# nianticlabs/relpose-gnn

Hardware: AMD Instinct MI355X
Metric: graphs/sec (8-node fully-connected, 224x224) (higher is better)
Workload: dtype f32; 1 GPU; BASELINE.json configs[1]: batch=32 8-node fully-connected graphs per GPU, 224x224 RGB, fp32, ResNet34 + GNN (D=2048, gnn_recursion=2, droprate=0, eval), random-init weights; nodes_per_graph=8, edges_per_graph=56, streams_per_gpu=2, loaded_library=relpose-gnn_amd/lib/librelpose_gnn_hip.so@a301a6756f67

## Files before the change

include/relpose_gnn_hip.h:

```cpp
#ifndef RELPOSE_GNN_HIP_H
#define RELPOSE_GNN_HIP_H

#include <stddef.h>
#include <stdint.h>

#ifdef __cplusplus
extern "C" {
#endif

#define RPG_OK 0
#define RPG_ERR_BAD_ARG (-1)
#define RPG_ERR_LAUNCH (-2)
#define RPG_ERR_WORKSPACE (-3)

#define RPG_ABI_VERSION 1

int rpg_abi_version(void);
const char* rpg_last_error(void);
int rpg_release_scratch(void);


int rpg_nchw3_to_nhwc4_f32(const float* x_nchw, float* y_nhwc4, int n, int h, int w, void* stream);

int rpg_conv2d_bn_act_nhwc_f32(const float* x, const float* w_ohwi, const float* scale, const float* shift,
                               const float* residual, float* y, int n, int h, int w, int cin, int cout,
                               int kh, int kw, int stride, int pad, int relu, void* stream);

size_t rpg_wino43_weights_floats(int cout, int cin);
int rpg_wino43_transform_weights_f32(const float* w_ohwi , float* u, int cout, int cin,
                                     void* stream);
int rpg_conv3x3_wino43_bn_act_nhwc_f32(const float* x, const float* u, const float* scale, const float* shift,
                                       const float* residual, float* y, int n, int h, int w, int cin, int cout,
                                       int relu, void* stream);

int rpg_stem_conv7x7s2_bn_relu_maxpool_f32(const float* x_nchw, const float* wpack, const float* shift, float* y_nhwc,
                                           int n, int h, int w, void* stream);
int rpg_stem_pair_table(int* tap_a, int* tap_b);

int rpg_maxpool3x3s2_nhwc_f32(const float* x, float* y, int n, int h, int w, int c, void* stream);

int rpg_global_avgpool_nhwc_f32(const float* x, float* y, int n, int hw, int c, void* stream);

size_t rpg_resnet_workspace_bytes(int n, int h, int w, const int* planes);
int rpg_resnet_forward_f32(const float* const* tensors, int n_tensors, const int* blocks, const int* planes,
                           int feat_dim, const float* x_nchw, int n, int h, int w, float* feat,
                           void* workspace, size_t workspace_bytes, void* stream);

int rpg_stem_conv7x7s2_bn_relu_maxpool_bf16(const float* x_nchw, const void* wpack_bf16, const float* scale, const float* shift,
                                            void* y_nhwc_bf16, int n, int h, int w, void* stream);
int rpg_stem_conv7x7s2_bn_relu_maxpool_bf16_xbf16(const void* x_nchw_bf16, const void* wpack_bf16, const float* scale, const float* shift,
                                                  void* y_nhwc_bf16, int n, int h, int w, void* stream);
int rpg_conv2d_bn_act_nhwc_bf16(const void* x, const void* w_ohwi, const float* scale, const float* shift,
                                const void* residual, void* y, int n, int h, int w, int cin, int cout, int kh, int kw,
                                int stride, int pad, int relu, int out_f32, void* stream);
size_t rpg_resnet_bf16_workspace_bytes(int n, int h, int w, const int* planes);
int rpg_resnet_forward_bf16(const void* const* tensors, int n_tensors, const int* blocks, const int* planes, int feat_dim,
                            const float* x_nchw, int n, int h, int w, float* feat, void* workspace,
                            size_t workspace_bytes, void* stream);
int rpg_resnet_forward_bf16_xbf16(const void* const* tensors, int n_tensors, const int* blocks, const int* planes, int feat_dim,
                                  const void* x_nchw_bf16, int n, int h, int w, float* feat, void* workspace,
                                  size_t workspace_bytes, void* stream);


int rpg_graph_prepare(const int64_t* src, const int64_t* dst, int64_t node_offset, int e, int n, int64_t* ends,
                      int32_t* rowptr, int32_t* cursor, int32_t* perm, int32_t* status, void* stream);

int rpg_knn_graph_f32(const float* x, const int64_t* batch, int n, int d, int k, int64_t* edge_index,
                      int32_t* cand, int32_t* cnt, int32_t* total, int32_t* status, void* stream);

int rpg_edge_concat_gather_f32(const float* x, const int64_t* edge_index, int e, int d, float* out, void* stream);

int rpg_linear_gather_f32(int n_src, const float* const* a, const int64_t* const* idx, const int* ld,
                          const int* width, const float* weight, const float* bias, const float* residual,
                          float* out, int m, int n_out, int relu, void* stream);

int rpg_linear_gather_ex_f32(int n_src, const float* const* a, const int64_t* const* idx, const int* ld,
                             const int* width, const long* rows, const float* weight, const float* bias,
                             const float* residual, const int64_t* res_idx, const float* residual2,
                             const int64_t* res2_idx, int ldr, float* out, float* out_relu, int m, int n_out, int relu,
                             void* stream);

int rpg_attention_rows_f32(const float* gtp, int r, int c, float* y, void* stream);

int rpg_scatter_mean_f32(const float* msg, const int32_t* rowptr, const int32_t* perm, int n, int e, int d,
                         float* out, void* stream);

int rpg_attention_aggregate_f32(const float* gtp, const float* msg, const int32_t* rowptr, const int32_t* perm,
                                const float* bias, int n, int e, int c, int d, float* ybar, float* mbar, void* stream);

int rpg_pose_heads_f32(const float* x, const float* w6, const float* b6, int r, int d, float* out, void* stream);

size_t rpg_gnn_workspace_bytes(int n, int e, int d);
int rpg_gnn_forward_f32(const float* const* tensors, int n_tensors, const float* feat, const int64_t* src,
                        const int64_t* dst, int64_t node_offset, int n, int e, int d, int gnn_recursion,
                        float* abs_pose, float* rel_pose,
                        float* node_out, float* edge_out, int32_t* status, void* workspace,
                        size_t workspace_bytes, void* stream);

int rpg_gnn_forward_bf16(const float* const* tensors, int n_tensors, const void* const* weights_bf16, int n_bf16,
                         const float* feat, const int64_t* src, const int64_t* dst, int64_t node_offset, int n, int e, int d,
                         int gnn_recursion, float* abs_pose, float* rel_pose, float* node_out, float* edge_out,
                         int32_t* status, void* workspace, size_t workspace_bytes, void* stream);

int rpg_basicblock64_bf16(const void* x, const void* w1_ohwi, const float* scale1, const float* shift1, const void* w2_ohwi,
                          const float* scale2, const float* shift2, void* y, int n, int h, int w, void* stream);

int rpg_f32_to_bf16(const float* src, int ld_src, void* dst, int ld_dst, int col_off, long rows, int cols, void* stream);
int rpg_linear_bf16(const void* a, const void* weight, const float* bias, const float* residual, const int64_t* res_idx,
                    const float* residual2, const int64_t* res2_idx, int ldr, float* out, int m, int k, int n_out,
                    int relu, void* stream);

#define RPG_TIMER_CONV 0
#define RPG_TIMER_LINEAR 1
#define RPG_TIMER_SCATTER 2
#define RPG_TIMER_ATTENTION 3
#define RPG_TIMER_CONV_WINO 4
#define RPG_TIMER_ATT_AGG 5
#define RPG_TIMER_COUNT 6
int rpg_timing_enable(int enable);
int rpg_timing_read(double* ms, long long* launches, double* work);
int rpg_timing_read_ex(double* ms, long long* launches, double* work, double* executed);

int rpg_probe_mfma_bf16(const void* operands, long iters, int workgroups, float* sink, void* stream);

#define RPG_TUNE_TILE 0
#define RPG_TUNE_BK 1
#define RPG_TUNE_EPILOGUE 2
#define RPG_TUNE_STREAMK 3
#define RPG_TUNE_GNN_SPLIT 5
#define RPG_TUNE_BF16_BK 6
#define RPG_TUNE_BF16_FAST 9
#define RPG_TUNE_GNN_FUSE_AGG 13
#define RPG_TUNE_WAVES8 11
#define RPG_TUNE_FUSED_STEM 10
#define RPG_TUNE_WINO_SPLIT 8
#define RPG_TUNE_FAST_LOADER 7
#define RPG_TUNE_WINOGRAD 4
#define RPG_TUNE_WINO_SHORT 12
#define RPG_TUNE_WINO_PERSIST 14
#define RPG_TUNE_BF16_TILE 15
#define RPG_TUNE_BF16_DMA 16
#define RPG_TUNE_BF16_PATCH 17
#define RPG_TUNE_BF16_WS64 18
int rpg_host_f32_to_bf16(const float* src, void* dst_bf16, size_t count);
int rpg_host_f32_to_bf16_isa(const float* src, void* dst_bf16, size_t count, int isa);

#define RPG_TUNE_SK_MIN_ITS 19
#define RPG_TUNE_INKERNEL_FIXUP 20
#define RPG_TUNE_BF16_CHUNK 21
#define RPG_TUNE_WINO2D 22
#define RPG_TUNE_BF16_LEAN_EPI 23
#define RPG_TUNE_BF16_LINEAR_DMA 24
#define RPG_TUNE_BF16_PERSIST 25
#define RPG_TUNE_FOLD_K 26
#define RPG_TUNE_BF16_FUSE_BLOCK 27
#define RPG_TUNE_BF16_TAIL 28
#define RPG_TUNE_LIN112 29
#define RPG_TUNE_FIXUP_PRIO 30
#define RPG_TUNE_BF16_PAIR 31
int rpg_set_tuning(int key, int value);

#ifdef __cplusplus
}
#endif
#endif
```

relpose-gnn_amd/_lib.py:

```python
from __future__ import annotations

import ctypes as C
import os
from typing import Optional, Sequence

HERE = os.path.dirname(os.path.abspath(__file__))
LIB_PATH = os.environ.get("RPG_HIP_LIB") or os.path.join(HERE, "lib", "librelpose_gnn_hip.so")

RPG_OK, RPG_ERR_BAD_ARG, RPG_ERR_LAUNCH, RPG_ERR_WORKSPACE = 0, -1, -2, -3
TIMER_NAMES = ("conv", "linear", "scatter", "attention", "conv_wino", "att_agg")

SYMBOLS = (
    "rpg_abi_version", "rpg_last_error", "rpg_nchw3_to_nhwc4_f32", "rpg_conv2d_bn_act_nhwc_f32",
    "rpg_maxpool3x3s2_nhwc_f32", "rpg_global_avgpool_nhwc_f32", "rpg_resnet_workspace_bytes",
    "rpg_resnet_forward_f32", "rpg_graph_prepare", "rpg_edge_concat_gather_f32", "rpg_linear_gather_f32",
    "rpg_attention_rows_f32", "rpg_scatter_mean_f32", "rpg_pose_heads_f32", "rpg_gnn_workspace_bytes",
    "rpg_gnn_forward_f32", "rpg_timing_enable", "rpg_timing_read", "rpg_set_tuning", "rpg_knn_graph_f32", "rpg_wino43_transform_weights_f32", "rpg_wino43_weights_floats",
    "rpg_conv3x3_wino43_bn_act_nhwc_f32", "rpg_conv2d_bn_act_nhwc_bf16", "rpg_resnet_bf16_workspace_bytes",
    "rpg_resnet_forward_bf16", "rpg_gnn_forward_bf16", "rpg_f32_to_bf16", "rpg_linear_bf16",
    "rpg_release_scratch", "rpg_timing_read_ex", "rpg_stem_conv7x7s2_bn_relu_maxpool_f32", "rpg_stem_pair_table",
    "rpg_attention_aggregate_f32", "rpg_stem_conv7x7s2_bn_relu_maxpool_bf16", "rpg_stem_conv7x7s2_bn_relu_maxpool_bf16_xbf16",
    "rpg_resnet_forward_bf16_xbf16", "rpg_host_f32_to_bf16", "rpg_basicblock64_bf16", "rpg_linear_gather_ex_f32", "rpg_probe_mfma_bf16", "rpg_host_f32_to_bf16_isa",
)


class HipLibraryMissing(RuntimeError):
    pass


class RpgError(RuntimeError):
    pass


_lib: Optional[C.CDLL] = None
_vp, _i, _sz = C.c_void_p, C.c_int, C.c_size_t


def _declare(lib: C.CDLL) -> None:
    lib.rpg_abi_version.restype = _i
    lib.rpg_last_error.restype = C.c_char_p
    lib.rpg_nchw3_to_nhwc4_f32.argtypes = [_vp, _vp, _i, _i, _i, _vp]
    lib.rpg_conv2d_bn_act_nhwc_f32.argtypes = [_vp] * 6 + [_i] * 10 + [_vp]
    lib.rpg_maxpool3x3s2_nhwc_f32.argtypes = [_vp, _vp, _i, _i, _i, _i, _vp]
    lib.rpg_global_avgpool_nhwc_f32.argtypes = [_vp, _vp, _i, _i, _i, _vp]
    lib.rpg_resnet_workspace_bytes.argtypes = [_i, _i, _i, C.POINTER(_i)]
    lib.rpg_resnet_workspace_bytes.restype = _sz
    lib.rpg_resnet_forward_f32.argtypes = [C.POINTER(_vp), _i, C.POINTER(_i), C.POINTER(_i), _i, _vp, _i, _i, _i, _vp,
                                           _vp, _sz, _vp]
    lib.rpg_graph_prepare.argtypes = [_vp, _vp, C.c_int64, _i, _i, _vp, _vp, _vp, _vp, _vp, _vp]
    lib.rpg_edge_concat_gather_f32.argtypes = [_vp, _vp, _i, _i, _vp, _vp]
    lib.rpg_linear_gather_f32.argtypes = [_i, C.POINTER(_vp), C.POINTER(_vp), C.POINTER(_i), C.POINTER(_i), _vp, _vp,
                                          _vp, _vp, _i, _i, _i, _vp]
    lib.rpg_linear_gather_ex_f32.argtypes = [_i, C.POINTER(_vp), C.POINTER(_vp), C.POINTER(_i), C.POINTER(_i), C.POINTER(C.c_long),
                                             _vp, _vp, _vp, _vp, _vp, _vp, _i, _vp, _vp, _i, _i, _i, _vp]
    lib.rpg_attention_rows_f32.argtypes = [_vp, _i, _i, _vp, _vp]
    lib.rpg_scatter_mean_f32.argtypes = [_vp, _vp, _vp, _i, _i, _i, _vp, _vp]
    lib.rpg_attention_aggregate_f32.argtypes = [_vp, _vp, _vp, _vp, _vp, _i, _i, _i, _i, _vp, _vp, _vp]
    lib.rpg_pose_heads_f32.argtypes = [_vp, _vp, _vp, _i, _i, _vp, _vp]
    lib.rpg_gnn_workspace_bytes.argtypes = [_i, _i, _i]
    lib.rpg_gnn_workspace_bytes.restype = _sz
    lib.rpg_gnn_forward_f32.argtypes = [C.POINTER(_vp), _i, _vp, _vp, _vp, C.c_int64, _i, _i, _i, _i, _vp, _vp, _vp, _vp,
                                        _vp, _vp, _sz, _vp]
    lib.rpg_gnn_forward_bf16.argtypes = [C.POINTER(_vp), _i, C.POINTER(_vp), _i, _vp, _vp, _vp, C.c_int64, _i, _i, _i, _i, _vp,
                                         _vp, _vp, _vp, _vp, _vp, _sz, _vp]
    lib.rpg_f32_to_bf16.argtypes = [_vp, _i, _vp, _i, _i, C.c_long, _i, _vp]
    lib.rpg_linear_bf16.argtypes = [_vp] * 7 + [_i, _vp, _i, _i, _i, _i, _vp]
    lib.rpg_timing_enable.argtypes = [_i]
    lib.rpg_set_tuning.argtypes = [_i, _i]
    lib.rpg_conv2d_bn_act_nhwc_bf16.argtypes = [_vp] * 6 + [_i] * 11 + [_vp]
    lib.rpg_basicblock64_bf16.argtypes = [_vp] * 8 + [_i] * 3 + [_vp]
    lib.rpg_resnet_bf16_workspace_bytes.argtypes = [_i, _i, _i, C.POINTER(_i)]
    lib.rpg_resnet_bf16_workspace_bytes.restype = _sz
    lib.rpg_resnet_forward_bf16.argtypes = [C.POINTER(_vp), _i, C.POINTER(_i), C.POINTER(_i), _i, _vp, _i, _i, _i, _vp,
                                            _vp, _sz, _vp]
    lib.rpg_wino43_transform_weights_f32.argtypes = [_vp, _vp, _i, _i, _vp]
    lib.rpg_wino43_weights_floats.argtypes = [_i, _i]
    lib.rpg_wino43_weights_floats.restype = C.c_size_t
    lib.rpg_conv3x3_wino43_bn_act_nhwc_f32.argtypes = [_vp] * 6 + [_i] * 6 + [_vp]
    lib.rpg_knn_graph_f32.argtypes = [_vp, _vp, _i, _i, _i, _vp, _vp, _vp, _vp, _vp, _vp]
    lib.rpg_timing_read.argtypes = [C.POINTER(C.c_double), C.POINTER(C.c_longlong), C.POINTER(C.c_double)]
    lib.rpg_timing_read_ex.argtypes = [C.POINTER(C.c_double), C.POINTER(C.c_longlong), C.POINTER(C.c_double),
                                       C.POINTER(C.c_double)]
    lib.rpg_release_scratch.argtypes = []
    lib.rpg_stem_conv7x7s2_bn_relu_maxpool_f32.argtypes = [_vp, _vp, _vp, _vp, _i, _i, _i, _vp]
    lib.rpg_stem_pair_table.argtypes = [C.POINTER(_i), C.POINTER(_i)]
    lib.rpg_stem_conv7x7s2_bn_relu_maxpool_bf16.argtypes = [_vp, _vp, _vp, _vp, _vp, _i, _i, _i, _vp]
    lib.rpg_stem_conv7x7s2_bn_relu_maxpool_bf16_xbf16.argtypes = [_vp, _vp, _vp, _vp, _vp, _i, _i, _i, _vp]
    lib.rpg_resnet_forward_bf16_xbf16.argtypes = lib.rpg_resnet_forward_bf16.argtypes
    lib.rpg_host_f32_to_bf16.argtypes = [_vp, _vp, _sz]
    lib.rpg_host_f32_to_bf16_isa.argtypes = [_vp, _vp, _sz, _i]
    lib.rpg_probe_mfma_bf16.argtypes = [_vp, C.c_long, _i, _vp, _vp]
    for name in SYMBOLS:
        getattr(lib, name)


def lib() -> C.CDLL:
    global _lib
    if _lib is None:
        path = os.environ.get("RPG_LIB_PATH") or LIB_PATH
        return _load(path)
    return _lib


def _load(LIB_PATH: str) -> C.CDLL:
    global _lib
    if _lib is None:
        if not os.path.exists(LIB_PATH):
            raise HipLibraryMissing(
                f"{LIB_PATH} not found: build it with `python relpose-gnn_amd/build.py` "
                "(the HIP library is the only compute path; there is no fallback)")
        l = C.CDLL(LIB_PATH)
        _declare(l)
        if l.rpg_abi_version() != 1:
            raise HipLibraryMissing(f"{LIB_PATH}: ABI version {l.rpg_abi_version()} != 1, rebuild")
        _lib = l
    return _lib


def check(rc: int, what: str) -> None:
    if rc == RPG_OK:
        return
    if rc == RPG_ERR_BAD_ARG:
        raise ValueError(f"{what}: bad argument (null pointer, non-positive size, unsupported shape or alignment)")
    if rc == RPG_ERR_WORKSPACE:
        raise RpgError(f"{what}: workspace too small")
    msg = lib().rpg_last_error().decode(errors="replace")
    raise RpgError(f"{what}: HIP launch failed: {msg}")


def ptr_array(ptrs: Sequence[Optional[int]]):
    arr = (_vp * len(ptrs))()
    for i, p in enumerate(ptrs):
        arr[i] = p
    return arr


def int_array(vals: Sequence[int]):
    return (_i * len(vals))(*vals)
```

relpose-gnn_amd/build.py:

```python
from __future__ import annotations

import os
import shutil
import subprocess
import sys

HERE = os.path.dirname(os.path.abspath(__file__))
CSRC = os.path.join(HERE, "csrc")
LIB_DIR = os.path.join(HERE, "lib")
LIB_PATH = os.path.join(LIB_DIR, "librelpose_gnn_hip.so")
SOURCES = ("gemm_f32.hip", "winograd.hip", "stem.hip", "stem_bf16.hip", "conv_bf16.hip", "encoder_ops.hip", "gnn_ops.hip", "forward.hip", "timing.hip", "host_ops.hip")
ARCH = "gfx950"
WINOGRAD_SOURCES = ("winograd.hip", "rpg_coherent.h")


def _hipcc() -> str:
    for cand in (os.environ.get("HIPCC"), shutil.which("hipcc"), "/opt/rocm/bin/hipcc"):
        if cand and os.path.exists(cand):
            return cand
    raise RuntimeError("hipcc not found (set HIPCC or install ROCm under /opt/rocm)")


def source_digest(names=None) -> str:
    import hashlib
    h = hashlib.sha256()
    if names is not None:
        files = [os.path.join(CSRC, f) for f in sorted(names)]
    else:
        files = sorted(os.path.join(CSRC, f) for f in os.listdir(CSRC)) + [
            os.path.join(os.path.dirname(HERE), "include", "relpose_gnn_hip.h")]
    for f in files:
        h.update(os.path.basename(f).encode())
        with open(f, "rb") as fh:
            h.update(fh.read())
    return h.hexdigest()[:12]


def needs_build() -> bool:
    if not os.path.exists(LIB_PATH):
        return True
    t = os.path.getmtime(LIB_PATH)
    deps = [os.path.join(CSRC, f) for f in os.listdir(CSRC)] + [
        os.path.join(os.path.dirname(HERE), "include", "relpose_gnn_hip.h")]
    return any(os.path.getmtime(d) > t for d in deps)


def build(force: bool = False, verbose: bool = False) -> str:
    defines = os.environ.get("RPG_BUILD_DEFINES", "").split()
    if defines:
        return _build_to(os.path.join(LIB_DIR, "librelpose_gnn_hip_probe.so"), defines, verbose, obj_suffix=".probe.o")
    if not force and not needs_build():
        return LIB_PATH
    return _build_to(LIB_PATH, [], verbose)


def _build_to(lib_path: str, defines, verbose: bool, obj_suffix: str = ".o") -> str:
    os.makedirs(LIB_DIR, exist_ok=True)
    from concurrent.futures import ThreadPoolExecutor

    def compile_one(src):
        obj = os.path.join(LIB_DIR, src.replace(".hip", obj_suffix))
        cmd = [_hipcc(), f"--offload-arch={ARCH}", "-O3", "-std=c++17", "-fPIC", *defines,
               "-c", os.path.join(CSRC, src), "-o", obj]
        if verbose:
            print(" ".join(cmd), flush=True)
        subprocess.run(cmd, check=True)
        return obj
    with ThreadPoolExecutor(max_workers=min(4, os.cpu_count() or 1)) as pool:
        objs = list(pool.map(compile_one, SOURCES))
    cmd = [_hipcc(), f"--offload-arch={ARCH}", "-shared", "-fPIC", "-o", lib_path + ".tmp", *objs]
    if verbose:
        print(" ".join(cmd), flush=True)
    subprocess.run(cmd, check=True)
    os.replace(lib_path + ".tmp", lib_path)
    return lib_path


if __name__ == "__main__":
    print(build(force="--force" in sys.argv, verbose=True))
```

relpose-gnn_amd/csrc/forward.hip:

```cpp
#include "rpg_common.h"

namespace rpg {
int launch_relu_inplace(float* x, long n_floats, hipStream_t s);
bool stem_pool_supported(int h, int w, int cout);
int launch_stem_pool(const float* x_nchw, const float* wpack, const float* shift, float* out, int n, int h, int w, hipStream_t s);
}

namespace {

inline size_t align_up(size_t v, size_t a) { return (v + a - 1) / a * a; }
inline int conv_out(int x, int k, int s, int p) { return (x + 2 * p - k) / s + 1; }

struct Carver {
    char* base;
    size_t off;
    template <class T>
    T* take(size_t count) {
        T* p = reinterpret_cast<T*>(base + off);
        off += align_up(count * sizeof(T), 256) + rpg::kWorkspaceSkew;
        return p;
    }
};

struct ResnetPlan {
    int h1, w1, h2, w2;
    size_t in4, stem, blk, pool, total_bytes;
};

ResnetPlan plan_resnet(int n, int h, int w, const int* planes) {
    ResnetPlan p{};
    p.h1 = conv_out(h, 7, 2, 3); p.w1 = conv_out(w, 7, 2, 3);
    p.h2 = conv_out(p.h1, 3, 2, 1); p.w2 = conv_out(p.w1, 3, 2, 1);
    p.in4 = (size_t)n * h * w * 4;
    p.stem = (size_t)n * p.h1 * p.w1 * planes[0];
    size_t blk = 0;
    int hh = p.h2, ww = p.w2;
    for (int l = 0; l < 4; ++l) {
        if (l > 0) { hh = conv_out(hh, 3, 2, 1); ww = conv_out(ww, 3, 2, 1); }
        const size_t sz = (size_t)n * hh * ww * planes[l];
        if (sz > blk) blk = sz;
    }
    p.blk = blk;
    p.pool = (size_t)n * planes[3];
    p.total_bytes = align_up(p.in4 * 4, 256) + align_up(p.stem * 4, 256) + 4 * align_up(p.blk * 4, 256) +
                    align_up(p.pool * 4, 256) + align_up(rpg::split_scratch_bytes(), 256) + 8 * rpg::kWorkspaceSkew;
    return p;
}

}

extern "C" size_t rpg_resnet_workspace_bytes(int n, int h, int w, const int* planes) {
    if (n <= 0 || h <= 0 || w <= 0 || !planes) return 0;
    return plan_resnet(n, h, w, planes).total_bytes;
}

extern "C" int rpg_resnet_forward_f32(const float* const* tensors, int n_tensors, const int* blocks, const int* planes,
                                      int feat_dim, const float* x_nchw, int n, int h, int w, float* feat,
                                      void* workspace, size_t workspace_bytes, void* stream) {
    if (!tensors || !blocks || !planes || !x_nchw || !feat || !workspace || n <= 0 || h <= 0 || w <= 0 || feat_dim <= 0)
        return RPG_ERR_BAD_ARG;
    int expect = 4 + 2, cin = planes[0];
    for (int l = 0; l < 4; ++l)
        for (int b = 0; b < blocks[l]; ++b) {
            const int stride = (l > 0 && b == 0) ? 2 : 1;
            expect += 8 + ((stride != 1 || cin != planes[l]) ? 4 : 0);
            cin = planes[l];
        }
    if (n_tensors != expect) return RPG_ERR_BAD_ARG;
    for (int i = 0; i < n_tensors; ++i)
        if (!tensors[i] && !((i & 3) == 3 && i < n_tensors - 2)) return RPG_ERR_BAD_ARG;
    const ResnetPlan p = plan_resnet(n, h, w, planes);
    if (workspace_bytes < p.total_bytes) return RPG_ERR_WORKSPACE;
    hipStream_t s = rpg::as_stream(stream);

    Carver cv{reinterpret_cast<char*>(workspace), 0};
    float* in4 = cv.take<float>(p.in4);
    float* stem = cv.take<float>(p.stem);
    float* buf[4];
    for (int i = 0; i < 4; ++i) buf[i] = cv.take<float>(p.blk);
    float* pool = cv.take<float>(p.pool);
    const size_t scratch_bytes = rpg::split_scratch_bytes();
    rpg::ScratchScope scratch(cv.take<char>(scratch_bytes), scratch_bytes, s);

    int rc;
    int ti = 0;
    if (tensors[3] && rpg::stem_pool_supported(h, w, planes[0])) {
        if ((rc = rpg::launch_stem_pool(x_nchw, tensors[3], tensors[2], buf[0], n, h, w, s)) != RPG_OK) return rc;
    } else {
        if ((rc = rpg_nchw3_to_nhwc4_f32(x_nchw, in4, n, h, w, stream)) != RPG_OK) return rc;
        if ((rc = rpg::launch_conv(in4, tensors[ti], tensors[ti + 1], tensors[ti + 2], nullptr, stem, n, h, w, 4,
                                   planes[0], 7, 7, 2, 3, 1, s, 3)) != RPG_OK)
            return rc;
        if ((rc = rpg_maxpool3x3s2_nhwc_f32(stem, buf[0], n, p.h1, p.w1, planes[0], stream)) != RPG_OK) return rc;
    }
    ti += 4;

    int cur = 0, hh = p.h2, ww = p.w2;
    cin = planes[0];
    for (int l = 0; l < 4; ++l) {
        for (int b = 0; b < blocks[l]; ++b) {
            const int stride = (l > 0 && b == 0) ? 2 : 1;
            const int c = planes[l];
            const bool ds = (stride != 1 || cin != c);
            const int ho = conv_out(hh, 3, stride, 1), wo = conv_out(ww, 3, stride, 1);
            float* X = buf[cur];
            float* T = buf[(cur + 1) & 3];
            float* Y = buf[(cur + 2) & 3];
            float* D = buf[(cur + 3) & 3];
            const bool wino1 = stride == 1 && tensors[ti + 3] && rpg::wino_pays(n, hh, ww, cin, c);
            const bool wino2 = tensors[ti + 7] && rpg::wino_pays(n, ho, wo, c, c);
            if (wino1)
                rc = rpg::launch_conv_wino(X, tensors[ti + 3], tensors[ti + 1], tensors[ti + 2], nullptr, T, n, hh, ww, cin,
                                           c, 1, s);
            else
                rc = rpg::launch_conv(X, tensors[ti], tensors[ti + 1], tensors[ti + 2], nullptr, T, n, hh, ww, cin, c, 3, 3,
                                      stride, 1, 1, s);
            if (rc != RPG_OK) return rc;
            const float* identity = X;
            if (ds) {
                if ((rc = rpg::launch_conv(X, tensors[ti + 8], tensors[ti + 9], tensors[ti + 10], nullptr, D, n, hh, ww,
                                           cin, c, 1, 1, stride, 0, 0, s)) != RPG_OK)
                    return rc;
                identity = D;
            }
            if (wino2)
                rc = rpg::launch_conv_wino(T, tensors[ti + 7], tensors[ti + 5], tensors[ti + 6], identity, Y, n, ho, wo, c, c,
                                           1, s);
            else
                rc = rpg::launch_conv(T, tensors[ti + 4], tensors[ti + 5], tensors[ti + 6], identity, Y, n, ho, wo, c, c, 3,
                                      3, 1, 1, 1, s);
            if (rc != RPG_OK) return rc;
            ti += ds ? 12 : 8;
            cur = (cur + 2) & 3;
            hh = ho; ww = wo; cin = c;
        }
    }
    if ((rc = rpg_global_avgpool_nhwc_f32(buf[cur], pool, n, hh * ww, cin, stream)) != RPG_OK) return rc;
    rpg::GatherSrc src{};
    src.n = 1; src.a[0] = pool; src.idx[0] = nullptr; src.ld[0] = cin; src.width[0] = cin;
    return rpg::launch_linear(src, tensors[ti], tensors[ti + 1], nullptr, feat, n, feat_dim, 0, s);
}

namespace {
enum GnnTensor {
    T_PROJ_W, T_PROJ_B, T_EDGE0_W, T_EDGE0_B, T_EDGE2_W, T_EDGE2_B, T_MSG0_W, T_MSG0_B, T_MSG2_W, T_MSG2_B,
    T_GTP_W, T_GTP_B, T_ATTW_W, T_ATTW_B, T_UPD0_W, T_UPD0_B, T_UPD2_W, T_UPD2_B, T_HEADN_W, T_HEADN_B,
    T_HEADE_W, T_HEADE_B, T_COUNT,
    T_PROJN_W = T_COUNT,
    T_NODE3_W,
    T_EDGE0E_W,
    T_MSG0E_W,
    T_COUNT_SPLIT
};

struct GnnPlan {
    size_t total_bytes;
};
size_t gnn_bytes(int n, int e, int d) {
    const size_t c = d / 8;
    size_t b = 0;
    auto add = [&](size_t bytes, int count = 1) { b += count * (align_up(bytes, 256) + rpg::kWorkspaceSkew); };
    add((size_t)4 * e * 8);
    add((size_t)(n + 1) * 4);
    add((size_t)n * 4);
    add((size_t)e * 4);
    add((size_t)e * d * 4, 6);
    add((size_t)e * 3 * c * 4);
    add((size_t)e * c * 4);
    add((size_t)n * d * 4, 4);
    add((size_t)n * 3 * d * 4);
    add((size_t)(e > 2 * n ? e : 2 * n) * d * 2);
    add(rpg::split_scratch_bytes());
    return b;
}
}

extern "C" size_t rpg_gnn_workspace_bytes(int n, int e, int d) {
    if (n <= 0 || e <= 0 || d <= 0 || (d & 31)) return 0;
    return gnn_bytes(n, e, d);
}

namespace {
enum BfWeight { B_PROJN, B_NODE3, B_EDGE0E, B_EDGE2, B_MSG0E, B_MSG2, B_GTP, B_ATTW, B_UPD0, B_UPD2, B_COUNT };

int gnn_forward_impl(const float* const* tensors, int n_tensors, const void* const* wb, const float* feat, const int64_t* esrc,
                     const int64_t* edst, int64_t node_offset, int n, int e, int d, int gnn_recursion, float* abs_pose,
                     float* rel_pose, float* node_out, float* edge_out, int32_t* status, void* workspace,
                     size_t workspace_bytes, void* stream) {
    if (!tensors || (n_tensors != T_COUNT && n_tensors != T_COUNT_SPLIT) || !feat || !esrc || !edst || !abs_pose || !rel_pose || !status || !workspace ||
        n <= 0 || e <= 0 || d <= 0 || (d & 31) || gnn_recursion < 0)
        return RPG_ERR_BAD_ARG;
    for (int i = 0; i < n_tensors; ++i)
        if (!tensors[i]) return RPG_ERR_BAD_ARG;
    if (workspace_bytes < gnn_bytes(n, e, d)) return RPG_ERR_WORKSPACE;
    const bool split = (n_tensors == T_COUNT_SPLIT) && (wb || rpg::gnn_split_enabled());
    if (wb && !split) return RPG_ERR_BAD_ARG;
    hipStream_t s = rpg::as_stream(stream);
    const int c = d / 8;

    Carver cv{reinterpret_cast<char*>(workspace), 0};
    int64_t* ends = cv.take<int64_t>((size_t)4 * e);
    int32_t* rowptr = cv.take<int32_t>((size_t)n + 1);
    int32_t* cursor = cv.take<int32_t>((size_t)n);
    int32_t* perm = cv.take<int32_t>((size_t)e);
    float* ebuf[2] = {cv.take<float>((size_t)e * d), cv.take<float>((size_t)e * d)};
    float* eraw = cv.take<float>((size_t)e * d);
    float* hid = cv.take<float>((size_t)e * d);
    float* msg = cv.take<float>((size_t)e * d);
    float* att = cv.take<float>((size_t)e * d);
    float* gtp = cv.take<float>((size_t)e * 3 * c);
    float* yat = cv.take<float>((size_t)e * c);
    float* agg = cv.take<float>((size_t)n * d);
    float* nhid = cv.take<float>((size_t)n * d);
    float* xbuf[2] = {cv.take<float>((size_t)n * d), cv.take<float>((size_t)n * d)};
    float* node3 = cv.take<float>((size_t)n * 3 * d);
    void* abf = cv.take<unsigned short>((size_t)(e > 2 * n ? e : 2 * n) * d);
    const size_t scratch_bytes = rpg::split_scratch_bytes();
    rpg::ScratchScope scratch(cv.take<char>(scratch_bytes), scratch_bytes, s);

    int rc;
    if ((rc = rpg_graph_prepare(esrc, edst, node_offset, e, n, ends, rowptr, cursor, perm, status, stream)) != RPG_OK) return rc;
    const int64_t* src = ends;
    const int64_t* dst = ends + e;
    const int64_t* lo = ends + 2 * (size_t)e;
    const int64_t* hi = ends + 3 * (size_t)e;

    auto linear = [&](int ns, const float* a0, const int64_t* i0, int w0, const float* a1, const int64_t* i1, int w1,
                      const float* a2, const int64_t* i2, int w2, int wt, const float* residual, float* out, int m,
                      int n_out, int relu, float* out_relu = nullptr, bool with_bias = true) {
        const float* bias = with_bias ? tensors[wt + 1] : nullptr;
        rpg::GatherSrc g{};
        g.n = ns;
        g.a[0] = a0; g.idx[0] = i0; g.ld[0] = w0; g.width[0] = w0;
        g.a[1] = a1; g.idx[1] = i1; g.ld[1] = w1; g.width[1] = w1;
        g.a[2] = a2; g.idx[2] = i2; g.ld[2] = w2; g.width[2] = w2;
        for (int i = 0; i < 3; ++i) g.rows[i] = g.idx[i] ? (n > e ? n : e) : 0;
        if (wb) {
            int bw = -1;
            switch (wt) {
                case T_EDGE2_W: bw = B_EDGE2; break;
                case T_MSG2_W: bw = B_MSG2; break;
                case T_GTP_W: bw = B_GTP; break;
                case T_ATTW_W: bw = B_ATTW; break;
                case T_UPD0_W: bw = B_UPD0; break;
                case T_UPD2_W: bw = B_UPD2; break;
                default: return RPG_ERR_BAD_ARG;
            }
            const int k = w0 + (ns > 1 ? w1 : 0);
            if (ns > 2 || i0 || i1) return RPG_ERR_BAD_ARG;
            int r2;
            if ((r2 = rpg::launch_f32_to_bf16(a0, w0, abf, k, 0, m, w0, s)) != RPG_OK) return r2;
            if (ns > 1 && (r2 = rpg::launch_f32_to_bf16(a1, w1, abf, k, w0, m, w1, s)) != RPG_OK) return r2;
            if (out_relu) return RPG_ERR_BAD_ARG;
            return rpg::launch_linear_bf16(abf, wb[bw], bias, residual, nullptr, nullptr, nullptr, n_out, out, m, k,
                                           n_out, relu, s);
        }
        return rpg::launch_linear(g, tensors[wt], bias, residual, out, m, n_out, relu, s, nullptr, out_relu);
    };

    auto node_gemm = [&](const float* xin, int wt, int n_out) {
        rpg::GatherSrc g{};
        g.n = 1; g.a[0] = xin; g.idx[0] = nullptr; g.ld[0] = d; g.width[0] = d;
        if (wb) {
            int r2;
            if ((r2 = rpg::launch_f32_to_bf16(xin, d, abf, d, 0, n, d, s)) != RPG_OK) return r2;
            return rpg::launch_linear_bf16(abf, wb[wt == T_PROJN_W ? B_PROJN : B_NODE3], nullptr, nullptr, nullptr, nullptr,
                                           nullptr, 0, node3, n, d, n_out, 0, s);
        }
        return rpg::launch_linear(g, tensors[wt], nullptr, nullptr, node3, n, n_out, 0, s);
    };
    auto edge_gemm = [&](const float* ein, int wt, int bias_t, const float* r1, const int64_t* i1, const float* r2,
                         const int64_t* i2, float* out) {
        rpg::GatherSrc g{};
        g.n = 1; g.a[0] = ein; g.idx[0] = nullptr; g.ld[0] = d; g.width[0] = d;
        const rpg::GatherRes gr{r1, i1, r2, i2, 3 * d};
        if (wb) {
            int rcb;
            if ((rcb = rpg::launch_f32_to_bf16(ein, d, abf, d, 0, e, d, s)) != RPG_OK) return rcb;
            return rpg::launch_linear_bf16(abf, wb[wt == T_EDGE0E_W ? B_EDGE0E : B_MSG0E], tensors[bias_t], r1, i1, r2, i2, 3 * d,
                                           out, e, d, d, 1, s);
        }
        return rpg::launch_linear(g, tensors[wt], tensors[bias_t], nullptr, out, e, d, 1, s, &gr);
    };

    const bool fuse_agg = rpg::gnn_fuse_agg_enabled();
    if (wb && fuse_agg && split) {
        typedef unsigned short bf;
        {
            const size_t e_buf = (size_t)e * d * sizeof(float), n_buf = (size_t)n * d * sizeof(float);
            const size_t a_buf = (size_t)(e > 2 * n ? e : 2 * n) * d * sizeof(bf);
            if (2 * (size_t)e * d * sizeof(bf) > e_buf ||
                (size_t)n * 2 * d * sizeof(bf) > n_buf ||
                (size_t)n * d * sizeof(bf) > n_buf ||
                (size_t)n * c * sizeof(bf) > a_buf)
                return RPG_ERR_WORKSPACE;
        }
        bf* eb = reinterpret_cast<bf*>(eraw);
        bf* enb = eb + (size_t)e * d;
        bf* hb = reinterpret_cast<bf*>(hid);
        bf* mb = hb + (size_t)e * d;
        bf* xab = reinterpret_cast<bf*>(nhid);
        bf* nhb = reinterpret_cast<bf*>(agg);
        bf* yb = reinterpret_cast<bf*>(abf);
        auto gemm = [&](const void* a, int lda, int k, int bw, const float* bias, const float* r1, const int64_t* i1, const float* r2,
                        const int64_t* i2, int ldr, void* out, int out_f32, void* out2, int ld2, int relu2, int m, int n_out, int relu) {
            rpg::LinearBf16Out o{};
            o.out = out; o.out_f32 = out_f32; o.out2 = out2; o.ld2 = ld2; o.relu2 = relu2;
            return rpg::launch_linear_bf16_ex(a, lda, wb[bw], bias, r1, i1, r2, i2, ldr, o, m, k, n_out, relu, s);
        };
        if ((rc = rpg::launch_f32_to_bf16(feat, d, xab, 2 * d, 0, n, d, s)) != RPG_OK) return rc;
        if ((rc = gemm(xab, 2 * d, d, B_PROJN, nullptr, nullptr, nullptr, nullptr, nullptr, 0, node3, 1, nullptr, 0, 0, n, 2 * d, 0)) != RPG_OK) return rc;
        float* ecur = ebuf[0];
        if ((rc = rpg::launch_gather_add2_relu(node3, lo, hi, tensors[T_PROJ_B], ecur, e, d, s)) != RPG_OK) return rc;
        if ((rc = rpg::launch_f32_to_bf16(ecur, d, eb, d, 0, e, d, s)) != RPG_OK) return rc;
        const float* x = feat;
        for (int r = 0; r < gnn_recursion; ++r) {
            const bool last = r + 1 == gnn_recursion;
            float* xnew = xbuf[r & 1];
            if ((rc = gemm(xab, 2 * d, d, B_NODE3, nullptr, nullptr, nullptr, nullptr, nullptr, 0, node3, 1, nullptr, 0, 0, n, 3 * d, 0)) != RPG_OK) return rc;
            if ((rc = gemm(eb, d, d, B_EDGE0E, tensors[T_EDGE0_B], node3, src, node3 + d, dst, 3 * d, hb, 0, nullptr, 0, 0, e, d, 1)) != RPG_OK) return rc;
            if (last) rc = gemm(hb, d, d, B_EDGE2, tensors[T_EDGE2_B], nullptr, nullptr, nullptr, nullptr, 0, ebuf[1], 1, enb, d, 0, e, d, 1);
            else rc = gemm(hb, d, d, B_EDGE2, tensors[T_EDGE2_B], nullptr, nullptr, nullptr, nullptr, 0, eb, 0, enb, d, 0, e, d, 1);
            if (rc != RPG_OK) return rc;
            if (last) ecur = ebuf[1];
            if ((rc = gemm(enb, d, d, B_MSG0E, tensors[T_MSG0_B], node3 + 2 * d, src, nullptr, nullptr, 3 * d, hb, 0, nullptr, 0, 0, e, d, 1)) != RPG_OK) return rc;
            if ((rc = gemm(hb, d, d, B_MSG2, tensors[T_MSG2_B], nullptr, nullptr, nullptr, nullptr, 0, msg, 1, mb, d, 0, e, d, 0)) != RPG_OK) return rc;
            if ((rc = gemm(mb, d, d, B_GTP, tensors[T_GTP_B], nullptr, nullptr, nullptr, nullptr, 0, gtp, 1, nullptr, 0, 0, e, 3 * c, 0)) != RPG_OK) return rc;
            if ((rc = rpg_attention_aggregate_f32(gtp, msg, rowptr, perm, tensors[T_ATTW_B], n, e, c, d, yat, att, stream)) != RPG_OK) return rc;
            if ((rc = rpg::launch_f32_to_bf16(yat, c, yb, c, 0, n, c, s)) != RPG_OK) return rc;
            if ((rc = gemm(yb, c, c, B_ATTW, nullptr, att, nullptr, nullptr, nullptr, d, nullptr, 0, xab + d, 2 * d, 0, n, d, 0)) != RPG_OK) return rc;
            if ((rc = gemm(xab, 2 * d, 2 * d, B_UPD0, tensors[T_UPD0_B], nullptr, nullptr, nullptr, nullptr, 0, nhb, 0, nullptr, 0, 0, n, d, 1)) != RPG_OK) return rc;
            if ((rc = gemm(nhb, d, d, B_UPD2, tensors[T_UPD2_B], nullptr, nullptr, nullptr, nullptr, 0, xnew, 1, xab, 2 * d, 1, n, d, 1)) != RPG_OK) return rc;
            x = xnew;
        }
        if (node_out && hipMemcpyAsync(node_out, x, (size_t)n * d * 4, hipMemcpyDeviceToDevice, s) != hipSuccess) {
            rpg::set_last_error("gnn_forward node_out", hipGetLastError());
            return RPG_ERR_LAUNCH;
        }
        if (edge_out && hipMemcpyAsync(edge_out, ecur, (size_t)e * d * 4, hipMemcpyDeviceToDevice, s) != hipSuccess) {
            rpg::set_last_error("gnn_forward edge_out", hipGetLastError());
            return RPG_ERR_LAUNCH;
        }
        if ((rc = rpg_pose_heads_f32(x, tensors[T_HEADN_W], tensors[T_HEADN_B], n, d, abs_pose, stream)) != RPG_OK) return rc;
        return rpg_pose_heads_f32(ecur, tensors[T_HEADE_W], tensors[T_HEADE_B], e, d, rel_pose, stream);
    }

    const float* x = feat;
    float* ecur = ebuf[0];
    if (split) {
        if ((rc = node_gemm(x, T_PROJN_W, 2 * d)) != RPG_OK) return rc;
        if ((rc = rpg::launch_gather_add2_relu(node3, lo, hi, tensors[T_PROJ_B], ecur, e, d, s)) != RPG_OK) return rc;
    } else if ((rc = linear(2, x, lo, d, x, hi, d, nullptr, nullptr, 0, T_PROJ_W, nullptr, ecur, e, d, 1)) != RPG_OK) {
        return rc;
    }

    const bool dual = !wb;
    for (int r = 0; r < gnn_recursion; ++r) {
        float* enext = (ecur == ebuf[0]) ? ebuf[1] : ebuf[0];
        float* enew = dual ? eraw : enext;
        float* xnew = xbuf[r & 1];
        if (split) {
            if ((rc = node_gemm(x, T_NODE3_W, 3 * d)) != RPG_OK) return rc;
            if ((rc = edge_gemm(ecur, T_EDGE0E_W, T_EDGE0_B, node3, src, node3 + d, dst, hid)) != RPG_OK) return rc;
        } else if ((rc = linear(3, x, src, d, x, dst, d, ecur, nullptr, d, T_EDGE0_W, nullptr, hid, e, d, 1)) != RPG_OK) {
            return rc;
        }
        if ((rc = linear(1, hid, nullptr, d, nullptr, nullptr, 0, nullptr, nullptr, 0, T_EDGE2_W, nullptr, enew, e, d, 0,
                         dual ? enext : nullptr)) != RPG_OK)
            return rc;
        if (split) {
            if ((rc = edge_gemm(enew, T_MSG0E_W, T_MSG0_B, node3 + 2 * d, src, nullptr, nullptr, hid)) != RPG_OK) return rc;
        } else if ((rc = linear(2, x, src, d, enew, nullptr, d, nullptr, nullptr, 0, T_MSG0_W, nullptr, hid, e, d, 1)) != RPG_OK) {
            return rc;
        }
        if ((rc = linear(1, hid, nullptr, d, nullptr, nullptr, 0, nullptr, nullptr, 0, T_MSG2_W, nullptr, msg, e, d, 0)) != RPG_OK) return rc;
        if ((rc = linear(1, msg, nullptr, d, nullptr, nullptr, 0, nullptr, nullptr, 0, T_GTP_W, nullptr, gtp, e, 3 * c, 0)) != RPG_OK) return rc;
        if (fuse_agg) {
            if ((rc = rpg_attention_aggregate_f32(gtp, msg, rowptr, perm, tensors[T_ATTW_B], n, e, c, d, yat, att, stream)) != RPG_OK)
                return rc;
            if ((rc = linear(1, yat, nullptr, c, nullptr, nullptr, 0, nullptr, nullptr, 0, T_ATTW_W, att, agg, n, d, 0, nullptr,
                             false)) != RPG_OK)
                return rc;
        } else {
            if ((rc = rpg_attention_rows_f32(gtp, e, c, yat, stream)) != RPG_OK) return rc;
            if ((rc = linear(1, yat, nullptr, c, nullptr, nullptr, 0, nullptr, nullptr, 0, T_ATTW_W, msg, att, e, d, 0)) != RPG_OK) return rc;
            if ((rc = rpg_scatter_mean_f32(att, rowptr, perm, n, e, d, agg, stream)) != RPG_OK) return rc;
        }
        if ((rc = linear(2, x, nullptr, d, agg, nullptr, d, nullptr, nullptr, 0, T_UPD0_W, nullptr, nhid, n, d, 1)) != RPG_OK) return rc;
        if ((rc = linear(1, nhid, nullptr, d, nullptr, nullptr, 0, nullptr, nullptr, 0, T_UPD2_W, nullptr, xnew, n, d, 1)) != RPG_OK) return rc;
        if (!dual && (rc = rpg::launch_relu_inplace(enext, (long)e * d, s)) != RPG_OK) return rc;
        x = xnew;
        ecur = enext;
    }
    if (node_out && hipMemcpyAsync(node_out, x, (size_t)n * d * 4, hipMemcpyDeviceToDevice, s) != hipSuccess) {
        rpg::set_last_error("gnn_forward node_out", hipGetLastError());
        return RPG_ERR_LAUNCH;
    }
    if (edge_out && hipMemcpyAsync(edge_out, ecur, (size_t)e * d * 4, hipMemcpyDeviceToDevice, s) != hipSuccess) {
        rpg::set_last_error("gnn_forward edge_out", hipGetLastError());
        return RPG_ERR_LAUNCH;
    }
    if ((rc = rpg_pose_heads_f32(x, tensors[T_HEADN_W], tensors[T_HEADN_B], n, d, abs_pose, stream)) != RPG_OK) return rc;
// ... 23 lines not shown
```

relpose-gnn_amd/csrc/gemm_f32.hip:

```cpp
#include <atomic>
#include <map>
#include <mutex>
#include <type_traits>
#include <utility>
#include <vector>

#include "rpg_common.h"

typedef float f32x16 __attribute__((ext_vector_type(16)));

namespace {


struct Epilogue {
    const float* scale;
    const float* shift;
    const float* residual;
    float* out;
    int ldc;
    int relu;
    const int64_t* res_idx = nullptr;
    const float* residual2 = nullptr;
    const int64_t* res2_idx = nullptr;
    int ldr = 0;
// ... 193 lines not shown
        const int row = qj < 4 ? 32 * qj : L112_BM + 32 * (qj - 4);
        if (qj == 3) {
            if (srow < 16) *reinterpret_cast<float4*>(&lds[img + st_off + row * L112_LD]) = rr[set][qj];
        } else {
            *reinterpret_cast<float4*>(&lds[img + st_off + row * L112_LD]) = rr[set][qj];
        }
    };
    const int a_off = (lane & 15) * L112_LD + 4 * (lane >> 4);
    const int b_off = (L112_BM + 16 * wave + (lane & 15)) * L112_LD + 4 * (lane >> 4);
    float4 fa[2][7], fb[2];
    auto read_job = [&](int set, int rj, int kb, int img) {
        if (rj < 7) fa[set][rj] = *reinterpret_cast<const float4*>(&lds[img + a_off + rj * 16 * L112_LD + kb]);
        else fb[set] = *reinterpret_cast<const float4*>(&lds[img + b_off + kb]);
    };
    auto comp = [](const float4& v, int c) { return c == 0 ? v.x : c == 1 ? v.y : c == 2 ? v.z : v.w; };
    f32x4m acc[7], acc2[7];
#pragma unroll
    for (int i = 0; i < 7; ++i)
#pragma unroll
        for (int e = 0; e < 4; ++e) { acc[i][e] = 0.f; acc2[i][e] = 0.f; }

    const int nsteps = K / L112_BK;
    auto kstep = [&](int cur, int nxt, int wset, int kload) {
        __builtin_amdgcn_sched_barrier(0);
#pragma unroll
        for (int g = 0; g < 2; ++g) {
#pragma unroll
            for (int ms = 0; ms < 28; ++ms) {
                const int c = ms / 7, i = ms % 7;
                acc[i] = __builtin_amdgcn_mfma_f32_16x16x4f32(comp(fa[g][i], c), comp(fb[g], c), acc[i], 0, 0, 0);
                if (g == 0) {
                    if (ms < 8) read_job(1, ms, 16, cur);
                    else if (ms < 14) write_job(wset, ms - 8, nxt);
                    else if (ms < 20) load_job(wset, ms - 14, kload);
                } else {
                    if (ms < 8) read_job(0, ms, 0, nxt);
                }
                __builtin_amdgcn_sched_barrier(0);
            }
            if (g == 0) {
                __syncthreads();
                __builtin_amdgcn_sched_barrier(0);
            }
        }
    };
#pragma unroll
    for (int qj = 0; qj < 6; ++qj) load_job(0, qj, 0);
#pragma unroll
    for (int qj = 0; qj < 6; ++qj) load_job(1, qj, L112_BK);
#pragma unroll
    for (int qj = 0; qj < 6; ++qj) write_job(0, qj, 0);
#pragma unroll
    for (int qj = 0; qj < 6; ++qj) load_job(0, qj, 2 * L112_BK);
    __syncthreads();
#pragma unroll
    for (int rj = 0; rj < 8; ++rj) read_job(0, rj, 0, 0);
    const int fold_steps = fold_k >= 2 * L112_BK ? (fold_k / L112_BK) & ~1 : 0x7ffffffe;
    int kt = 0;
    while (kt + 1 < nsteps) {
        int kstop = kt + fold_steps;
        if (kstop > nsteps) kstop = nsteps;
        for (; kt + 1 < kstop; kt += 2) {
            kstep(0, L112_STAGE, 1, (kt + 3) * L112_BK);
            kstep(L112_STAGE, 0, 0, (kt + 4) * L112_BK);
        }
        if (kt + 1 < nsteps) {
            asm volatile("");
#pragma unroll
            for (int i = 0; i < 7; ++i) { acc2[i] += acc[i]; acc[i] = f32x4m{0.f, 0.f, 0.f, 0.f}; }
        }
    }
    if (kt < nsteps) kstep(0, L112_STAGE, 1, (kt + 3) * L112_BK);
#pragma unroll
    for (int i = 0; i < 7; ++i) acc[i] += acc2[i];
    __syncthreads();
    constexpr int SP = L112_BN + 4;
#pragma unroll
    for (int i = 0; i < 7; ++i)
#pragma unroll
        for (int e = 0; e < 4; ++e) lds[(16 * i + 4 * (lane >> 4) + e) * SP + 16 * wave + (lane & 15)] = acc[i][e];
    __syncthreads();
#pragma unroll
    for (int t = 0; t < L112_BM * (L112_BN / 4) / L112_NT; ++t) {
        const int idx4 = t * L112_NT + tid;
        const int row = idx4 / (L112_BN / 4), c4 = idx4 % (L112_BN / 4);
        const float4 v = *reinterpret_cast<const float4*>(&lds[row * SP + 4 * c4]);
        eng4::streamk_finish_quad<L112_BM, L112_BN>(v, ep, M, N, tiles_n, tile, idx4, 1);
    }
}

constexpr int L112_NT2 = 512;
__global__ __launch_bounds__(L112_NT2, 1) void linear112k2_kernel(const float* __restrict__ A, int lda, const float* __restrict__ Wt, int ldw,
                                                                 int M, int N, int K, Epilogue ep, int tiles_n, int fold_k) {
    extern __shared__ __attribute__((aligned(16))) float lds[];
    const int nwg = gridDim.x, bid = blockIdx.x;
    const int xcd = bid & 7, loc = bid >> 3, q = nwg >> 3, r = nwg & 7;
    const int tile = (xcd < r ? xcd * (q + 1) : r * (q + 1) + (xcd - r) * q) + loc;
    const int m0 = (tile / tiles_n) * L112_BM, n0 = (tile % tiles_n) * L112_BN;
    const int tid = threadIdx.x, lane = tid & 63;
    const int wave = __builtin_amdgcn_readfirstlane(tid >> 6);
    const int kw = wave >> 2, wv = wave & 3;
    const int slot = tid & 7, srow = tid >> 3;
    const __amdgpu_buffer_rsrc_t rsa = make_rsrc(A + (size_t)m0 * lda);
    const __amdgpu_buffer_rsrc_t rsw = make_rsrc(Wt + (size_t)n0 * ldw);
    unsigned soff[3];
    soff[0] = 4u * (unsigned)(srow * lda + 4 * slot);
    soff[1] = srow + 64 < L112_BM ? 4u * (unsigned)((srow + 64) * lda + 4 * slot) : OOB;
    soff[2] = 4u * (unsigned)(srow * ldw + 4 * slot);
    const int st_off = srow * L112_LD + 4 * slot;
    float4 rr[2][3];
    auto load_job = [&](int set, int qj, int kpos) {
        const bool live = kpos < K;
        rr[set][qj] = buf_ld4(qj < 2 ? rsa : rsw, live ? soff[qj] : OOB, 4u * (unsigned)kpos);
    };
    auto write_job = [&](int set, int qj, int img) {
        const int row = qj == 0 ? 0 : (qj == 1 ? 64 : L112_BM);
        if (qj == 1) {
            if (srow + 64 < L112_BM) *reinterpret_cast<float4*>(&lds[img + st_off + row * L112_LD]) = rr[set][qj];
        } else {
            *reinterpret_cast<float4*>(&lds[img + st_off + row * L112_LD]) = rr[set][qj];
        }
    };
    const int a_off = (lane & 15) * L112_LD + 4 * (lane >> 4) + 16 * kw;
    const int b_off = (L112_BM + 16 * wv + (lane & 15)) * L112_LD + 4 * (lane >> 4) + 16 * kw;
    float4 fa[2][7], fb[2];
    auto read_job = [&](int set, int rj, int img) {
        if (rj < 7) fa[set][rj] = *reinterpret_cast<const float4*>(&lds[img + a_off + rj * 16 * L112_LD]);
        else fb[set] = *reinterpret_cast<const float4*>(&lds[img + b_off]);
    };
    auto comp = [](const float4& v, int c) { return c == 0 ? v.x : c == 1 ? v.y : c == 2 ? v.z : v.w; };
    f32x4m acc[7], acc2[7];
#pragma unroll
    for (int i = 0; i < 7; ++i)
#pragma unroll
        for (int e = 0; e < 4; ++e) { acc[i][e] = 0.f; acc2[i][e] = 0.f; }
    const int nsteps = K / L112_BK;
    auto kstep = [&](int fset, int nxt, int wset, int kload) {
        __builtin_amdgcn_sched_barrier(0);
#pragma unroll
        for (int ms = 0; ms < 28; ++ms) {
            const int c = ms / 7, i = ms % 7;
            acc[i] = __builtin_amdgcn_mfma_f32_16x16x4f32(comp(fa[fset][i], c), comp(fb[fset], c), acc[i], 0, 0, 0);
            if (ms < 3) write_job(wset, ms, nxt);
            else if (ms < 6) load_job(wset, ms - 3, kload);
            else if (ms >= 14 && ms < 22) read_job(fset ^ 1, ms - 14, nxt);
            __builtin_amdgcn_sched_barrier(0);
            if (ms == 13) {
                __syncthreads();
                __builtin_amdgcn_sched_barrier(0);
            }
        }
    };
#pragma unroll
    for (int qj = 0; qj < 3; ++qj) load_job(0, qj, 0);
#pragma unroll
    for (int qj = 0; qj < 3; ++qj) load_job(1, qj, L112_BK);
#pragma unroll
    for (int qj = 0; qj < 3; ++qj) write_job(0, qj, 0);
#pragma unroll
    for (int qj = 0; qj < 3; ++qj) load_job(0, qj, 2 * L112_BK);
    __syncthreads();
#pragma unroll
    for (int rj = 0; rj < 8; ++rj) read_job(0, rj, 0);
    const int fold_steps = fold_k >= 2 * L112_BK ? (fold_k / L112_BK) & ~1 : 0x7ffffffe;
    int kt = 0;
    while (kt + 1 < nsteps) {
        int kstop = kt + fold_steps;
        if (kstop > nsteps) kstop = nsteps;
        for (; kt + 1 < kstop; kt += 2) {
            kstep(0, L112_STAGE, 1, (kt + 3) * L112_BK);
            kstep(1, 0, 0, (kt + 4) * L112_BK);
        }
        if (kt + 1 < nsteps) {
            asm volatile("");
#pragma unroll
            for (int i = 0; i < 7; ++i) { acc2[i] += acc[i]; acc[i] = f32x4m{0.f, 0.f, 0.f, 0.f}; }
        }
    }
    if (kt < nsteps) kstep(0, L112_STAGE, 1, (kt + 3) * L112_BK);
#pragma unroll
    for (int i = 0; i < 7; ++i) acc[i] += acc2[i];
    __syncthreads();
    constexpr int SP = L112_BN + 4;
    if (kw == 1) {
#pragma unroll
        for (int i = 0; i < 7; ++i)
#pragma unroll
            for (int e = 0; e < 4; ++e) lds[(16 * i + 4 * (lane >> 4) + e) * SP + 16 * wv + (lane & 15)] = acc[i][e];
    }
    __syncthreads();
    if (kw == 0) {
#pragma unroll
        for (int i = 0; i < 7; ++i)
#pragma unroll
            for (int e = 0; e < 4; ++e) {
                float* p = &lds[(16 * i + 4 * (lane >> 4) + e) * SP + 16 * wv + (lane & 15)];
                *p = acc[i][e] + *p;
            }
    }
    __syncthreads();
    for (int idx4 = tid; idx4 < L112_BM * (L112_BN / 4); idx4 += L112_NT2) {
        const int row = idx4 / (L112_BN / 4), c4 = idx4 % (L112_BN / 4);
        const float4 v = *reinterpret_cast<const float4*>(&lds[row * SP + 4 * c4]);
        eng4::streamk_finish_quad<L112_BM, L112_BN>(v, ep, M, N, tiles_n, tile, idx4, 1);
    }
}

bool launch_linear112(const float* A, int lda, const float* Wt, int ldw, int M, int N, int K, const Epilogue& ep, hipStream_t s) {
    if (!(g_lin112 & 1) || M % L112_BM || N % L112_BN || K % L112_BK || K < 2 * L112_BK) return false;
    const int tm = M / L112_BM, tn = N / L112_BN;
    const long tiles = (long)tm * tn;
    if (tiles < cu_count() || (long)L112_BM * lda * 4 >= (1L << 31) || (long)L112_BN * ldw * 4 >= (1L << 31)) return false;
    const bool vec_ok = (ep.ldc % 4 == 0) && rpg::aligned16(ep.out) && (!ep.residual || rpg::aligned16(ep.residual)) &&
                        (!ep.residual2 || rpg::aligned16(ep.residual2)) && (ep.ldr % 4 == 0) && (!ep.scale || rpg::aligned16(ep.scale)) &&
                        (!ep.shift || rpg::aligned16(ep.shift)) && (!ep.out_relu || rpg::aligned16(ep.out_relu)) && rpg::aligned16(A) &&
                        rpg::aligned16(Wt) && (lda % 4 == 0) && (ldw % 4 == 0);
    if (!vec_ok) return false;
    t_executed = 2.0 * (double)M * N * (double)K;
    if ((g_lin112 & 2) && 2 * tiles < 3L * cu_count())
        hipLaunchKernelGGL(linear112k2_kernel, dim3((unsigned)tiles), dim3(L112_NT2), L112_LDS_BYTES, s, A, lda, Wt, ldw, M, N, K, ep, tn, g_fold_k);
    else
        hipLaunchKernelGGL(linear112_kernel, dim3((unsigned)tiles), dim3(L112_NT), L112_LDS_BYTES, s, A, lda, Wt, ldw, M, N, K, ep, tn, g_fold_k);
    return true;
}

template <int BK, bool EPI, template <int, int> class Loader, class Args>
void launch_shape(TileShape t, const Args& args, const float* Wt, int ldw, int M, int N, int K, const Epilogue& ep,
                  bool vec_ok, hipStream_t s) {
    switch (t) {
        case TILE_128x128: eng4::launch_one<128, 128, 2, 2, BK, EPI, Loader, Args>(args, Wt, ldw, M, N, K, ep, vec_ok, s); break;
        case TILE_256x64: eng4::launch_one<256, 64, 4, 1, BK, EPI, Loader, Args>(args, Wt, ldw, M, N, K, ep, vec_ok, s); break;
        case TILE_128x64: eng4::launch_one<128, 64, 2, 2, BK, EPI, Loader, Args>(args, Wt, ldw, M, N, K, ep, vec_ok, s); break;
        default: eng4::launch_one<64, 64, 2, 2, BK, EPI, Loader, Args>(args, Wt, ldw, M, N, K, ep, vec_ok, s); break;
    }
}

template <template <int, int> class Loader8, class Args>
void launch_shape8(TileShape t, const Args& args, const float* Wt, int ldw, int M, int N, int K, const Epilogue& ep,
                   hipStream_t s) {
    if (t == TILE_128x128) eng8::launch_one<128, 128, 2, 4, 32, true, Loader8, Args>(args, Wt, ldw, M, N, K, ep, true, s);
    else eng8::launch_one<128, 64, 4, 2, 32, true, Loader8, Args>(args, Wt, ldw, M, N, K, ep, true, s);
}

int g_fast = 1;
int g_waves8 = 1;

struct ConvKind {
    template <int R, int BK> using L4 = eng4::ConvLoader<R, BK>;
    template <int R, int BK> using B4 = eng4::ConvLoaderB<R, BK>;
    template <int R, int BK> using T4 = eng4::ConvLoaderTap<R, BK>;
    template <int R, int BK> using B8 = eng8::ConvLoaderB<R, BK>;
};
struct GatherKind {
    template <int R, int BK> using L4 = eng4::GatherLoader<R, BK>;
    template <int R, int BK> using B4 = eng4::GatherLoaderB<R, BK>;
    template <int R, int BK> using T4 = eng4::GatherLoaderB<R, BK>;
    template <int R, int BK> using B8 = eng8::GatherLoaderB<R, BK>;
};

template <class Kind, class Args>
int launch_tiles(const Args& args, const float* Wt, int ldw, int M, int N, int K, const Epilogue& ep, hipStream_t s,
                 int seg_align) {
    TileShape t = pick_tile(M, N, K);
    if (std::is_same<Kind, GatherKind>::value && g_fold_k > 0 && g_force_tile < 0 && t == TILE_128x128 && K >= 2 * g_fold_k) t = TILE_128x64;
    const int bk = g_bk ? g_bk : (((t == TILE_128x128 || t == TILE_128x64) && K >= 256) ? 32 : 16);
    const bool vec_ok = (N % 4 == 0) && (ep.ldc % 4 == 0) && rpg::aligned16(ep.out) &&
                        (!ep.residual || rpg::aligned16(ep.residual)) && (!ep.residual2 || rpg::aligned16(ep.residual2)) &&
                        (ep.ldr % 4 == 0) && (!ep.scale || rpg::aligned16(ep.scale)) &&
                        (!ep.shift || rpg::aligned16(ep.shift));
    const bool epi = g_epi_lds && vec_ok;
    const bool fast = g_fast && epi && seg_align > 0 && seg_align % bk == 0 && K % bk == 0 &&
                      (long)N * ldw * 4 < (1L << 31);
    if (g_fast && epi && seg_align == -1 && (long)N * ldw * 4 < (1L << 31)) {
        if (bk == 32) launch_shape<32, true, Kind::template T4, Args>(t, args, Wt, ldw, M, N, K, ep, vec_ok, s);
        else launch_shape<16, true, Kind::template T4, Args>(t, args, Wt, ldw, M, N, K, ep, vec_ok, s);
        return 0;
    }
    if (fast && bk == 32 && g_waves8 && (t == TILE_128x128 || t == TILE_128x64)) {
        launch_shape8<Kind::template B8, Args>(t, args, Wt, ldw, M, N, K, ep, s);
        return 0;
    }
    if (bk == 32) {
        if (fast) launch_shape<32, true, Kind::template B4, Args>(t, args, Wt, ldw, M, N, K, ep, vec_ok, s);
        else if (epi) launch_shape<32, true, Kind::template L4, Args>(t, args, Wt, ldw, M, N, K, ep, vec_ok, s);
        else launch_shape<32, false, Kind::template L4, Args>(t, args, Wt, ldw, M, N, K, ep, vec_ok, s);
    } else {
        if (fast) launch_shape<16, true, Kind::template B4, Args>(t, args, Wt, ldw, M, N, K, ep, vec_ok, s);
        else if (epi) launch_shape<16, true, Kind::template L4, Args>(t, args, Wt, ldw, M, N, K, ep, vec_ok, s);
        else launch_shape<16, false, Kind::template L4, Args>(t, args, Wt, ldw, M, N, K, ep, vec_ok, s);
    }
    return 0;
}

}

namespace rpg {

bool gnn_split_enabled() { return g_gnn_split != 0; }
bool gnn_fuse_agg_enabled() { return g_gnn_fuse_agg != 0; }
float* stream_scratch(hipStream_t s, size_t bytes, unsigned** counters) { return get_scratch(s, bytes, counters); }
hipStream_t fixup_hop_begin(hipStream_t s) { return fixup_hop_begin_impl(s); }
void fixup_hop_end(hipStream_t s, hipStream_t used) { fixup_hop_end_impl(s, used); }
bool inkernel_fixup_enabled() { return (g_inkernel_fixup & 2) != 0; }
ScratchScope::ScratchScope(void* p, size_t bytes, hipStream_t s) {
    if (p && bytes >= kCounterBytes && hipMemsetAsync(p, 0, kCounterBytes, s) != hipSuccess) { (void)hipGetLastError(); p = nullptr; bytes = 0; }
    t_scratch.p = static_cast<float*>(p);
    t_scratch.bytes = p ? bytes : 0;
    t_scratch.on = true;
}
ScratchScope::~ScratchScope() { t_scratch = ScratchTls{}; }
size_t split_scratch_bytes() { return (size_t)2 * 3 * cu_count() * 65536 + kCounterBytes; }
int num_cus() { return cu_count(); }

int launch_conv(const float* x, const float* w, const float* scale, const float* shift, const float* residual,
                float* y, int n, int h, int wd, int cin, int cout, int kh, int kw, int stride, int pad, int relu,
                hipStream_t s, int alg_cin) {
    if (!x || !w || !y || n <= 0 || h <= 0 || wd <= 0 || cin <= 0 || cout <= 0 || kh <= 0 || kw <= 0 ||
        stride <= 0 || pad < 0 || (cin & 3) || !aligned16(x) || !aligned16(w) || !aligned16(y))
        return RPG_ERR_BAD_ARG;
    const int ho = (h + 2 * pad - kh) / stride + 1, wo = (wd + 2 * pad - kw) / stride + 1;
    if (ho <= 0 || wo <= 0) return RPG_ERR_BAD_ARG;
    const long M = (long)n * ho * wo;
    const long K = (long)kh * kw * cin;
    if (M >= (1L << 31) || K >= (1 << 24) || (long)h * wd * cin >= (1L << 31)) return RPG_ERR_BAD_ARG;
    ConvArgs a{x, h, wd, cin, kh, kw, stride, pad, ho, wo};
    Epilogue ep{scale, shift, residual, y, cout, relu};
    const int slot = timing_begin(RPG_TIMER_CONV, s);
    const long span = 256 / ((long)ho * wo) + 2;
    int seg = span * h * wd * cin * 4 >= (1L << 31) ? 0 : (cin % 32 == 0 ? 32 : (cin % 16 == 0 ? 16 : 0));
    if (cin == 4 && kh * kw <= 64 && kw >= 4 && span * h * wd * cin * 4 < (1L << 31)) seg = -1;
    launch_tiles<ConvKind, ConvArgs>(a, w, (int)K, (int)M, cout, (int)K, ep, s, seg);
    timing_end(slot, 2.0 * (double)M * cout * (double)kh * kw * (alg_cin > 0 ? alg_cin : cin), s, t_executed);
    RPG_CHECK_LAUNCH("conv2d_bn_act");
    return RPG_OK;
}

int launch_linear(const GatherSrc& src, const float* weight, const float* bias, const float* residual, float* out,
                  int m, int n_out, int relu, hipStream_t s, const GatherRes* gres, float* out_relu) {
    if (src.n < 1 || src.n > 3 || !weight || !out || m <= 0 || n_out <= 0 || !aligned16(weight)) return RPG_ERR_BAD_ARG;
    GatherArgs a{};
    int K = 0;
    for (int i = 0; i < 3; ++i) {
        if (i < src.n) {
            if (!src.a[i] || src.width[i] <= 0 || (src.width[i] & 3) || (src.ld[i] & 3) || src.ld[i] < src.width[i] ||
                !aligned16(src.a[i]))
                return RPG_ERR_BAD_ARG;
            a.a[i] = src.a[i]; a.idx[i] = src.idx[i]; a.ld[i] = src.ld[i];
            K += src.width[i];
        } else {
            a.a[i] = nullptr; a.idx[i] = nullptr; a.ld[i] = 0;
        }
    }
    a.w0 = src.width[0];
    a.w01 = src.n >= 2 ? src.width[0] + src.width[1] : K;
    a.K = K;
    a.fold_k = g_fold_k;
    Epilogue ep{nullptr, bias, residual, out, n_out, relu};
    ep.out_relu = out_relu;
    if (out_relu && !aligned16(out_relu)) return RPG_ERR_BAD_ARG;
    if (gres) {
        if (!gres->res1 || !gres->idx1 || gres->ld < n_out || (gres->res2 && !gres->idx2)) return RPG_ERR_BAD_ARG;
        ep.residual = gres->res1; ep.res_idx = gres->idx1;
        ep.residual2 = gres->res2; ep.res2_idx = gres->idx2;
        ep.ldr = gres->ld;
    }
    const int slot = timing_begin(RPG_TIMER_LINEAR, s);
    int seg = 32;
    for (int i = 0; i < src.n; ++i) {
        if (src.width[i] % 32) seg = src.width[i] % 16 ? 0 : (seg ? 16 : 0);
        const long rows = src.idx[i] ? src.rows[i] : (long)m;
        if (rows <= 0 || rows * src.ld[i] * 4 >= (1L << 31)) seg = 0;
    }
    if (!(src.n == 1 && !src.idx[0] && launch_linear112(src.a[0], src.ld[0], weight, K, m, n_out, K, ep, s)))
        launch_tiles<GatherKind, GatherArgs>(a, weight, K, m, n_out, K, ep, s, seg);
    timing_end(slot, 2.0 * (double)m * n_out * (double)K, s, t_executed);
    RPG_CHECK_LAUNCH("linear_gather");
    return RPG_OK;
}

}

extern "C" int rpg_conv2d_bn_act_nhwc_f32(const float* x, const float* w_ohwi, const float* scale, const float* shift,
                                          const float* residual, float* y, int n, int h, int w, int cin, int cout,
                                          int kh, int kw, int stride, int pad, int relu, void* stream) {
    return rpg::launch_conv(x, w_ohwi, scale, shift, residual, y, n, h, w, cin, cout, kh, kw, stride, pad, relu,
                            rpg::as_stream(stream));
}

extern "C" int rpg_linear_gather_f32(int n_src, const float* const* a, const int64_t* const* idx, const int* ld,
                                     const int* width, const float* weight, const float* bias, const float* residual,
                                     float* out, int m, int n_out, int relu, void* stream) {
    if (n_src < 1 || n_src > 3 || !a || !ld || !width) return RPG_ERR_BAD_ARG;
    rpg::GatherSrc src{};
    src.n = n_src;
    for (int i = 0; i < n_src; ++i) {
        src.a[i] = a[i];
        src.idx[i] = idx ? idx[i] : nullptr;
        src.ld[i] = ld[i];
        src.width[i] = width[i];
    }
    return rpg::launch_linear(src, weight, bias, residual, out, m, n_out, relu, rpg::as_stream(stream));
}

extern "C" int rpg_linear_gather_ex_f32(int n_src, const float* const* a, const int64_t* const* idx, const int* ld,
                                        const int* width, const long* rows, const float* weight, const float* bias,
                                        const float* residual, const int64_t* res_idx, const float* residual2,
                                        const int64_t* res2_idx, int ldr, float* out, float* out_relu, int m, int n_out,
                                        int relu, void* stream) {
    if (n_src < 1 || n_src > 3 || !a || !ld || !width) return RPG_ERR_BAD_ARG;
    rpg::GatherSrc src{};
    src.n = n_src;
    for (int i = 0; i < n_src; ++i) {
        src.a[i] = a[i];
        src.idx[i] = idx ? idx[i] : nullptr;
        src.ld[i] = ld[i];
        src.width[i] = width[i];
        src.rows[i] = rows ? rows[i] : 0;
    }
    if (!res_idx && !residual2)
        return (res2_idx || (residual && ldr && ldr != n_out)) ? RPG_ERR_BAD_ARG
               : rpg::launch_linear(src, weight, bias, residual, out, m, n_out, relu, rpg::as_stream(stream), nullptr, out_relu);
    rpg::GatherRes gr{residual, res_idx, residual2, res2_idx, ldr};
    return rpg::launch_linear(src, weight, bias, nullptr, out, m, n_out, relu, rpg::as_stream(stream), &gr, out_relu);
}

extern "C" int rpg_release_scratch(void) {
    if (hipDeviceSynchronize() != hipSuccess) {
        rpg::set_last_error("release_scratch", hipGetLastError());
        return RPG_ERR_LAUNCH;
    }
    std::lock_guard<std::mutex> lk(g_scratch_mu);
    for (auto& kv : g_scratch)
        if (kv.second.p) (void)hipFree(kv.second.p);
    g_scratch.clear();
    for (float* p : g_retired) (void)hipFree(p);
    g_retired.clear();
    return RPG_OK;
}

extern "C" int rpg_set_tuning(int key, int value) {
    switch (key) {
        case RPG_TUNE_FIXUP_PRIO: g_fixup_prio = value != 0; return RPG_OK;
        case RPG_TUNE_BF16_PAIR: rpg::bf16_set_pair(value != 0); return RPG_OK;
        case RPG_TUNE_TILE: g_force_tile = value; return RPG_OK;
        case RPG_TUNE_BK: if (value != 0 && value != 16 && value != 32) return RPG_ERR_BAD_ARG; g_bk = value; return RPG_OK;
        case RPG_TUNE_EPILOGUE: g_epi_lds = value != 0; return RPG_OK;
        case RPG_TUNE_STREAMK: g_streamk = value != 0; return RPG_OK;
        case RPG_TUNE_BF16_BK: if (value != 32 && value != 64) return RPG_ERR_BAD_ARG; rpg::bf16_set_bk(value); return RPG_OK;
        case RPG_TUNE_INKERNEL_FIXUP:
            if (value < 0 || value > 7) return RPG_ERR_BAD_ARG;
            g_inkernel_fixup = value & 3;
            rpg::wino_combine_max_set((value & 4) ? 32 : 8);
            return RPG_OK;
        case RPG_TUNE_GNN_SPLIT: g_gnn_split = value != 0; return RPG_OK;
        case RPG_TUNE_GNN_FUSE_AGG: g_gnn_fuse_agg = value != 0; return RPG_OK;
        case RPG_TUNE_LIN112: if (value < 0 || value > 3) return RPG_ERR_BAD_ARG; g_lin112 = value; return RPG_OK;
        case RPG_TUNE_FOLD_K: if (value < 0 || (value % 64)) return RPG_ERR_BAD_ARG; g_fold_k = value; return RPG_OK;
        case RPG_TUNE_FAST_LOADER: g_fast = value != 0; return RPG_OK;
        case RPG_TUNE_WAVES8: g_waves8 = value != 0; return RPG_OK;
        case RPG_TUNE_WINO_SPLIT: if (value < 0 || value > 96) return RPG_ERR_BAD_ARG; rpg::wino_split_set(value); return RPG_OK;
        case RPG_TUNE_BF16_TILE: if (value < -1 || value > 3) return RPG_ERR_BAD_ARG; rpg::bf16_set_tile(value); return RPG_OK;
        case RPG_TUNE_BF16_FAST: rpg::bf16_set_fast(value != 0); return RPG_OK;
        case RPG_TUNE_BF16_LEAN_EPI: rpg::bf16_set_lean_epi(value != 0); return RPG_OK;
        case RPG_TUNE_BF16_PERSIST: rpg::bf16_set_persist(value != 0); return RPG_OK;
        case RPG_TUNE_BF16_FUSE_BLOCK: rpg::bf16_set_fuse_block((int)(value & 7)); return RPG_OK;
        case RPG_TUNE_BF16_TAIL: if (value < 0 || value > 7) return RPG_ERR_BAD_ARG; rpg::bf16_set_tail(value); return RPG_OK;
        case RPG_TUNE_BF16_LINEAR_DMA: if (value != 0 && (value < 10 || value > 19)) return RPG_ERR_BAD_ARG; rpg::bf16_set_linear_dma(value); return RPG_OK;
        case RPG_TUNE_WINO2D:
            if (value < 0 || value > 2 || (value != 0 && rpg_wino43_weights_floats(1, 1) != 42)) return RPG_ERR_BAD_ARG;
            rpg::wino2d_set(value);
            return RPG_OK;
        case RPG_TUNE_BF16_CHUNK:
            if (value < 0) return RPG_ERR_BAD_ARG;
            rpg::bf16_set_chunk(value & 4095, (value >> 12) ? (value >> 12) : 64);
            return RPG_OK;
        case RPG_TUNE_BF16_PATCH: if (value < 0 || value % 10 > 4 || value > 14) return RPG_ERR_BAD_ARG; rpg::bf16_set_patch(value); return RPG_OK;
        case RPG_TUNE_BF16_DMA: if (value < 0 || value > 40) return RPG_ERR_BAD_ARG; rpg::bf16_set_dma(value); return RPG_OK;
        case RPG_TUNE_SK_MIN_ITS: if (value < 1 || value > 4096) return RPG_ERR_BAD_ARG; SK_MIN_ITS = value; return RPG_OK;
        case RPG_TUNE_BF16_WS64: if (value < 0 || value > 2) return RPG_ERR_BAD_ARG; return rpg::bf16_set_ws64(value);
        case RPG_TUNE_FUSED_STEM: rpg::stem_pool_set((value & 1) != 0); rpg::stem_pool_set_strip((value & 128) != 0, value >> 8); rpg::bf16_set_fused_stem((value & 1) != 0); rpg::bf16_set_stem_strip((value & 2) ? 0 : ((value & 32) ? 1 : 9), value >> 8); return RPG_OK;
        case RPG_TUNE_WINOGRAD: if (value < 0 || (value > 3 && value < 16)) return RPG_ERR_BAD_ARG; rpg::wino_set(value); return RPG_OK;
        case RPG_TUNE_WINO_PERSIST: if (value < 0 || value > 2) return RPG_ERR_BAD_ARG; rpg::wino_persist_set(value); return RPG_OK;
        case RPG_TUNE_WINO_SHORT: if (value < 0) return RPG_ERR_BAD_ARG; rpg::wino_short_set(value); return RPG_OK;
        default: return RPG_ERR_BAD_ARG;
    }
}
```

relpose-gnn_amd/csrc/rpg_common.h:

```cpp
#pragma once
#include <hip/hip_runtime.h>
#include <stdint.h>
#include <stdio.h>

#include "../../include/relpose_gnn_hip.h"

#include "rpg_coherent.h"

namespace rpg {

void set_last_error(const char* where, hipError_t e);

inline hipStream_t as_stream(void* s) { return reinterpret_cast<hipStream_t>(s); }

int timing_begin(int klass, hipStream_t s);
void timing_end(int slot, double work, hipStream_t s, double executed = 0.0);

#define RPG_CHECK_LAUNCH(where)                         \
    do {                                                \
        hipError_t _e = hipGetLastError();              \
        if (_e != hipSuccess) {                         \
            rpg::set_last_error(where, _e);             \
            return RPG_ERR_LAUNCH;                      \
        }                                               \
    } while (0)

inline bool aligned16(const void* p) { return (reinterpret_cast<uintptr_t>(p) & 15u) == 0; }


struct GatherSrc {
    const float* a[3];
    const int64_t* idx[3];
    int ld[3];
    int width[3];
    int n;
    long rows[3];
};

int launch_conv(const float* x, const float* w, const float* scale, const float* shift, const float* residual,
                float* y, int n, int h, int wd, int cin, int cout, int kh, int kw, int stride, int pad, int relu,
                hipStream_t s, int alg_cin = 0 );
int launch_conv_wino(const float* x, const float* u, const float* scale, const float* shift, const float* residual,
                     float* y, int n, int h, int w, int cin, int cout, int relu, hipStream_t s);
constexpr size_t kWorkspaceSkew = 260 * 1024 + 4096;

float* stream_scratch(hipStream_t s, size_t bytes, unsigned** counters = nullptr);
hipStream_t fixup_hop_begin(hipStream_t s);
void fixup_hop_end(hipStream_t s, hipStream_t used);
bool inkernel_fixup_enabled();
struct ScratchScope {
    ScratchScope(void* p, size_t bytes, hipStream_t s);
    ~ScratchScope();
    ScratchScope(const ScratchScope&) = delete;
    ScratchScope& operator=(const ScratchScope&) = delete;
};
size_t split_scratch_bytes();
int num_cus();
bool wino_enabled();
bool wino_pays(int n, int h, int w, int cin, int cout);
void wino_set(int on);
void wino2d_set(int v);
size_t wino_weight_floats(int cout, int cin);
int launch_wino2d_weights(const float* w_ohwi, float* u2, int cout, int cin, hipStream_t s);
bool wino2d_takes(int n, int h, int w, int cin, int cout);
int launch_conv_wino2d(const float* x, const float* u2, const float* scale, const float* shift, const float* residual, float* y,
                       int n, int h, int w, int cin, int cout, int relu, hipStream_t s);
void stem_pool_set(int on);
void stem_pool_set_strip(int on, int band_rows);
void wino_split_set(int on);
void wino_short_set(int cin);
void wino_persist_set(int on);
void wino_combine_max_set(int v);
void bf16_set_fast(int on);
void bf16_set_tile(int t);
void bf16_set_dma(int v);
void bf16_set_patch(int v);
void bf16_set_fused_stem(int on);
void bf16_set_stem_strip(int on, int band_rows);
void bf16_set_chunk(int images, int min_mb);
void bf16_set_lean_epi(int on);
void bf16_set_persist(int v);
void bf16_set_fuse_block(int v);
void bf16_set_tail(int v);
void bf16_set_pair(int v);
void bf16_set_linear_dma(int v);
int bf16_set_ws64(int v);
bool stem_pool_bf16_supported(int n, int h, int w, int cout);
int launch_stem_pool_bf16(const void* x_nchw, int x_is_bf16, const void* wpack, const float* scale, const float* shift, void* out, int n, int h,
                          int w, hipStream_t s);
int launch_f32_to_bf16(const float* src, int ld_src, void* dst, int ld_dst, int col_off, long rows, int cols, hipStream_t s);
int launch_linear_bf16(const void* a, const void* w, const float* bias, const float* res, const int64_t* res_idx,
                       const float* res2, const int64_t* res2_idx, int ldr, float* out, int m, int k, int n_out, int relu,
                       hipStream_t s);
struct LinearBf16Out {
    void* out = nullptr;
    int out_f32 = 1;
    void* out2 = nullptr;
    int ld2 = 0;
    int relu2 = 0;
};
int launch_linear_bf16_ex(const void* a, int lda, const void* w, const float* bias, const float* res, const int64_t* res_idx,
                          const float* res2, const int64_t* res2_idx, int ldr, const LinearBf16Out& o, int m, int k, int n_out,
                          int relu, hipStream_t s);
struct GatherRes {
    const float* res1;
    const int64_t* idx1;
    const float* res2;
    const int64_t* idx2;
    int ld;
};
int launch_linear(const GatherSrc& src, const float* weight, const float* bias, const float* residual, float* out,
                  int m, int n_out, int relu, hipStream_t s, const GatherRes* gres = nullptr, float* out_relu = nullptr);
int launch_gather_add2_relu(const float* pq, const int64_t* lo, const int64_t* hi, const float* bias, float* out, int e,
                            int d, hipStream_t s);
bool gnn_split_enabled();
bool gnn_fuse_agg_enabled();
void bf16_set_bk(int bk);

}
```

relpose-gnn_amd/csrc/winograd.hip:

```cpp
#include "rpg_common.h"

typedef float f32x16 __attribute__((ext_vector_type(16)));

namespace {

constexpr int NT = 256;
constexpr int BK = 16, LD = BK;
constexpr int P = 6;
constexpr int BMT = 64, BN = 64;
constexpr int A_FLOATS = P * BMT * LD, B_FLOATS = P * BN * LD;
constexpr int LDS_BYTES = (A_FLOATS + B_FLOATS) * (int)sizeof(float);

struct Epi {
    const float* scale;
    const float* shift;
    const float* residual;
    float* out;
    int relu;
};

__device__ __forceinline__ float4 f4zero() { return make_float4(0.f, 0.f, 0.f, 0.f); }
__device__ __forceinline__ float4 lin(float a, const float4& x, float b, const float4& y) {
    return make_float4(a * x.x + b * y.x, a * x.y + b * y.y, a * x.z + b * y.z, a * x.w + b * y.w);
}
__device__ __forceinline__ float4 add(const float4& x, const float4& y) {
    return make_float4(x.x + y.x, x.y + y.y, x.z + y.z, x.w + y.w);
}
__device__ __forceinline__ float4 sub(const float4& x, const float4& y) {
    return make_float4(x.x - y.x, x.y - y.y, x.z - y.z, x.w - y.w);
}

typedef unsigned int u32x4 __attribute__((ext_vector_type(4)));
typedef float f32x2 __attribute__((ext_vector_type(2)));
__device__ __forceinline__ void wino43_epilogue(const f32x16 (&acc)[P], float* slab, int lane, int mw0, int nw0, int M,
                                                int Tw, int W, int Cout, const Epi& ep) {
    constexpr int EP = 32 + 4;
    constexpr unsigned OOB = 0x80000000u;
    const int c4 = lane & 7, pr = lane >> 3;
    const int nb = nw0 + 4 * c4;
    const bool n_ok = nb < Cout;
    float4 sc = make_float4(1.f, 1.f, 1.f, 1.f), sh = f4zero();
    if (n_ok && ep.scale) sc = *reinterpret_cast<const float4*>(ep.scale + nb);
    if (n_ok && ep.shift) sh = *reinterpret_cast<const float4*>(ep.shift + nb);

    const int t_first = mw0 / Tw;
    const size_t row0 = (size_t)t_first * W * Cout;
    const __amdgpu_buffer_rsrc_t ro = __builtin_amdgcn_make_buffer_rsrc(ep.out + row0, 0, 0x7fffffff, 0x00020000);
    const __amdgpu_buffer_rsrc_t rr = __builtin_amdgcn_make_buffer_rsrc(
        const_cast<float*>(ep.residual ? ep.residual + row0 : ep.out + row0), 0, 0x7fffffff, 0x00020000);
    const int step_t = 4 / Tw, step_tw = 4 % Tw;
    int mt = mw0 + (pr >> 1);
    int trel = mt / Tw - t_first, tw = mt % Tw;
    unsigned voff[2][8];
#pragma unroll
    for (int it = 0; it < 8; ++it) {
        const int wo = 4 * tw + (pr & 1);
        const bool ok = n_ok && mt < M;
        const unsigned o = 4u * (unsigned)((trel * W + wo) * Cout + nb);
        voff[0][it] = ok && wo < W ? o : OOB;
        voff[1][it] = ok && wo + 2 < W ? o + 8u * (unsigned)Cout : OOB;
        mt += 4;
        trel += step_t;
        tw += step_tw;
        if (tw >= Tw) { tw -= Tw; ++trel; }
    }
    float4 rs[2][8];
    if (ep.residual) {
#pragma unroll
        for (int half = 0; half < 2; ++half)
#pragma unroll
            for (int it = 0; it < 8; ++it)
                rs[half][it] = __builtin_bit_cast(float4, __builtin_amdgcn_raw_buffer_load_b128(rr, voff[half][it], 0, 0));
    } else {
#pragma unroll
        for (int half = 0; half < 2; ++half)
#pragma unroll
            for (int it = 0; it < 8; ++it) rs[half][it] = f4zero();
    }
    const float floor_v = ep.relu ? 0.f : -INFINITY;
    f32x2 y[4][8];
#pragma unroll
    for (int q = 0; q < 8; ++q) {
        const int e = 2 * q;
        const f32x2 m0 = {acc[0][e], acc[0][e + 1]}, m1 = {acc[1][e], acc[1][e + 1]}, m2 = {acc[2][e], acc[2][e + 1]};
        const f32x2 m3 = {acc[3][e], acc[3][e + 1]}, m4 = {acc[4][e], acc[4][e + 1]}, m5 = {acc[5][e], acc[5][e + 1]};
        const f32x2 s12 = m1 + m2, d12 = m1 - m2, s34 = m3 + m4, d34 = m3 - m4;
        const f32x2 u = d34 + d34;
        y[0][q] = (m0 + s12) + s34;
        y[1][q] = d12 + u;
        y[2][q] = s12 + 4.f * s34;
        y[3][q] = (d12 + 4.f * u) + m5;
    }
#pragma unroll
    for (int half = 0; half < 2; ++half) {
#pragma unroll
        for (int q = 0; q < 8; ++q) {
            const int e = 2 * q;
            const int trow = (e & 3) + 8 * (e >> 2) + 4 * (lane >> 5);
            float* sp = slab + (2 * trow) * EP + (lane & 31);
            sp[0] = y[2 * half][q].x;
            sp[EP] = y[2 * half + 1][q].x;
            sp[2 * EP] = y[2 * half][q].y;
            sp[3 * EP] = y[2 * half + 1][q].y;
        }
        __builtin_amdgcn_wave_barrier();
#pragma unroll
        for (int it = 0; it < 8; ++it) {
            const int prow = pr + 8 * it;
            const float4 v = *reinterpret_cast<const float4*>(&slab[prow * EP + 4 * c4]);
            const f32x2 r0 = {rs[half][it].x, rs[half][it].y}, r1 = {rs[half][it].z, rs[half][it].w};
            f32x2 o0 = f32x2{v.x, v.y} * f32x2{sc.x, sc.y} + f32x2{sh.x, sh.y} + r0;
            f32x2 o1 = f32x2{v.z, v.w} * f32x2{sc.z, sc.w} + f32x2{sh.z, sh.w} + r1;
            const float4 yv = make_float4(fmaxf(o0.x, floor_v), fmaxf(o0.y, floor_v), fmaxf(o1.x, floor_v), fmaxf(o1.y, floor_v));
            __builtin_amdgcn_raw_buffer_store_b128(__builtin_bit_cast(u32x4, yv), ro, voff[half][it], 0, 0);
        }
        __builtin_amdgcn_wave_barrier();
    }
}

template <bool RES, class Mid>
__device__ __forceinline__ void wino43_epilogue_lean_body(const f32x16 (&acc)[P], float* slab, int lane, int mw0, int nw0, int M,
                                                          int Tw, int W, int Cout, const Epi& ep, Mid mid) {
    constexpr int EP = 32 + 4;
    constexpr unsigned OOB = 0x80000000u;
    const int c4 = lane & 7, pr = lane >> 3;
    const int nb = nw0 + 4 * c4;
    const bool n_ok = nb < Cout;
    float4 sc = make_float4(1.f, 1.f, 1.f, 1.f), sh = f4zero();
    if (n_ok && ep.scale) sc = *reinterpret_cast<const float4*>(ep.scale + nb);
    if (n_ok && ep.shift) sh = *reinterpret_cast<const float4*>(ep.shift + nb);
    const int t_first = mw0 / Tw;
    const size_t row0 = (size_t)t_first * W * Cout;
    const __amdgpu_buffer_rsrc_t ro = __builtin_amdgcn_make_buffer_rsrc(ep.out + row0, 0, 0x7fffffff, 0x00020000);
    const __amdgpu_buffer_rsrc_t rr = __builtin_amdgcn_make_buffer_rsrc(
        const_cast<float*>(ep.residual ? ep.residual + row0 : ep.out + row0), 0, 0x7fffffff, 0x00020000);
    const int step_t = 4 / Tw, step_tw = 4 % Tw;
    int mt = mw0 + (pr >> 1);
    int trel = mt / Tw - t_first, tw = mt % Tw;
    unsigned voff[8], ok2 = 0;
#pragma unroll
    for (int it = 0; it < 8; ++it) {
        const int wo = 4 * tw + (pr & 1);
        const bool ok = n_ok && mt < M;
        voff[it] = ok && wo < W ? 4u * (unsigned)((trel * W + wo) * Cout + nb) : OOB;
        if (ok && wo + 2 < W) ok2 |= 1u << it;
        mt += 4;
        trel += step_t;
        tw += step_tw;
        if (tw >= Tw) { tw -= Tw; ++trel; }
    }
    const unsigned half_b = 8u * (unsigned)Cout;
    auto off = [&](int half, int it) -> unsigned {
        return half == 0 ? voff[it] : ((ok2 >> it) & 1u) ? voff[it] + half_b : OOB;
    };
    int relu_i = ep.relu;
    asm volatile("" : "+s"(relu_i));
    const float floor_v = relu_i ? 0.f : -INFINITY;
    float4 rs[2][8];
    auto load_res = [&](int half) {
        if (RES) {
#pragma unroll
            for (int it = 0; it < 8; ++it)
                rs[half][it] = __builtin_bit_cast(float4, __builtin_amdgcn_raw_buffer_load_b128(rr, off(half, it), 0, 0));
        }
    };
    auto transform_to_slab = [&](int half) {
#pragma unroll
        for (int q = 0; q < 8; ++q) {
            const int e = 2 * q;
            const f32x2 m1 = {acc[1][e], acc[1][e + 1]}, m2 = {acc[2][e], acc[2][e + 1]};
            const f32x2 m3 = {acc[3][e], acc[3][e + 1]}, m4 = {acc[4][e], acc[4][e + 1]};
            f32x2 ya, yb;
            if (half == 0) {
                const f32x2 m0 = {acc[0][e], acc[0][e + 1]};
                const f32x2 d34 = m3 - m4;
                ya = (m0 + (m1 + m2)) + (m3 + m4);
                yb = (m1 - m2) + (d34 + d34);
            } else {
                const f32x2 m5 = {acc[5][e], acc[5][e + 1]};
                const f32x2 d34 = m3 - m4, u = d34 + d34;
                ya = (m1 + m2) + 4.f * (m3 + m4);
                yb = ((m1 - m2) + 4.f * u) + m5;
            }
            const int trow = (e & 3) + 8 * (e >> 2) + 4 * (lane >> 5);
            float* sp = slab + (2 * trow) * EP + (lane & 31);
            sp[0] = ya.x;
            sp[EP] = yb.x;
            sp[2 * EP] = ya.y;
            sp[3 * EP] = yb.y;
        }
    };
    auto finish = [&](int half) {
#pragma unroll
        for (int it = 0; it < 8; ++it) {
            const int prow = pr + 8 * it;
            const float4 v = *reinterpret_cast<const float4*>(&slab[prow * EP + 4 * c4]);
            f32x2 o0 = f32x2{v.x, v.y} * f32x2{sc.x, sc.y} + f32x2{sh.x, sh.y};
            f32x2 o1 = f32x2{v.z, v.w} * f32x2{sc.z, sc.w} + f32x2{sh.z, sh.w};
            if (RES) {
                o0 += f32x2{rs[half][it].x, rs[half][it].y};
                o1 += f32x2{rs[half][it].z, rs[half][it].w};
            }
            const float4 yv = make_float4(fmaxf(o0.x, floor_v), fmaxf(o0.y, floor_v), fmaxf(o1.x, floor_v), fmaxf(o1.y, floor_v));
#ifdef RPG_ABL_NOSTORE
            if (yv.x == 1234.5678f)
#endif
            __builtin_amdgcn_raw_buffer_store_b128(__builtin_bit_cast(u32x4, yv), ro, off(half, it), 0, 0);
        }
    };
    load_res(0);
    transform_to_slab(0);
    __builtin_amdgcn_wave_barrier();
    finish(0);
    load_res(1);
    __builtin_amdgcn_wave_barrier();
    transform_to_slab(1);
    mid();
    __builtin_amdgcn_wave_barrier();
    finish(1);
    __builtin_amdgcn_wave_barrier();
}

template <class Mid>
__device__ __forceinline__ void wino43_epilogue_lean(const f32x16 (&acc)[P], float* slab, int lane, int mw0, int nw0, int M,
                                                     int Tw, int W, int Cout, const Epi& ep, Mid mid) {
    if (ep.residual) wino43_epilogue_lean_body<true>(acc, slab, lane, mw0, nw0, M, Tw, W, Cout, ep, mid);
    else wino43_epilogue_lean_body<false>(acc, slab, lane, mw0, nw0, M, Tw, W, Cout, ep, mid);
}

struct NoMid { __device__ __forceinline__ void operator()() const {} };
template <class Mid = NoMid>
__device__ __forceinline__ void wino43_epilogue_partial(const f32x16 (&acc)[P], float* slab, int lane, int mw, int nw,
                                                        float* __restrict__ dst, Mid mid = Mid()) {
    constexpr int EP = 32 + 4;
    const int c4 = lane & 7, pr = lane >> 3;
    const __amdgpu_buffer_rsrc_t rd = rpg::agent_rsrc(dst);
#pragma unroll
    for (int half = 0; half < 2; ++half) {
#pragma unroll
        for (int e = 0; e < 16; ++e) {
            const float m1 = acc[1][e], m2 = acc[2][e], m3 = acc[3][e], m4 = acc[4][e];
            float ya, yb;
            if (half == 0) {
                ya = acc[0][e] + m1 + m2 + m3 + m4;
                yb = (m1 - m2) + 2.f * (m3 - m4);
            } else {
                ya = (m1 + m2) + 4.f * (m3 + m4);
                yb = (m1 - m2) + 8.f * (m3 - m4) + acc[5][e];
            }
            const int trow = (e & 3) + 8 * (e >> 2) + 4 * (lane >> 5);
            slab[(2 * trow) * EP + (lane & 31)] = ya;
            slab[(2 * trow + 1) * EP + (lane & 31)] = yb;
        }
        if (half == 1) mid();
        __builtin_amdgcn_wave_barrier();
#pragma unroll
        for (int it = 0; it < 8; ++it) {
            const int prow = pr + 8 * it;
            const float4 v = *reinterpret_cast<const float4*>(&slab[prow * EP + 4 * c4]);
            const int px = 4 * (mw + (prow >> 1)) + 2 * half + (prow & 1);
            rpg::agent_store_f4(rd, 4u * (unsigned)(px * BN + nw + 4 * c4), 0, v);
        }
        __builtin_amdgcn_wave_barrier();
    }
}

__global__ __launch_bounds__(NT, 2) void wino43_conv_kernel(const float* __restrict__ x, const float* __restrict__ U,
                                                         int H, int W, int Cin, int Cout, int Tw, int M, Epi ep,
                                                         int tiles_n) {
    extern __shared__ __attribute__((aligned(16))) float lds[];
    float* As = lds;
    float* Bs = lds + A_FLOATS;
    const int K = 3 * Cin;

    const int nwg = gridDim.x, bid = blockIdx.x;
    const int xcd = bid & 7, loc = bid >> 3, q = nwg >> 3, r8 = nwg & 7;
    const int tile = (xcd < r8 ? xcd * (q + 1) : r8 * (q + 1) + (xcd - r8) * q) + loc;
    const int m0 = (tile / tiles_n) * BMT;
    const int n0 = (tile % tiles_n) * BN;

    const int tid = threadIdx.x, lane = tid & 63, wave = tid >> 6;
    const int wm = wave >> 1, wn = wave & 1;
    const int row = tid >> 2, slot = tid & 3;

    const int n_first = (m0 / Tw) / H;
    const size_t img_floats = (size_t)H * W * Cin;
    const __amdgpu_buffer_rsrc_t ra = __builtin_amdgcn_make_buffer_rsrc(
        const_cast<float*>(x + n_first * img_floats) - (size_t)W * Cin, 0, 0x7fffffff, 0x00020000);
    const __amdgpu_buffer_rsrc_t rb = __builtin_amdgcn_make_buffer_rsrc(const_cast<float*>(U), 0, 0x7fffffff, 0x00020000);
    constexpr unsigned OOB = 0x80000000u;
    const int m = m0 + row;
    unsigned va[P];
    unsigned rowbits = 0;
    {
        int img_off = 0, ho = 0, wi0 = -(1 << 24);
        if (m < M) {
            const int tw = m % Tw;
            const int t = m / Tw;
            ho = t % H;
            img_off = (t / H - n_first) * (int)img_floats;
            wi0 = 4 * tw - 1;
            rowbits = (ho > 0 ? 1u : 0u) | 2u | (ho < H - 1 ? 4u : 0u);
        }
#pragma unroll
        for (int j = 0; j < P; ++j) {
            const int wi = wi0 + j;
            va[j] = (unsigned)wi < (unsigned)W ? 4u * (unsigned)(img_off + (ho * W + wi) * Cin + 4 * slot) : OOB;
        }
    }
    const int nrow = n0 + row;
    const unsigned vb = nrow < Cout ? 4u * (unsigned)(nrow * K + 4 * slot) : OOB;
    const unsigned ustride_b = (unsigned)Cout * K * 4u;
    const int nk = 3 * ((Cin + BK - 1) / BK);
    int f_kt = 0, f_kh = 0, f_c0 = 0;

    float4 d[P], ub[P];
    auto fetch_one = [&](int i) {
        const bool cv = f_c0 + 4 * slot < Cin;
        if (i < P) {
            const bool rv = ((rowbits >> f_kh) & 1u) && cv;
            const unsigned sa = 4u * (unsigned)(f_kh * W * Cin + f_c0);
            d[i] = __builtin_bit_cast(float4, __builtin_amdgcn_raw_buffer_load_b128(ra, rv ? va[i] : OOB, sa, 0));
        } else {
            const unsigned vbe = (f_kt < nk && cv) ? vb : OOB;
            const unsigned sb = 4u * (unsigned)(f_kh * Cin + f_c0) + (unsigned)(i - P) * ustride_b;
            ub[i - P] = __builtin_bit_cast(float4, __builtin_amdgcn_raw_buffer_load_b128(rb, vbe, sb, 0));
        }
    };
    auto fetch_next = [&]() {
        ++f_kt;
        f_c0 += BK;
        if (f_c0 >= Cin) { f_c0 = 0; ++f_kh; }
    };
    auto stage = [&]() {
        const float4 t0 = lin(4.f, d[0], -5.f, d[2]);
        const float4 v0 = add(t0, d[4]);
        const float4 s12 = lin(-4.f, d[2], 1.f, d[4]);
        const float4 q12 = lin(4.f, d[1], -1.f, d[3]);
        const float4 v1 = sub(s12, q12);
        const float4 v2 = add(s12, q12);
        const float4 s34 = sub(d[4], d[2]);
        const float4 q34 = lin(2.f, d[3], -2.f, d[1]);
        const float4 v3 = add(s34, q34);
        const float4 v4 = sub(s34, q34);
        const float4 v5 = add(lin(4.f, d[1], -5.f, d[3]), d[5]);
        const int sw = 4 * (slot ^ ((row >> 2) & 3));
        float* ap = As + row * LD + sw;
        *reinterpret_cast<float4*>(ap + 0 * BMT * LD) = v0;
        *reinterpret_cast<float4*>(ap + 1 * BMT * LD) = v1;
        *reinterpret_cast<float4*>(ap + 2 * BMT * LD) = v2;
        *reinterpret_cast<float4*>(ap + 3 * BMT * LD) = v3;
        *reinterpret_cast<float4*>(ap + 4 * BMT * LD) = v4;
        *reinterpret_cast<float4*>(ap + 5 * BMT * LD) = v5;
        float* bp = Bs + row * LD + sw;
#pragma unroll
        for (int xi = 0; xi < P; ++xi) *reinterpret_cast<float4*>(bp + xi * BN * LD) = ub[xi];
    };

    f32x16 acc[P];
#pragma unroll
    for (int xi = 0; xi < P; ++xi)
#pragma unroll
        for (int e = 0; e < 16; ++e) acc[xi][e] = 0.f;

    const int rsw = 4 * ((lane >> 5) ^ ((lane >> 2) & 3));
    const int a_off = (wm * 32 + (lane & 31)) * LD + rsw;
    const int b_off = (wn * 32 + (lane & 31)) * LD + rsw;
#pragma unroll
    for (int i = 0; i < 2 * P; ++i) fetch_one(i);
    fetch_next();
    for (int kt = 0; kt < nk; ++kt) {
        __syncthreads();
        stage();
        __syncthreads();
        float4 fa[2][2], fb[2][2];
        auto frag_one = [&](int g, int set, int i) {
            const int kb = (g / 3) * 8, xi = 2 * (g % 3) + (i >> 1);
            if (i & 1) fb[set][i >> 1] = *reinterpret_cast<const float4*>(&Bs[xi * BN * LD + (b_off ^ kb)]);
            else       fa[set][i >> 1] = *reinterpret_cast<const float4*>(&As[xi * BMT * LD + (a_off ^ kb)]);
        };
#pragma unroll
        for (int i = 0; i < 4; ++i) frag_one(0, 0, i);
        __builtin_amdgcn_sched_barrier(0);
#pragma unroll
        for (int g = 0; g < 6; ++g) {
            const int set = g & 1, x0 = 2 * (g % 3);
#pragma unroll
            for (int i = 0; i < 8; ++i) {
                const int j = i & 1, e = i >> 1;
                const float av = e == 0 ? fa[set][j].x : e == 1 ? fa[set][j].y : e == 2 ? fa[set][j].z : fa[set][j].w;
                const float bv = e == 0 ? fb[set][j].x : e == 1 ? fb[set][j].y : e == 2 ? fb[set][j].z : fb[set][j].w;
                acc[x0 + j] = __builtin_amdgcn_mfma_f32_32x32x2f32(av, bv, acc[x0 + j], 0, 0, 0);
                if (i < 4 && g + 1 < 6) frag_one(g + 1, set ^ 1, i);
                if (i >= 4 && i < 6) fetch_one(2 * g + (i - 4));
                __builtin_amdgcn_sched_barrier(0);
            }
        }
        fetch_next();
    }
    __syncthreads();

    const int ws = __builtin_amdgcn_readfirstlane(wave);
    wino43_epilogue(acc, lds + ws * (64 * 36), lane, m0 + (ws >> 1) * 32, n0 + (ws & 1) * 32, M, Tw, W, Cout, ep);
}

constexpr int NT8 = 512, BMT8 = 128;
constexpr int A8_FLOATS = P * BMT8 * LD, IMG8_FLOATS = A8_FLOATS + B_FLOATS;
constexpr int LDS8_BYTES = 2 * IMG8_FLOATS * (int)sizeof(float);

typedef float f32x2 __attribute__((ext_vector_type(2)));
struct F4 { f32x2 lo, hi; };
__device__ __forceinline__ F4 to_f4(const float4& v) { return F4{f32x2{v.x, v.y}, f32x2{v.z, v.w}}; }
__device__ __forceinline__ float4 to_float4(const F4& v) { return make_float4(v.lo.x, v.lo.y, v.hi.x, v.hi.y); }
#define RPG_PK_FMA(NAME, CONST)                                                                               \
    __device__ __forceinline__ f32x2 NAME(f32x2 x, f32x2 y) {                                                 \
        f32x2 r;                                                                                              \
        asm("v_pk_fma_f32 %0, %1, " CONST ", %2 op_sel_hi:[1,0,1]" : "=v"(r) : "v"(x), "v"(y));               \
        return r;                                                                                             \
    }
RPG_PK_FMA(pk_fma_p4, "4.0")
RPG_PK_FMA(pk_fma_m4, "-4.0")
RPG_PK_FMA(pk_fma_p2, "2.0")
RPG_PK_FMA(pk_fma_m2, "-2.0")
#undef RPG_PK_FMA
__device__ __forceinline__ f32x2 pk_add(f32x2 x, f32x2 y) {
    f32x2 r;
    asm("v_pk_add_f32 %0, %1, %2" : "=v"(r) : "v"(x), "v"(y));
    return r;
}
__device__ __forceinline__ f32x2 pk_sub(f32x2 x, f32x2 y) {
    f32x2 r;
    asm("v_pk_add_f32 %0, %1, %2 neg_lo:[0,1] neg_hi:[0,1]" : "=v"(r) : "v"(x), "v"(y));
    return r;
}
#define RPG_F4_OP(NAME, OP) \
    __device__ __forceinline__ F4 NAME(const F4& x, const F4& y) { return F4{OP(x.lo, y.lo), OP(x.hi, y.hi)}; }
RPG_F4_OP(fma4_p4, pk_fma_p4)
RPG_F4_OP(fma4_m4, pk_fma_m4)
RPG_F4_OP(fma4_p2, pk_fma_p2)
RPG_F4_OP(fma4_m2, pk_fma_m2)
RPG_F4_OP(add4, pk_add)
RPG_F4_OP(sub4, pk_sub)
#undef RPG_F4_OP

struct Split { int tile_base, parts, n_split; float* partial; unsigned* arrive; };

#ifdef RPG_WINO_TRACE
__device__ unsigned long long* g_wino_trace = nullptr;
#define RPG_TRACE(i)                                                                         \
    do {                                                                                     \
        if (g_wino_trace && threadIdx.x == 0) g_wino_trace[5 * blockIdx.x + (i)] = __builtin_readcyclecounter(); \
    } while (0)
#else
#define RPG_TRACE(i) do {} while (0)
#endif

__device__ __forceinline__ void wino43_finish_quad(const float4& s, const Epi& ep, int tile, int p, int c4, int M, int Tw, int W,
                                                   int Cout, int tiles_n) {
    const int m = (tile / tiles_n) * BMT8 + (p >> 2), nb = (tile % tiles_n) * BN + 4 * c4;
    if (m >= M || nb >= Cout) return;
    const int t = m / Tw, wo = 4 * (m - t * Tw) + (p & 3);
    if (wo >= W) return;
    const size_t o = ((size_t)t * W + wo) * Cout + nb;
    float4 sc = make_float4(1.f, 1.f, 1.f, 1.f), sh = f4zero(), rs = f4zero();
    if (ep.scale) sc = *reinterpret_cast<const float4*>(ep.scale + nb);
    if (ep.shift) sh = *reinterpret_cast<const float4*>(ep.shift + nb);
    if (ep.residual) rs = *reinterpret_cast<const float4*>(ep.residual + o);
    float4 y;
    y.x = s.x * sc.x + sh.x + rs.x; y.y = s.y * sc.y + sh.y + rs.y;
    y.z = s.z * sc.z + sh.z + rs.z; y.w = s.w * sc.w + sh.w + rs.w;
    if (ep.relu) { y.x = fmaxf(y.x, 0.f); y.y = fmaxf(y.y, 0.f); y.z = fmaxf(y.z, 0.f); y.w = fmaxf(y.w, 0.f); }
    *reinterpret_cast<float4*>(ep.out + o) = y;
}

__device__ __forceinline__ void wino43_combine_last(const Split& sp, int tt, const Epi& ep, int M, int Tw, int W, int Cout,
                                                    int tiles_n, int* flag) {
    if (!rpg::last_arriver(sp.arrive + tt, (unsigned)sp.parts, flag)) return;
    const __amdgpu_buffer_rsrc_t rs = rpg::agent_rsrc(sp.partial + (size_t)tt * sp.parts * (BMT8 * 4 * BN));
    constexpr unsigned SLAB_B = BMT8 * 4 * BN * 4;
    const int tile = sp.tile_base + tt;
    const int tid_c = threadIdx.x;
#pragma unroll 1
    for (int h = 0; h < 2; ++h) {
        const unsigned vo = 16u * (unsigned)(tid_c + h * 8 * NT8);
        float4 sum[8];
#pragma unroll
        for (int c = 0; c < 8; ++c) sum[c] = rpg::agent_load_f4(rs, vo + 16u * c * NT8, 0);
        for (int i = 1; i < sp.parts; ++i) {
            float4 v[8];
#pragma unroll
            for (int c = 0; c < 8; ++c) v[c] = rpg::agent_load_f4(rs, vo + 16u * c * NT8, (unsigned)i * SLAB_B);
#pragma unroll
            for (int c = 0; c < 8; ++c) { sum[c].x += v[c].x; sum[c].y += v[c].y; sum[c].z += v[c].z; sum[c].w += v[c].w; }
        }
#pragma unroll
        for (int c = 0; c < 8; ++c) {
            const int idx = tid_c + NT8 * (8 * h + c);
            wino43_finish_quad(sum[c], ep, tile, idx >> 4, idx & 15, M, Tw, W, Cout, tiles_n);
        }
    }
}

__global__ __launch_bounds__(NT8) void wino43_conv8_kernel(const float* __restrict__ x, const float* __restrict__ U, int H,
                                                          int W, int Cin, int Cout, int Tw, int M, Epi ep, int tiles_n,
                                                          Split sp) {
    extern __shared__ __attribute__((aligned(16))) float lds[];
#ifdef RPG_WINO_TRACE
    if (g_wino_trace && threadIdx.x == 0) g_wino_trace[5 * blockIdx.x] = __builtin_amdgcn_s_getreg(0xF804);
#endif
    RPG_TRACE(1);
    const int K = 3 * Cin;
    const int kpr = (Cin + BK - 1) / BK;
    int tile, kb = 0, nk = 3 * kpr;
    const bool is_split = (int)blockIdx.x < sp.n_split;
    if (is_split) {
        const int tt = blockIdx.x / sp.parts, part = blockIdx.x - tt * sp.parts;
        tile = sp.tile_base + tt;
        kb = 3 * (part * kpr / sp.parts);
        nk = 3 * ((part + 1) * kpr / sp.parts);
    } else {
        const int nwg = gridDim.x - sp.n_split, bid = blockIdx.x - sp.n_split;
        const int xcd = bid & 7, loc = bid >> 3, q = nwg >> 3, r8 = nwg & 7;
        tile = (xcd < r8 ? xcd * (q + 1) : r8 * (q + 1) + (xcd - r8) * q) + loc;
    }
    const int m0 = (tile / tiles_n) * BMT8;
    const int n0 = (tile % tiles_n) * BN;

    const int tid = threadIdx.x, lane = tid & 63, wave = tid >> 6;
    const int wm = wave >> 1, wn = wave & 1;
    const int row = tid >> 2, slot = tid & 3;
// ... 149 lines not shown
        kstep(0, IMG8_FLOATS, 0);
        kstep(IMG8_FLOATS, 0, 1);
    }
    if (kt < nk) {
        kstep(0, IMG8_FLOATS, 2);
        kstep(IMG8_FLOATS, 0, 0);
        kstep(0, IMG8_FLOATS, 1);
    }
    __syncthreads();
    RPG_TRACE(3);
    const int ws = __builtin_amdgcn_readfirstlane(wave);
    if (is_split) {
        wino43_epilogue_partial(acc, lds + ws * (64 * 36), lane, (ws >> 1) * 32, (ws & 1) * 32,
                                sp.partial + (size_t)blockIdx.x * (BMT8 * 4 * BN));
        if (sp.arrive) wino43_combine_last(sp, tile - sp.tile_base, ep, M, Tw, W, Cout, tiles_n, reinterpret_cast<int*>(lds));
    } else
        wino43_epilogue(acc, lds + ws * (64 * 36), lane, m0 + (ws >> 1) * 32, n0 + (ws & 1) * 32, M, Tw, W, Cout, ep);
#ifdef RPG_WINO_TRACE
    asm volatile("s_waitcnt vmcnt(0)" ::: "memory");
#endif
    RPG_TRACE(4);
}

__global__ __launch_bounds__(NT8) void wino43_conv8p_kernel(const float* __restrict__ x, const float* __restrict__ U, int H,
                                                           int W, int Cin, int Cout, int Tw, int M, Epi ep, int tiles_n,
                                                           Split sp, int n_items) {
    extern __shared__ __attribute__((aligned(16))) float lds[];
#ifdef RPG_ABL_STAGGER
    {
        const unsigned long long t0 = __builtin_readcyclecounter();
        const unsigned long long wait = (unsigned long long)((blockIdx.x >> 3) & 7) * RPG_ABL_STAGGER;
        while (__builtin_readcyclecounter() - t0 < wait) __builtin_amdgcn_s_sleep(8);
    }
#endif
    const int K = 3 * Cin;
    const int kpr = Cin / BK;
    const int tid = threadIdx.x, lane = tid & 63, wave = tid >> 6;
    const int wm = wave >> 1, wn = wave & 1;
    const int row = tid >> 2, slot = tid & 3;
    const int brow = row & 63, bhalf = tid >> 8;
    const size_t img_floats = (size_t)H * W * Cin;
    const __amdgpu_buffer_rsrc_t rb = __builtin_amdgcn_make_buffer_rsrc(const_cast<float*>(U), 0, 0x7fffffff, 0x00020000);
    constexpr unsigned OOB = 0x80000000u;
    const unsigned ustride_b = (unsigned)Cout * K * 4u;
    const unsigned row_b = 4u * (unsigned)(W * Cin), krow_b = 4u * (unsigned)Cin;

    int f_item = blockIdx.x, f_m0 = 0, f_n0 = 0, f_kb = 0, f_nk = 0, f_kt = 0, f_c0 = 0;
    const float* f_base = x;
    unsigned va3[3][P], vb_eff;
    auto decode = [&]() {
        asm volatile("" ::: "memory");
        int tid_d = tid;
        asm volatile("" : "+v"(tid_d));
        const int row = tid_d >> 2, slot = tid_d & 3, brow = row & 63, bhalf = tid_d >> 8;
        const bool valid = f_item < n_items;
        int tile, kb = 0, nk = 3 * kpr;
        if (f_item < sp.n_split) {
            const int tt = f_item / sp.parts, part = f_item - tt * sp.parts;
            tile = sp.tile_base + tt;
            kb = 3 * (part * kpr / sp.parts);
            nk = 3 * ((part + 1) * kpr / sp.parts);
        } else {
            const int nwg = n_items - sp.n_split, bid = f_item - sp.n_split;
            const int xcd = bid & 7, loc = bid >> 3, q = nwg >> 3, r8 = nwg & 7;
            tile = (xcd < r8 ? xcd * (q + 1) : r8 * (q + 1) + (xcd - r8) * q) + loc;
        }
        f_m0 = (tile / tiles_n) * BMT8;
        f_n0 = (tile - (tile / tiles_n) * tiles_n) * BN;
        const int n_first = (f_m0 / Tw) / H;
        f_base = x + n_first * img_floats - (size_t)W * Cin;
        const int m = f_m0 + row;
        int img_off = 0, ho = 0, wi0 = -(1 << 24);
        unsigned rowbits = 0;
        if (valid && m < M) {
            const int t = m / Tw;
            const int tw = m - t * Tw;
            const int n = t / H;
            ho = t - n * H;
            img_off = (n - n_first) * (int)img_floats;
            wi0 = 4 * tw - 1;
            rowbits = (ho > 0 ? 1u : 0u) | 2u | (ho < H - 1 ? 4u : 0u);
        }
#pragma unroll
        for (int j = 0; j < P; ++j) {
            const int wi = wi0 + j;
            const unsigned o = (unsigned)wi < (unsigned)W ? 4u * (unsigned)(img_off + (ho * W + wi) * Cin + 4 * slot) : OOB;
            va3[0][j] = (rowbits & 1u) ? o : OOB;
            va3[1][j] = OOB;
            va3[2][j] = (rowbits & 4u) ? o : OOB;
        }
        vb_eff = valid && f_n0 + brow < Cout ? 4u * (unsigned)((f_n0 + brow) * K + 4 * slot) + 3u * bhalf * ustride_b : OOB;
        f_kb = kb;
        f_kt = kb;
        f_nk = valid ? nk : 0x3fffffff;
        f_c0 = (kb / 3) * BK;
    };
    auto fix_row1 = [&]() {
#pragma unroll
        for (int j = 0; j < P; ++j) va3[1][j] = va3[0][j] < va3[2][j] ? va3[0][j] : va3[2][j];
    };
    decode();
    fix_row1();

    float4 d[P], ub[3];
    auto fetch_one = [&](int i, int kh) {
        if (i < P) {
            const __amdgpu_buffer_rsrc_t ra =
                __builtin_amdgcn_make_buffer_rsrc(const_cast<float*>(f_base), 0, 0x7fffffff, 0x00020000);
            const unsigned sa = (unsigned)kh * row_b + 4u * (unsigned)f_c0;
            d[i] = __builtin_bit_cast(float4, __builtin_amdgcn_raw_buffer_load_b128(ra, va3[kh][i], sa, 0));
        } else {
            const unsigned sb = (unsigned)kh * krow_b + 4u * (unsigned)f_c0 + (unsigned)(i - P) * ustride_b;
            ub[i - P] = __builtin_bit_cast(float4, __builtin_amdgcn_raw_buffer_load_b128(rb, vb_eff, sb, 0));
        }
    };
    auto fetch_next = [&](int kh) {
        ++f_kt;
        if (kh == 2) {
            f_c0 += BK;
            if (f_kt >= f_nk) {
                f_item += gridDim.x;
                decode();
            }
        }
    };

    const int st_a = row * LD + 4 * (slot ^ ((row >> 2) & 3));
    const int st_b = A8_FLOATS + (3 * bhalf) * BN * LD + brow * LD + 4 * (slot ^ ((brow >> 2) & 3));
    struct Img { int a[2], b[2], sa, sb; };
    float4* lds4 = reinterpret_cast<float4*>(lds);
    auto stage_one = [&](int p, const Img& I) {
        if (p >= P) {
            lds4[I.sb + (p - P) * (BN * LD / 4)] = ub[p - P];
            return;
        }
#ifdef RPG_ABL_NOXF
        lds4[I.sa + p * (BMT8 * LD / 4)] = d[p];
        return;
#endif
        const F4 d0 = to_f4(d[0]), d1 = to_f4(d[1]), d2 = to_f4(d[2]), d3 = to_f4(d[3]), d4 = to_f4(d[4]), d5 = to_f4(d[5]);
        F4 v;
        if (p == 0) v = fma4_p4(sub4(d0, d2), sub4(d4, d2));
        else if (p == 5) v = fma4_m4(sub4(d3, d1), sub4(d5, d3));
        else if (p <= 2) {
            const F4 sx = fma4_m4(d2, d4);
            const F4 tx = fma4_m4(d1, d3);
            v = p == 1 ? add4(sx, tx) : sub4(sx, tx);
        } else {
            const F4 r = sub4(d4, d2), t = sub4(d3, d1);
            v = p == 3 ? fma4_p2(t, r) : fma4_m2(t, r);
        }
        lds4[I.sa + p * (BMT8 * LD / 4)] = to_float4(v);
    };

    f32x16 acc[P];
    const int rsw = 4 * ((lane >> 5) ^ ((lane >> 2) & 3));
    const int a_off = (wm * 32 + (lane & 31)) * LD + rsw;
    const int b_off = A8_FLOATS + (wn * 32 + (lane & 31)) * LD + rsw;
    float4 fa[2][2], fb[2][2];
    constexpr int IMG4 = IMG8_FLOATS / 4;
    Img X{{a_off >> 2, (a_off ^ 8) >> 2}, {b_off >> 2, (b_off ^ 8) >> 2}, st_a >> 2, st_b >> 2};
    Img Y{{X.a[0] + IMG4, X.a[1] + IMG4}, {X.b[0] + IMG4, X.b[1] + IMG4}, X.sa + IMG4, X.sb + IMG4};
    int ybase = IMG8_FLOATS;
    auto frag_one = [&](int g, int set, int i, const Img& I) {
        const int xi = 2 * (g % 3) + (i >> 1);
        if (i & 1) fb[set][i >> 1] = lds4[I.b[g / 3] + xi * (BN * LD / 4)];
        else       fa[set][i >> 1] = lds4[I.a[g / 3] + xi * (BMT8 * LD / 4)];
    };
    auto kstep = [&](const Img& cur, const Img& nxt, int khf) {
        __builtin_amdgcn_sched_barrier(0);
#pragma unroll
        for (int g = 0; g < 6; ++g) {
            const int set = g & 1, x0 = 2 * (g % 3);
#pragma unroll
            for (int i = 0; i < 8; ++i) {
                const int j = i & 1, e = i >> 1;
                const float av = e == 0 ? fa[set][j].x : e == 1 ? fa[set][j].y : e == 2 ? fa[set][j].z : fa[set][j].w;
                const float bv = e == 0 ? fb[set][j].x : e == 1 ? fb[set][j].y : e == 2 ? fb[set][j].z : fb[set][j].w;
                acc[x0 + j] = __builtin_amdgcn_mfma_f32_32x32x2f32(av, bv, acc[x0 + j], 0, 0, 0);
                if (i < 4) {
                    if (g < 5) frag_one(g + 1, set ^ 1, i, cur);
                    else frag_one(0, 0, i, nxt);
                } else {
                    const int s = 4 * (g % 3) + (i - 4);
                    if (s < 9) {
                        if (g < 3) stage_one(s, nxt);
                        else fetch_one(s, khf);
                    }
                }
                __builtin_amdgcn_sched_barrier(0);
            }
#ifndef RPG_ABL_NOBAR
            if (g == 4) {
                __syncthreads();
                __builtin_amdgcn_sched_barrier(0);
            }
#endif
        }
        fetch_next(khf);
    };

    int c_item = f_item, c_m0 = f_m0, c_n0 = f_n0, c_ns = f_nk - f_kb;
#pragma unroll
    for (int i = 0; i < 9; ++i) fetch_one(i, 0);
    fetch_next(0);
#pragma unroll
    for (int p = 0; p < 9; ++p) stage_one(p, X);
#pragma unroll
    for (int i = 0; i < 9; ++i) fetch_one(i, 1);
    fetch_next(1);
    const int ws = __builtin_amdgcn_readfirstlane(wave);
    for (;;) {
#ifdef RPG_WINO_TRACE
        if (g_wino_trace && threadIdx.x == 0) {
            g_wino_trace[5 * c_item] = __builtin_amdgcn_s_getreg(0xF804);
            g_wino_trace[5 * c_item + 1] = __builtin_readcyclecounter();
        }
#endif
#pragma unroll
        for (int xi = 0; xi < P; ++xi)
#pragma unroll
            for (int e = 0; e < 16; ++e) acc[xi][e] = 0.f;
        __syncthreads();
#pragma unroll
        for (int i = 0; i < 4; ++i) frag_one(0, 0, i, X);
#ifdef RPG_WINO_TRACE
        if (g_wino_trace && threadIdx.x == 0) g_wino_trace[5 * c_item + 2] = __builtin_readcyclecounter();
#endif
        int s = 0;
        for (; s + 6 <= c_ns; s += 6) {
            kstep(X, Y, 2);
            kstep(Y, X, 0);
            kstep(X, Y, 1);
            kstep(Y, X, 2);
            kstep(X, Y, 0);
            kstep(Y, X, 1);
        }
        if (s < c_ns) {
            kstep(X, Y, 2);
            kstep(Y, X, 0);
            kstep(X, Y, 1);
            const Img t = X;
            X = Y;
            Y = t;
            ybase = IMG8_FLOATS - ybase;
        }
        __syncthreads();
        float* slab = lds + ybase + ws * (64 * 36);
#ifdef RPG_WINO_TRACE
        if (g_wino_trace && threadIdx.x == 0) g_wino_trace[5 * c_item + 3] = __builtin_readcyclecounter();
#endif
        auto refetch = [&]() {
            fix_row1();
#pragma unroll
            for (int i = 0; i < 9; ++i) fetch_one(i, 1);
        };
        int lane_e = lane;
        asm volatile("" : "+v"(lane_e));
        if (c_item < sp.n_split)
            wino43_epilogue_partial(acc, slab, lane_e, (ws >> 1) * 32, (ws & 1) * 32,
                                    sp.partial + (size_t)c_item * (BMT8 * 4 * BN), refetch);
        else
            wino43_epilogue_lean(acc, slab, lane_e, c_m0 + (ws >> 1) * 32, c_n0 + (ws & 1) * 32, M, Tw, W, Cout, ep, refetch);
#ifdef RPG_WINO_TRACE
        if (g_wino_trace && threadIdx.x == 0) g_wino_trace[5 * c_item + 4] = __builtin_readcyclecounter();
#endif
        if (f_item >= n_items) break;
        c_item = f_item;
        c_m0 = f_m0;
        c_n0 = f_n0;
        c_ns = f_nk - f_kb;
    }
}

__global__ __launch_bounds__(256) void wino43_fixup_kernel(const float* __restrict__ partial, Epi ep, int M, int Tw, int W,
                                                           int Cout, int tiles_n, Split sp) {
    const int tt = blockIdx.x >> 5, idx = (blockIdx.x & 31) * 256 + threadIdx.x;
    const float* src = partial + (size_t)tt * sp.parts * (BMT8 * 4 * BN) + 4 * idx;
    float4 s = *reinterpret_cast<const float4*>(src);
    for (int i = 1; i < sp.parts; ++i) {
        const float4 v = *reinterpret_cast<const float4*>(src + (size_t)i * (BMT8 * 4 * BN));
        s.x += v.x; s.y += v.y; s.z += v.z; s.w += v.w;
    }
    wino43_finish_quad(s, ep, sp.tile_base + tt, idx >> 4, idx & 15, M, Tw, W, Cout, tiles_n);
}

__global__ __launch_bounds__(NT) void wino43_weights_kernel(const float* __restrict__ w, float* __restrict__ U, int Cout,
                                                            int Cin, long total) {
    const long i = (long)blockIdx.x * NT + threadIdx.x;
    if (i >= total) return;
    const int c = (int)(i % Cin);
    const long t = i / Cin;
    const int kh = (int)(t % 3);
    const long co = t / 3;
    const float* wp = w + ((co * 3 + kh) * 3) * (long)Cin + c;
    const double g0 = wp[0], g1 = wp[Cin], g2 = wp[2 * (long)Cin];
    const double u[6] = {g0 / 4.0, -(g0 + g1 + g2) / 6.0, -(g0 - g1 + g2) / 6.0,
                         g0 / 24.0 + g1 / 12.0 + g2 / 6.0, g0 / 24.0 - g1 / 12.0 + g2 / 6.0, g2};
    const long plane = (long)Cout * 3 * Cin;
#pragma unroll
    for (int xi = 0; xi < 6; ++xi) U[xi * plane + i] = (float)u[xi];
}

int g_wino_split = 1;
int g_wino_split_steps = 3;
int g_wino = 1;
int g_wino_min_blocks = 16;
int g_wino_persist = 1;
int g_wino_combine_max = 8;

}

#ifdef RPG_PROBE_WINO2D
#include "../../tools/probes/winograd2d.hip"
#endif

namespace rpg {

#ifndef RPG_PROBE_WINO2D
void wino2d_set(int) {}
#endif
bool wino_enabled() { return g_wino != 0; }
void wino_set(int on) { if (on >= 16) { g_wino = 1; g_wino_min_blocks = on; } else { g_wino = on; g_wino_min_blocks = 16; } }
void wino_split_set(int v) { g_wino_split = v != 0; g_wino_split_steps = v >= 2 ? v : 3; }
void wino_short_set(int) {}
void wino_persist_set(int on) { g_wino_persist = on; }
void wino_combine_max_set(int v) { g_wino_combine_max = v; }

bool wino_pays(int n, int h, int w, int cin, int cout) {
    if (!g_wino || (cin & 3) || (cout & 3)) return false;
    const long tiles = (long)n * h * ((w + 3) / 4);
    const long blocks = ((tiles + BMT - 1) / BMT) * ((cout + BN - 1) / BN);
    const int tw = (w + 3) / 4;
    return blocks >= g_wino_min_blocks && (long)h * w * cin * 4 * 67 < (1L << 31) && 6L * cout * 3 * cin * 4 < (1L << 31) &&
           (32L / tw + 3) * w * cout * 4 < (1L << 31);
}

int launch_conv_wino(const float* x, const float* u, const float* scale, const float* shift, const float* residual,
                     float* y, int n, int h, int w, int cin, int cout, int relu, hipStream_t s) {
    if (!x || !u || !y || n <= 0 || h <= 0 || w <= 0 || cin <= 0 || cout <= 0 || (cin & 3) || (cout & 3) ||
        !aligned16(x) || !aligned16(u) || !aligned16(y) || (scale && !aligned16(scale)) || (shift && !aligned16(shift)) ||
        (residual && !aligned16(residual)))
        return RPG_ERR_BAD_ARG;
#ifdef RPG_PROBE_WINO2D
    if (wino2d_takes(n, h, w, cin, cout))
        return launch_conv_wino2d(x, u + (size_t)18 * cout * cin, scale, shift, residual, y, n, h, w, cin, cout, relu, s);
#endif
    const int tw = (w + 3) / 4;
    const long M = (long)n * h * tw;
    if (M >= (1L << 31) || (long)h * w * cin * 4 * 67 >= (1L << 31) || 6L * cout * 3 * cin * 4 >= (1L << 31) ||
        (32L / tw + 3) * w * cout * 4 >= (1L << 31))
        return RPG_ERR_BAD_ARG;
    int dev = 0;
    if (hipGetDevice(&dev) != hipSuccess || dev < 0 || dev >= 64) dev = 0;
    static bool attr[64] = {};
    if (!attr[dev]) {
        (void)hipFuncSetAttribute(reinterpret_cast<const void*>(wino43_conv_kernel),
                                  hipFuncAttributeMaxDynamicSharedMemorySize, LDS_BYTES);
        attr[dev] = true;
    }
    const int tn = (cout + BN - 1) / BN;
    Epi ep{scale, shift, residual, y, relu};
    const int slot = timing_begin(RPG_TIMER_CONV_WINO, s);
    double executed = 0.0;
    const long tm8 = (M + BMT8 - 1) / BMT8;
    const bool fits8 = (long)h * w * cin * 4 * 131 < (1L << 31);
    if (fits8 && (g_wino == 3 || (g_wino == 1 && tm8 * tn >= 8))) {
        static bool attr8[64] = {};
        if (!attr8[dev]) {
            (void)hipFuncSetAttribute(reinterpret_cast<const void*>(wino43_conv8_kernel),
                                      hipFuncAttributeMaxDynamicSharedMemorySize, LDS8_BYTES);
            attr8[dev] = true;
        }
        const long T = tm8 * tn;
        const int S = num_cus(), kpr = (cin + BK - 1) / BK, nk = 3 * kpr;
        executed = (double)T * nk * 48.0 * 8.0 * 4096.0;
        long t_main = T;
        Split sp{0, 1, 0, nullptr, nullptr};
        const long tail = T % S;
        if (g_wino_persist && cin % BK == 0 && (T > S || g_wino_persist == 2) && h >= 2) {
            static bool attr8p[64] = {};
            if (!attr8p[dev]) {
                (void)hipFuncSetAttribute(reinterpret_cast<const void*>(wino43_conv8p_kernel),
                                          hipFuncAttributeMaxDynamicSharedMemorySize, LDS8_BYTES);
                attr8p[dev] = true;
            }
            if (g_wino_split && tail > 0) {
                int parts = (int)(S / tail);
                if (parts > kpr) parts = kpr;
                if (parts >= 2) {
                    sp.partial = stream_scratch(s, (size_t)tail * parts * (BMT8 * 4 * BN) * sizeof(float));
                    if (sp.partial) { sp.parts = parts; t_main = T - tail; sp.tile_base = (int)t_main; sp.n_split = (int)(tail * parts); }
                }
            }
            const long items = sp.n_split + t_main;
            hipLaunchKernelGGL(wino43_conv8p_kernel, dim3((unsigned)(items < S ? items : S)), dim3(NT8), LDS8_BYTES, s, x, u, h, w,
                               cin, cout, tw, (int)M, ep, tn, sp, (int)items);
            if (sp.n_split) {
                hipStream_t fs = fixup_hop_begin(s);
                hipLaunchKernelGGL(wino43_fixup_kernel, dim3((unsigned)(T - t_main) * 32), dim3(256), 0, fs, sp.partial, ep, (int)M,
                                   tw, w, cout, tn, sp);
                fixup_hop_end(s, fs);
            }
            timing_end(slot, 2.0 * (double)n * h * w * cout * 9.0 * cin, s, executed);
            RPG_CHECK_LAUNCH("conv3x3_wino43");
            return RPG_OK;
        }
        if (g_wino_split && tail > 0) {
            int parts = (int)(S / tail);
            if (parts > kpr) parts = kpr;
            if (parts > nk / g_wino_split_steps && nk / g_wino_split_steps >= 2) parts = nk / g_wino_split_steps;
            if (parts >= 2) {
                unsigned* counters = nullptr;
                sp.partial = stream_scratch(s, (size_t)tail * parts * (BMT8 * 4 * BN) * sizeof(float), &counters);
                if (sp.partial) { sp.parts = parts; t_main = T - tail; sp.tile_base = (int)t_main; sp.n_split = (int)(tail * parts); }
                if (sp.partial && inkernel_fixup_enabled() && parts <= g_wino_combine_max) sp.arrive = counters;
            }
        }
        hipLaunchKernelGGL(wino43_conv8_kernel, dim3((unsigned)(sp.n_split + t_main)), dim3(NT8), LDS8_BYTES, s, x, u, h, w, cin,
                           cout, tw, (int)M, ep, tn, sp);
        if (sp.n_split && !sp.arrive) {
            hipStream_t fs = fixup_hop_begin(s);
            hipLaunchKernelGGL(wino43_fixup_kernel, dim3((unsigned)(T - t_main) * 32), dim3(256), 0, fs, sp.partial, ep, (int)M, tw, w,
                               cout, tn, sp);
            fixup_hop_end(s, fs);
        }
    } else {
        const int tm = (int)((M + BMT - 1) / BMT);
        executed = (double)tm * tn * (3 * ((cin + BK - 1) / BK)) * 48.0 * 4.0 * 4096.0;
        hipLaunchKernelGGL(wino43_conv_kernel, dim3(tm * tn), dim3(NT), LDS_BYTES, s, x, u, h, w, cin, cout, tw, (int)M, ep, tn);
    }
    timing_end(slot, 2.0 * (double)n * h * w * cout * 9.0 * cin, s, executed);
    RPG_CHECK_LAUNCH("conv3x3_wino43");
    return RPG_OK;
}

}

#ifdef RPG_WINO_TRACE
extern "C" int rpg_wino_trace_set(unsigned long long* buf) {
    return hipMemcpyToSymbol(HIP_SYMBOL(g_wino_trace), &buf, sizeof(buf)) == hipSuccess ? RPG_OK : RPG_ERR_LAUNCH;
}
#endif

extern "C" size_t rpg_wino43_weights_floats(int cout, int cin) {
    if (cout <= 0 || cin <= 0) return 0;
#ifdef RPG_PROBE_WINO2D
    return rpg::wino_weight_floats(cout, cin);
#else
    return (size_t)18 * cout * cin;
#endif
}

extern "C" int rpg_wino43_transform_weights_f32(const float* w_ohwi, float* u, int cout, int cin, void* stream) {
    if (!w_ohwi || !u || cout <= 0 || cin <= 0) return RPG_ERR_BAD_ARG;
    const long total = (long)cout * 3 * cin;
    hipLaunchKernelGGL(wino43_weights_kernel, dim3((unsigned)((total + NT - 1) / NT)), dim3(NT), 0, rpg::as_stream(stream),
                       w_ohwi, u, cout, cin, total);
    RPG_CHECK_LAUNCH("wino43_transform_weights");
#ifdef RPG_PROBE_WINO2D
    return rpg::launch_wino2d_weights(w_ohwi, u + (size_t)18 * cout * cin, cout, cin, rpg::as_stream(stream));
#else
    return RPG_OK;
#endif
}

extern "C" int rpg_conv3x3_wino43_bn_act_nhwc_f32(const float* x, const float* u, const float* scale, const float* shift,
                                                  const float* residual, float* y, int n, int h, int w, int cin, int cout,
                                                  int relu, void* stream) {
    return rpg::launch_conv_wino(x, u, scale, shift, residual, y, n, h, w, cin, cout, relu, rpg::as_stream(stream));
}
```

relpose-gnn_amd/ops.py:

```python
from __future__ import annotations

import ctypes as C
from typing import Dict, Optional, Sequence, Tuple

import torch

from . import _lib as L


def _stream() -> int:
    return torch.cuda.current_stream().cuda_stream


def _req(t: torch.Tensor, name: str, dtype=torch.float32) -> torch.Tensor:
    if not torch.is_tensor(t):
        raise TypeError(f"{name}: expected a tensor")
    if not t.is_cuda:
        raise RuntimeError(f"{name}: expected a tensor on the GPU (the HIP kernels are the only compute path), got {t.device}")
    if t.dtype != dtype:
        raise TypeError(f"{name}: expected {dtype}, got {t.dtype}")
    return t if t.is_contiguous() else t.contiguous()


def _p(t: Optional[torch.Tensor]) -> Optional[int]:
# ... 61 lines not shown
    for name, t in (("scale", scale), ("shift", shift)):
        if t is not None and t.numel() != cout:
            raise ValueError(f"{name} must have Cout = {cout} elements, got {t.numel()}")
    if residual is not None and tuple(residual.shape) != (n, h, w, cout):
        raise ValueError("residual shape mismatch")
    L.check(L.lib().rpg_conv3x3_wino43_bn_act_nhwc_f32(_p(x), _p(u), _p(scale), _p(shift), _p(residual), _p(y), n, h, w, cin,
                                                        cout, int(relu), _stream()), "conv3x3_wino43_bn_act_nhwc")
    return y


def conv2d_bn_act_nhwc_bf16(x: torch.Tensor, w_ohwi: torch.Tensor, scale: Optional[torch.Tensor], shift: Optional[torch.Tensor],
                            residual: Optional[torch.Tensor] = None, stride: int = 1, pad: int = 0, relu: bool = False,
                            out_f32: bool = False) -> torch.Tensor:
    x, w_ohwi = _req(x, "x", torch.bfloat16), _req(w_ohwi, "w_ohwi", torch.bfloat16)
    n, h, w, cin = x.shape
    cout, kh, kw, cin_w = w_ohwi.shape
    if cin_w != cin:
        raise ValueError(f"channel mismatch: x has {cin}, weight has {cin_w}")
    ho, wo = (h + 2 * pad - kh) // stride + 1, (w + 2 * pad - kw) // stride + 1
    y = torch.empty((n, ho, wo, cout), dtype=torch.float32 if out_f32 else torch.bfloat16, device=x.device)
    scale = None if scale is None else _req(scale, "scale")
    shift = None if shift is None else _req(shift, "shift")
    residual = None if residual is None else _req(residual, "residual", torch.bfloat16)
    L.check(L.lib().rpg_conv2d_bn_act_nhwc_bf16(_p(x), _p(w_ohwi), _p(scale), _p(shift), _p(residual), _p(y), n, h, w, cin,
                                                 cout, kh, kw, stride, pad, int(relu), int(out_f32), _stream()),
            "conv2d_bn_act_nhwc_bf16")
    return y


def basicblock64_bf16(x: torch.Tensor, w1_ohwi: torch.Tensor, scale1: torch.Tensor, shift1: torch.Tensor, w2_ohwi: torch.Tensor,
                      scale2: torch.Tensor, shift2: torch.Tensor) -> torch.Tensor:
    x = _req(x, "x", torch.bfloat16)
    w1_ohwi, w2_ohwi = _req(w1_ohwi, "w1_ohwi", torch.bfloat16), _req(w2_ohwi, "w2_ohwi", torch.bfloat16)
    n, h, w, c = x.shape
    if c != 64 or tuple(w1_ohwi.shape) != (64, 3, 3, 64) or tuple(w2_ohwi.shape) != (64, 3, 3, 64):
        raise ValueError("basicblock64_bf16: x [n,h,w,64], weights [64,3,3,64]")
    ps = [_req(t, nm) for t, nm in ((scale1, "scale1"), (shift1, "shift1"), (scale2, "scale2"), (shift2, "shift2"))]
    if any(t.numel() != 64 for t in ps):
        raise ValueError("basicblock64_bf16: scale / shift must have 64 elements")
    y = torch.empty_like(x)
    L.check(L.lib().rpg_basicblock64_bf16(_p(x), _p(w1_ohwi), _p(ps[0]), _p(ps[1]), _p(w2_ohwi), _p(ps[2]), _p(ps[3]), _p(y), n, h, w,
                                          _stream()), "basicblock64_bf16")
    return y


def probe_mfma_bf16(data: str = "relu_like", iters: int = 20000, workgroups: int = 0, device=None) -> float:
    dev = torch.device("cuda", torch.cuda.current_device()) if device is None else torch.device(device)
    g = torch.Generator(device=dev).manual_seed(17)
    n = 65536 * 8
    if data == "zeros":
        v = torch.zeros(n, device=dev)
    elif data == "random":
        v = (torch.rand(n, generator=g, device=dev) - 0.5) * 2e-3
    elif data == "relu_like":
        v = torch.rand(n, generator=g, device=dev) * 2e-3 * (torch.rand(n, generator=g, device=dev) < 0.5)
    else:
        raise ValueError("data: zeros | random | relu_like")
    src = v.bfloat16().contiguous()
    sink = torch.zeros(1, device=dev)
    wgs = workgroups or 2 * torch.cuda.get_device_properties(dev).multi_processor_count
    lib = L.lib()
    L.check(lib.rpg_probe_mfma_bf16(_p(src), max(1, iters // 10), wgs, _p(sink), _stream()), "probe_mfma_bf16")
    e0, e1 = torch.cuda.Event(enable_timing=True), torch.cuda.Event(enable_timing=True)
    e0.record()
    L.check(lib.rpg_probe_mfma_bf16(_p(src), iters, wgs, _p(sink), _stream()), "probe_mfma_bf16")
    e1.record()
    e1.synchronize()
    return wgs * 8 * iters * 16 * 32768.0 / (e0.elapsed_time(e1) * 1e-3) / 1e15


def f32_to_bf16(x: torch.Tensor, out: Optional[torch.Tensor] = None, col_off: int = 0) -> torch.Tensor:
    x = _req(x, "x")
    rows, cols = x.shape
    if out is None:
        out = torch.empty((rows, cols), dtype=torch.bfloat16, device=x.device)
    out = _req(out, "out", torch.bfloat16)
    L.check(L.lib().rpg_f32_to_bf16(_p(x), cols, _p(out), out.shape[1], col_off, rows, cols, _stream()), "f32_to_bf16")
    return out


def linear_bf16(a: torch.Tensor, weight: torch.Tensor, bias: Optional[torch.Tensor] = None,
                residual: Optional[torch.Tensor] = None, res_idx: Optional[torch.Tensor] = None,
                residual2: Optional[torch.Tensor] = None, res2_idx: Optional[torch.Tensor] = None, relu: bool = False) -> torch.Tensor:
    a, weight = _req(a, "a", torch.bfloat16), _req(weight, "weight", torch.bfloat16)
    m, k = a.shape
    n_out = weight.shape[0]
    if weight.shape[1] != k:
        raise ValueError("a.shape[1] != weight.shape[1]")
    bias = None if bias is None else _req(bias, "bias")
    residual = None if residual is None else _req(residual, "residual")
    residual2 = None if residual2 is None else _req(residual2, "residual2")
    res_idx = None if res_idx is None else _req(res_idx, "res_idx", torch.int64)
    res2_idx = None if res2_idx is None else _req(res2_idx, "res2_idx", torch.int64)
    if residual2 is not None and (residual is None or residual2.shape[1] != residual.shape[1]):
        raise ValueError("residual2 needs residual with the same row pitch")
    ldr = 0 if residual is None else residual.shape[1]
    out = torch.empty((m, n_out), dtype=torch.float32, device=a.device)
    L.check(L.lib().rpg_linear_bf16(_p(a), _p(weight), _p(bias), _p(residual), _p(res_idx), _p(residual2), _p(res2_idx), ldr,
                                    _p(out), m, k, n_out, int(relu), _stream()), "linear_bf16")
    return out


def stem_conv_bn_relu_maxpool(x_nchw: torch.Tensor, wpack: torch.Tensor, shift: torch.Tensor) -> torch.Tensor:
    x, wpack, shift = _req(x_nchw, "x_nchw"), _req(wpack, "wpack"), _req(shift, "shift")
    n, c, h, w = x.shape
    if c != 3 or wpack.numel() != (74 + 75) * 2 * 64 or shift.numel() != 64:
        raise ValueError("expected x [N,3,H,W], wpack from params.pack_stem_pairs (19,072 floats), shift [64]")
    hc, wc = (h - 1) // 2 + 1, (w - 1) // 2 + 1
    y = torch.empty((n, (hc - 1) // 2 + 1, (wc - 1) // 2 + 1, 64), dtype=torch.float32, device=x.device)
    L.check(L.lib().rpg_stem_conv7x7s2_bn_relu_maxpool_f32(_p(x), _p(wpack), _p(shift), _p(y), n, h, w, _stream()),
            "stem_conv_bn_relu_maxpool")
    return y


def stem_conv_bn_relu_maxpool_bf16(x_nchw: torch.Tensor, wpack_bf16: torch.Tensor, scale: torch.Tensor, shift: torch.Tensor) -> torch.Tensor:
    xbf = x_nchw.dtype == torch.bfloat16
    x_nchw, scale, shift = _req(x_nchw, "x_nchw", torch.bfloat16 if xbf else torch.float32), _req(scale, "scale"), _req(shift, "shift")
    wpack_bf16 = _req(wpack_bf16, "wpack_bf16", torch.bfloat16)
    n, c, h, w = x_nchw.shape
    if c != 3 or wpack_bf16.numel() != (11 * 2 + 2 * 3 * 4) * 64 * 8 or scale.numel() != 64 or shift.numel() != 64:
        raise ValueError("expected x [N,3,H,W], wpack_bf16 from params.pack_stem_bf16 (23,552 bf16), scale / shift [64]")
    hc, wc = (h - 1) // 2 + 1, (w - 1) // 2 + 1
    hp, wp = (hc - 1) // 2 + 1, (wc - 1) // 2 + 1
    y = torch.empty((n, hp, wp, 64), dtype=torch.bfloat16, device=x_nchw.device)
    fn = L.lib().rpg_stem_conv7x7s2_bn_relu_maxpool_bf16_xbf16 if xbf else L.lib().rpg_stem_conv7x7s2_bn_relu_maxpool_bf16
    L.check(fn(_p(x_nchw), _p(wpack_bf16), _p(scale), _p(shift), _p(y), n, h, w, _stream()), "stem_conv_bn_relu_maxpool_bf16")
    return y


def maxpool3x3s2_nhwc(x: torch.Tensor) -> torch.Tensor:
    x = _req(x, "x")
    n, h, w, c = x.shape
    y = torch.empty((n, (h - 1) // 2 + 1, (w - 1) // 2 + 1, c), dtype=torch.float32, device=x.device)
    L.check(L.lib().rpg_maxpool3x3s2_nhwc_f32(_p(x), _p(y), n, h, w, c, _stream()), "maxpool3x3s2_nhwc")
    return y


def global_avgpool_nhwc(x: torch.Tensor) -> torch.Tensor:
    x = _req(x, "x")
    n, h, w, c = x.shape
    y = torch.empty((n, c), dtype=torch.float32, device=x.device)
    L.check(L.lib().rpg_global_avgpool_nhwc_f32(_p(x), _p(y), n, h * w, c, _stream()), "global_avgpool_nhwc")
    return y


def graph_prepare(edge_index: torch.Tensor, n: int) -> Dict[str, torch.Tensor]:
    ei = _req(edge_index, "edge_index", torch.int64)
    if ei.dim() != 2 or ei.shape[0] != 2:
        raise ValueError("edge_index must be [2, E]")
    e = ei.shape[1]
    dev = ei.device
    ends = torch.empty((4, e), dtype=torch.int64, device=dev)
    rowptr = torch.empty(n + 1, dtype=torch.int32, device=dev)
    cursor = torch.empty(n, dtype=torch.int32, device=dev)
    perm = torch.empty(e, dtype=torch.int32, device=dev)
    status = torch.zeros(1, dtype=torch.int32, device=dev)
    L.check(L.lib().rpg_graph_prepare(ei.data_ptr(), ei.data_ptr() + 8 * e, 0, e, n, _p(ends), _p(rowptr), _p(cursor), _p(perm),
                                      _p(status), _stream()), "graph_prepare")
    return {"ends": ends, "rowptr": rowptr, "perm": perm, "status": status}


def knn_graph_launch(x: torch.Tensor, k: int, batch: Optional[torch.Tensor] = None) -> Tuple[torch.Tensor, torch.Tensor]:
    x = _req(x, "x")
    n, d = x.shape
    batch = None if batch is None else _req(batch, "batch", torch.int64)
    cap = n * (k + 1)
    ei = torch.empty((2, cap), dtype=torch.int64, device=x.device)
    cand = torch.empty((n, k + 1), dtype=torch.int32, device=x.device)
    cnt = torch.empty(n, dtype=torch.int32, device=x.device)
    meta = torch.zeros(2, dtype=torch.int32, device=x.device)
    L.check(L.lib().rpg_knn_graph_f32(_p(x), _p(batch), n, d, k, _p(ei), _p(cand), _p(cnt), meta.data_ptr(),
                                      meta.data_ptr() + 4, _stream()), "knn_graph")
    return ei, meta


def knn_graph(x: torch.Tensor, k: int, batch: Optional[torch.Tensor] = None) -> torch.Tensor:
    ei, meta = knn_graph_launch(x, k, batch)
    total, bad = (int(v) for v in meta.tolist())
    if bad:
        raise ValueError("knn_graph: a graph has more than 2048 nodes (unsupported)")
    return ei[:, :total].contiguous()


def edge_concat_gather(x: torch.Tensor, edge_index: torch.Tensor) -> torch.Tensor:
    x, ei = _req(x, "x"), _req(edge_index, "edge_index", torch.int64)
    e, d = ei.shape[1], x.shape[1]
    out = torch.empty((e, 2 * d), dtype=torch.float32, device=x.device)
    L.check(L.lib().rpg_edge_concat_gather_f32(_p(x), _p(ei), e, d, _p(out), _stream()), "edge_concat_gather")
    return out


def linear_gather(sources: Sequence[Tuple[torch.Tensor, Optional[torch.Tensor]]], weight: torch.Tensor,
                  bias: Optional[torch.Tensor], m: int, residual: Optional[torch.Tensor] = None, relu: bool = False) -> torch.Tensor:
    ns = len(sources)
    keep = [(_req(a, f"a{i}"), None if ix is None else _req(ix, f"idx{i}", torch.int64)) for i, (a, ix) in enumerate(sources)]
    weight = _req(weight, "weight")
    bias = None if bias is None else _req(bias, "bias")
    residual = None if residual is None else _req(residual, "residual")
    n_out = weight.shape[0]
    if sum(a.shape[1] for a, _ in keep) != weight.shape[1]:
        raise ValueError("sum of source widths != weight.shape[1]")
    out = torch.empty((m, n_out), dtype=torch.float32, device=weight.device)
    a_arr = L.ptr_array([a.data_ptr() for a, _ in keep])
    i_arr = L.ptr_array([None if ix is None else ix.data_ptr() for _, ix in keep])
    ld = L.int_array([a.shape[1] for a, _ in keep])
    wd = L.int_array([a.shape[1] for a, _ in keep])
    L.check(L.lib().rpg_linear_gather_f32(ns, a_arr, i_arr, ld, wd, _p(weight), _p(bias), _p(residual), _p(out), m, n_out,
                                           int(relu), _stream()), "linear_gather")
    return out


def linear_gather_ex(sources: Sequence[Tuple[torch.Tensor, Optional[torch.Tensor]]], weight: torch.Tensor, bias: Optional[torch.Tensor],
                     m: int, residual: Optional[torch.Tensor] = None, res_idx: Optional[torch.Tensor] = None,
                     residual2: Optional[torch.Tensor] = None, res2_idx: Optional[torch.Tensor] = None, relu: bool = False,
                     want_relu_copy: bool = False, widths: Optional[Sequence[int]] = None):
    ns = len(sources)
    keep = [(_req(a, f"a{i}"), None if ix is None else _req(ix, f"idx{i}", torch.int64)) for i, (a, ix) in enumerate(sources)]
    wd_l = [a.shape[1] for a, _ in keep] if widths is None else [int(v) for v in widths]
    if len(wd_l) != ns or any(w <= 0 or w > a.shape[1] for w, (a, _) in zip(wd_l, keep)):
        raise ValueError("widths: one positive entry per source, at most the source's row pitch")
    weight = _req(weight, "weight")
    bias = None if bias is None else _req(bias, "bias")
    residual = None if residual is None else _req(residual, "residual")
    residual2 = None if residual2 is None else _req(residual2, "residual2")
    res_idx = None if res_idx is None else _req(res_idx, "res_idx", torch.int64)
    res2_idx = None if res2_idx is None else _req(res2_idx, "res2_idx", torch.int64)
    n_out = weight.shape[0]
    if sum(wd_l) != weight.shape[1]:
        raise ValueError("sum of source widths != weight.shape[1]")
    for r_, i_ in ((residual, res_idx), (residual2, res2_idx)):
        if r_ is not None and (r_.shape[1] < n_out or (i_ is None and r_.shape[0] != m) or (i_ is not None and i_.numel() != m)):
            raise ValueError("residual: [rows][>= n_out] with one (gathered) row per output row")
    if residual is not None and residual2 is not None and residual.shape[1] != residual2.shape[1]:
        raise ValueError("residual and residual2 share one row pitch")
    out = torch.empty((m, n_out), dtype=torch.float32, device=weight.device)
    out_relu = torch.empty_like(out) if want_relu_copy else None
    a_arr = L.ptr_array([a.data_ptr() for a, _ in keep])
    i_arr = L.ptr_array([None if ix is None else ix.data_ptr() for _, ix in keep])
    ld = L.int_array([a.shape[1] for a, _ in keep])
    wd = L.int_array(wd_l)
    import ctypes as C
    rows = (C.c_long * ns)(*[a.shape[0] if ix is not None else 0 for a, ix in keep])
    L.check(L.lib().rpg_linear_gather_ex_f32(ns, a_arr, i_arr, ld, wd, rows, _p(weight), _p(bias), _p(residual), _p(res_idx), _p(residual2),
                                              _p(res2_idx), 0 if residual is None else residual.shape[1], _p(out), _p(out_relu), m, n_out,
                                              int(relu), _stream()), "linear_gather_ex")
    return (out, out_relu) if want_relu_copy else out


def attention_rows(gtp: torch.Tensor) -> torch.Tensor:
    gtp = _req(gtp, "gtp")
    r, c3 = gtp.shape
    c = c3 // 3
    y = torch.empty((r, c), dtype=torch.float32, device=gtp.device)
    L.check(L.lib().rpg_attention_rows_f32(_p(gtp), r, c, _p(y), _stream()), "attention_rows")
    return y


def scatter_mean(msg: torch.Tensor, rowptr: torch.Tensor, perm: torch.Tensor, n: int) -> torch.Tensor:
    msg = _req(msg, "msg")
    rowptr, perm = _req(rowptr, "rowptr", torch.int32), _req(perm, "perm", torch.int32)
    e, d = msg.shape
    out = torch.empty((n, d), dtype=torch.float32, device=msg.device)
    L.check(L.lib().rpg_scatter_mean_f32(_p(msg), _p(rowptr), _p(perm), n, e, d, _p(out), _stream()), "scatter_mean")
    return out


def attention_aggregate(gtp: torch.Tensor, msg: torch.Tensor, rowptr: torch.Tensor, perm: torch.Tensor, n: int,
                        bias: Optional[torch.Tensor] = None) -> Tuple[torch.Tensor, torch.Tensor]:
    gtp, msg = _req(gtp, "gtp"), _req(msg, "msg")
    rowptr, perm = _req(rowptr, "rowptr", torch.int32), _req(perm, "perm", torch.int32)
    bias = None if bias is None else _req(bias, "bias")
    e, c3 = gtp.shape
    c, d = c3 // 3, msg.shape[1]
    ybar = torch.empty((n, c), dtype=torch.float32, device=gtp.device)
    mbar = torch.empty((n, d), dtype=torch.float32, device=gtp.device)
    L.check(L.lib().rpg_attention_aggregate_f32(_p(gtp), _p(msg), _p(rowptr), _p(perm), _p(bias), n, e, c, d, _p(ybar), _p(mbar),
                                                _stream()), "attention_aggregate")
    return ybar, mbar


def pose_heads(x: torch.Tensor, w6: torch.Tensor, b6: torch.Tensor, out: Optional[torch.Tensor] = None) -> torch.Tensor:
    x, w6, b6 = _req(x, "x"), _req(w6, "w6"), _req(b6, "b6")
    r, d = x.shape
    if out is None:
        out = torch.empty((r, 6), dtype=torch.float32, device=x.device)
    elif tuple(out.shape) != (r, 6) or out.dtype != torch.float32 or not out.is_contiguous() or out.device != x.device:
        raise ValueError("pose_heads: out must be a contiguous fp32 [rows, 6] tensor on x's device")
    L.check(L.lib().rpg_pose_heads_f32(_p(x), _p(w6), _p(b6), r, d, _p(out), _stream()), "pose_heads")
    return out


def timing_enable(on: bool) -> None:
    L.check(L.lib().rpg_timing_enable(int(on)), "timing_enable")


def timing_read() -> Dict[str, Dict[str, float]]:
    n = len(L.TIMER_NAMES)
    ms, cnt, work, ex = (C.c_double * n)(), (C.c_longlong * n)(), (C.c_double * n)(), (C.c_double * n)()
    L.check(L.lib().rpg_timing_read_ex(ms, cnt, work, ex), "timing_read")
    return {name: {"ms": ms[i], "launches": int(cnt[i]), "work": work[i], "executed": ex[i]}
            for i, name in enumerate(L.TIMER_NAMES)}


def release_scratch() -> None:
    L.check(L.lib().rpg_release_scratch(), "release_scratch")


TUNE_TILE, TUNE_BK, TUNE_EPILOGUE, TUNE_STREAMK, TUNE_WINOGRAD, TUNE_GNN_SPLIT, TUNE_BF16_BK, TUNE_FAST_LOADER, TUNE_WINO_SPLIT, TUNE_BF16_FAST, TUNE_FUSED_STEM, TUNE_WAVES8, TUNE_WINO_SHORT, TUNE_GNN_FUSE_AGG, TUNE_WINO_PERSIST, TUNE_BF16_TILE, TUNE_BF16_DMA, TUNE_BF16_PATCH, TUNE_BF16_WS64, TUNE_SK_MIN_ITS, TUNE_INKERNEL_FIXUP, TUNE_BF16_CHUNK, TUNE_WINO2D, TUNE_BF16_LEAN_EPI, TUNE_BF16_LINEAR_DMA, TUNE_BF16_PERSIST, TUNE_FOLD_K, TUNE_BF16_FUSE_BLOCK, TUNE_BF16_TAIL, TUNE_LIN112, TUNE_FIXUP_PRIO, TUNE_BF16_PAIR = 0, 1, 2, 3, 4, 5, 6, 7, 8, 9, 10, 11, 12, 13, 14, 15, 16, 17, 18, 19, 20, 21, 22, 23, 24, 25, 26, 27, 28, 29, 30, 31


def set_tuning(key: int, value: int) -> None:
    L.check(L.lib().rpg_set_tuning(key, value), "set_tuning")
```

Measured before the change: 3038 graphs/s.

## Chain ResNet layer1/layer2 Winograd convs in one persistent dependency-tracked kernel

Adds a persistent Winograd F(4,3) chain kernel that runs up to seven consecutive 3x3 convs of a ResNet stage in one launch. Tiles of conv k+1 spin-wait on per-tile done flags from conv k instead of waiting at kernel boundaries. The aim is to remove per-conv launch gaps and tail idling, so the next conv starts while the previous one drains. This costs extra activation buffers and a zeroed flag area, and relies on spin-waits with a timeout error path that could stall or deadlock if residency assumptions fail.

```diff
diff --git a/include/relpose_gnn_hip.h b/include/relpose_gnn_hip.h
--- a/include/relpose_gnn_hip.h
+++ b/include/relpose_gnn_hip.h
@@ -12,6 +12,7 @@
 #define RPG_ERR_BAD_ARG (-1)
 #define RPG_ERR_LAUNCH (-2)
 #define RPG_ERR_WORKSPACE (-3)
+#define RPG_ERR_CHAIN_WAIT (-4)
 
 #define RPG_ABI_VERSION 1
 
@@ -32,6 +33,11 @@
 int rpg_conv3x3_wino43_bn_act_nhwc_f32(const float* x, const float* u, const float* scale, const float* shift,
                                        const float* residual, float* y, int n, int h, int w, int cin, int cout,
                                        int relu, void* stream);
+
+size_t rpg_wino43_chain_ctl_bytes(int n_conv, int n, int h, int w, int c);
+int rpg_wino43_chain_f32(const float* const* convs, const int* relu, int n_conv, int n, int h, int w, int c, void* ctl,
+                         size_t ctl_bytes, void* stream);
+int rpg_wino43_chain_error(int reset);
 
 int rpg_stem_conv7x7s2_bn_relu_maxpool_f32(const float* x_nchw, const float* wpack, const float* shift, float* y_nhwc,
                                            int n, int h, int w, void* stream);
@@ -158,6 +164,7 @@
 #define RPG_TUNE_LIN112 29
 #define RPG_TUNE_FIXUP_PRIO 30
 #define RPG_TUNE_BF16_PAIR 31
+#define RPG_TUNE_WINO_CHAIN 32
 int rpg_set_tuning(int key, int value);
 
 #ifdef __cplusplus
diff --git a/relpose-gnn_amd/_lib.py b/relpose-gnn_amd/_lib.py
--- a/relpose-gnn_amd/_lib.py
+++ b/relpose-gnn_amd/_lib.py
@@ -7,7 +7,7 @@
 HERE = os.path.dirname(os.path.abspath(__file__))
 LIB_PATH = os.environ.get("RPG_HIP_LIB") or os.path.join(HERE, "lib", "librelpose_gnn_hip.so")
 
-RPG_OK, RPG_ERR_BAD_ARG, RPG_ERR_LAUNCH, RPG_ERR_WORKSPACE = 0, -1, -2, -3
+RPG_OK, RPG_ERR_BAD_ARG, RPG_ERR_LAUNCH, RPG_ERR_WORKSPACE, RPG_ERR_CHAIN_WAIT = 0, -1, -2, -3, -4
 TIMER_NAMES = ("conv", "linear", "scatter", "attention", "conv_wino", "att_agg")
 
 SYMBOLS = (
@@ -21,6 +21,7 @@
     "rpg_release_scratch", "rpg_timing_read_ex", "rpg_stem_conv7x7s2_bn_relu_maxpool_f32", "rpg_stem_pair_table",
     "rpg_attention_aggregate_f32", "rpg_stem_conv7x7s2_bn_relu_maxpool_bf16", "rpg_stem_conv7x7s2_bn_relu_maxpool_bf16_xbf16",
     "rpg_resnet_forward_bf16_xbf16", "rpg_host_f32_to_bf16", "rpg_basicblock64_bf16", "rpg_linear_gather_ex_f32", "rpg_probe_mfma_bf16", "rpg_host_f32_to_bf16_isa",
+    "rpg_wino43_chain_ctl_bytes", "rpg_wino43_chain_f32", "rpg_wino43_chain_error",
 )
 
 
@@ -77,6 +78,10 @@
     lib.rpg_wino43_weights_floats.argtypes = [_i, _i]
     lib.rpg_wino43_weights_floats.restype = C.c_size_t
     lib.rpg_conv3x3_wino43_bn_act_nhwc_f32.argtypes = [_vp] * 6 + [_i] * 6 + [_vp]
+    lib.rpg_wino43_chain_ctl_bytes.argtypes = [_i] * 5
+    lib.rpg_wino43_chain_ctl_bytes.restype = _sz
+    lib.rpg_wino43_chain_f32.argtypes = [C.POINTER(_vp), C.POINTER(_i), _i, _i, _i, _i, _i, _vp, _sz, _vp]
+    lib.rpg_wino43_chain_error.argtypes = [_i]
     lib.rpg_knn_graph_f32.argtypes = [_vp, _vp, _i, _i, _i, _vp, _vp, _vp, _vp, _vp, _vp]
     lib.rpg_timing_read.argtypes = [C.POINTER(C.c_double), C.POINTER(C.c_longlong), C.POINTER(C.c_double)]
     lib.rpg_timing_read_ex.argtypes = [C.POINTER(C.c_double), C.POINTER(C.c_longlong), C.POINTER(C.c_double),
@@ -124,6 +129,8 @@
         raise ValueError(f"{what}: bad argument (null pointer, non-positive size, unsupported shape or alignment)")
     if rc == RPG_ERR_WORKSPACE:
         raise RpgError(f"{what}: workspace too small")
+    if rc == RPG_ERR_CHAIN_WAIT:
+        raise RpgError(f"{what}: a chain launch gave up waiting for a dependency")
     msg = lib().rpg_last_error().decode(errors="replace")
     raise RpgError(f"{what}: HIP launch failed: {msg}")
 
diff --git a/relpose-gnn_amd/build.py b/relpose-gnn_amd/build.py
--- a/relpose-gnn_amd/build.py
+++ b/relpose-gnn_amd/build.py
@@ -11,7 +11,7 @@
 LIB_PATH = os.path.join(LIB_DIR, "librelpose_gnn_hip.so")
 SOURCES = ("gemm_f32.hip", "winograd.hip", "stem.hip", "stem_bf16.hip", "conv_bf16.hip", "encoder_ops.hip", "gnn_ops.hip", "forward.hip", "timing.hip", "host_ops.hip")
 ARCH = "gfx950"
-WINOGRAD_SOURCES = ("winograd.hip", "rpg_coherent.h")
+WINOGRAD_SOURCES = ("winograd.hip", "wino_chain.inc", "rpg_coherent.h")
 
 
 def _hipcc() -> str:
diff --git a/relpose-gnn_amd/csrc/forward.hip b/relpose-gnn_amd/csrc/forward.hip
--- a/relpose-gnn_amd/csrc/forward.hip
+++ b/relpose-gnn_amd/csrc/forward.hip
@@ -22,9 +22,14 @@
     }
 };
 
+constexpr int kChainConvs = 7;
+constexpr int kChainSlots[2] = {kChainConvs - 3, kChainConvs - 2};
+
 struct ResnetPlan {
     int h1, w1, h2, w2;
     size_t in4, stem, blk, pool, total_bytes;
+    size_t chain_act[2];
+    size_t chain_bytes, ctl_bytes;
 };
 
 ResnetPlan plan_resnet(int n, int h, int w, const int* planes) {
@@ -42,8 +47,21 @@
     }
     p.blk = blk;
     p.pool = (size_t)n * planes[3];
+    p.chain_bytes = p.ctl_bytes = 0;
+    hh = p.h2; ww = p.w2;
+    for (int l = 0; l < 2; ++l) {
+        if (l > 0) { hh = conv_out(hh, 3, 2, 1); ww = conv_out(ww, 3, 2, 1); }
+        p.chain_act[l] = 0;
+        if (!rpg::wino_chain_fits(n, hh, ww, planes[l])) continue;
+        p.chain_act[l] = (size_t)n * hh * ww * planes[l];
+        const size_t bytes = kChainSlots[l] * (align_up(p.chain_act[l] * 4, 256) + rpg::kWorkspaceSkew);
+        if (bytes > p.chain_bytes) p.chain_bytes = bytes;
+        const size_t ctl = rpg::wino_chain_ctl_bytes(kChainConvs, n, hh, ww, planes[l]);
+        if (ctl > p.ctl_bytes) p.ctl_bytes = ctl;
+    }
     p.total_bytes = align_up(p.in4 * 4, 256) + align_up(p.stem * 4, 256) + 4 * align_up(p.blk * 4, 256) +
                     align_up(p.pool * 4, 256) + align_up(rpg::split_scratch_bytes(), 256) + 8 * rpg::kWorkspaceSkew;
+    if (p.chain_bytes) p.total_bytes += p.chain_bytes + 2 * align_up(p.ctl_bytes, 256) + rpg::kWorkspaceSkew;
     return p;
 }
 
@@ -80,7 +98,11 @@
     for (int i = 0; i < 4; ++i) buf[i] = cv.take<float>(p.blk);
     float* pool = cv.take<float>(p.pool);
     const size_t scratch_bytes = rpg::split_scratch_bytes();
-    rpg::ScratchScope scratch(cv.take<char>(scratch_bytes), scratch_bytes, s);
+    const size_t ctl_total = p.chain_bytes ? 2 * align_up(p.ctl_bytes, 256) : 0;
+    char* ctl_and_scratch = cv.take<char>(ctl_total + scratch_bytes);
+    rpg::ScratchScope scratch(ctl_and_scratch + ctl_total, scratch_bytes, s, ctl_total);
+    char* chain_base = p.chain_bytes ? cv.take<char>(p.chain_bytes) : nullptr;
+    const bool chain_ctl_zeroed = ctl_total && scratch.lead_zeroed();
 
     int rc;
     int ti = 0;
@@ -98,6 +120,63 @@
     int cur = 0, hh = p.h2, ww = p.w2;
     cin = planes[0];
     for (int l = 0; l < 4; ++l) {
+        if (l < 2 && p.chain_act[l] && chain_ctl_zeroed && blocks[l] >= 1) {
+            const int nb = blocks[l], c = planes[l];
+            const int stride0 = l > 0 ? 2 : 1;
+            const bool ds0 = stride0 != 1 || cin != c;
+            const int ho = conv_out(hh, 3, stride0, 1), wo = conv_out(ww, 3, stride0, 1);
+            const int n_conv = ds0 ? 2 * nb - 1 : 2 * nb;
+            bool ok = n_conv <= kChainConvs && rpg::wino_chain_takes(n, ho, wo, c) && (size_t)n * ho * wo * c <= p.chain_act[l] &&
+                      (l > 0 ? ds0 : !ds0);
+            for (int b = 0, t = ti; ok && b < nb; t += (b == 0 && ds0) ? 12 : 8, ++b)
+                ok = (b > 0 || !ds0 ? tensors[t + 3] != nullptr : true) && tensors[t + 7] != nullptr;
+            if (ok) {
+                float* X = buf[cur];
+                float* T = buf[(cur + 1) & 3];
+                float* D = buf[(cur + 3) & 3];
+                const int fin = (cur + 2 * nb) & 3;
+                rpg::WinoChainConv chain[kChainConvs];
+                int k = 0, t = ti;
+                const float* prev = X;
+                if (ds0) {
+                    if ((rc = rpg::launch_conv(X, tensors[t], tensors[t + 1], tensors[t + 2], nullptr, T, n, hh, ww, cin, c, 3, 3,
+                                               stride0, 1, 1, s)) != RPG_OK)
+                        return rc;
+                    if ((rc = rpg::launch_conv(X, tensors[t + 8], tensors[t + 9], tensors[t + 10], nullptr, D, n, hh, ww, cin, c, 1,
+                                               1, stride0, 0, 0, s)) != RPG_OK)
+                        return rc;
+                    chain[k++] = rpg::WinoChainConv{T, tensors[t + 7], tensors[t + 5], tensors[t + 6], D, nullptr, 1};
+                    prev = T;
+                    t += 12;
+                }
+                for (int b = ds0 ? 1 : 0; b < nb; ++b, t += 8) {
+                    chain[k++] = rpg::WinoChainConv{prev, tensors[t + 3], tensors[t + 1], tensors[t + 2], nullptr, nullptr, 1};
+                    chain[k++] = rpg::WinoChainConv{nullptr, tensors[t + 7], tensors[t + 5], tensors[t + 6], nullptr, nullptr, 1};
+                }
+                float* pool_bufs[4 + kChainSlots[1]];
+                int np = 0;
+                for (int i = 1; i <= 4; ++i) {
+                    float* bi = buf[(cur + i) & 3];
+                    const bool read = bi == chain[0].x || (ds0 ? bi == D : bi == X);
+                    if (!read && bi != buf[fin]) pool_bufs[np++] = bi;
+                }
+                for (int i = 0; i < kChainSlots[l]; ++i)
+                    pool_bufs[np++] = reinterpret_cast<float*>(chain_base + i * (align_up(p.chain_act[l] * 4, 256) + rpg::kWorkspaceSkew));
+                if (np < n_conv - 1) return RPG_ERR_WORKSPACE;
+                for (int i = 0; i < n_conv; ++i) {
+                    chain[i].y = i + 1 < n_conv ? pool_bufs[i] : buf[fin];
+                    if (i + 1 < n_conv) chain[i + 1].x = chain[i].y;
+                }
+                for (int i = ds0 ? 2 : 1; i < n_conv; i += 2) chain[i].residual = i >= 2 ? chain[i - 2].y : X;
+                if ((rc = rpg::launch_wino_chain(chain, n_conv, n, ho, wo, c, ctl_and_scratch + l * align_up(p.ctl_bytes, 256),
+                                                 p.ctl_bytes, s, true)) != RPG_OK)
+                    return rc;
+                ti = t;
+                cur = fin;
+                hh = ho; ww = wo; cin = c;
+                continue;
+            }
+        }
         for (int b = 0; b < blocks[l]; ++b) {
             const int stride = (l > 0 && b == 0) ? 2 : 1;
             const int c = planes[l];
diff --git a/relpose-gnn_amd/csrc/gemm_f32.hip b/relpose-gnn_amd/csrc/gemm_f32.hip
--- a/relpose-gnn_amd/csrc/gemm_f32.hip
+++ b/relpose-gnn_amd/csrc/gemm_f32.hip
@@ -519,8 +519,17 @@
 hipStream_t fixup_hop_begin(hipStream_t s) { return fixup_hop_begin_impl(s); }
 void fixup_hop_end(hipStream_t s, hipStream_t used) { fixup_hop_end_impl(s, used); }
 bool inkernel_fixup_enabled() { return (g_inkernel_fixup & 2) != 0; }
-ScratchScope::ScratchScope(void* p, size_t bytes, hipStream_t s) {
-    if (p && bytes >= kCounterBytes && hipMemsetAsync(p, 0, kCounterBytes, s) != hipSuccess) { (void)hipGetLastError(); p = nullptr; bytes = 0; }
+ScratchScope::ScratchScope(void* p, size_t bytes, hipStream_t s, size_t zero_before) {
+    lead_zeroed_ = false;
+    if (p && bytes >= kCounterBytes) {
+        if (hipMemsetAsync(static_cast<char*>(p) - zero_before, 0, zero_before + kCounterBytes, s) != hipSuccess) {
+            (void)hipGetLastError();
+            p = nullptr;
+            bytes = 0;
+        } else {
+            lead_zeroed_ = true;
+        }
+    }
     t_scratch.p = static_cast<float*>(p);
     t_scratch.bytes = p ? bytes : 0;
     t_scratch.on = true;
@@ -657,6 +666,7 @@
 
 extern "C" int rpg_set_tuning(int key, int value) {
     switch (key) {
+        case RPG_TUNE_WINO_CHAIN: if (value < 0 || value > 1) return RPG_ERR_BAD_ARG; rpg::wino_chain_set(value); return RPG_OK;
         case RPG_TUNE_FIXUP_PRIO: g_fixup_prio = value != 0; return RPG_OK;
         case RPG_TUNE_BF16_PAIR: rpg::bf16_set_pair(value != 0); return RPG_OK;
         case RPG_TUNE_TILE: g_force_tile = value; return RPG_OK;
diff --git a/relpose-gnn_amd/csrc/rpg_common.h b/relpose-gnn_amd/csrc/rpg_common.h
--- a/relpose-gnn_amd/csrc/rpg_common.h
+++ b/relpose-gnn_amd/csrc/rpg_common.h
@@ -49,8 +49,10 @@
 void fixup_hop_end(hipStream_t s, hipStream_t used);
 bool inkernel_fixup_enabled();
 struct ScratchScope {
-    ScratchScope(void* p, size_t bytes, hipStream_t s);
+    ScratchScope(void* p, size_t bytes, hipStream_t s, size_t zero_before = 0);
     ~ScratchScope();
+    bool lead_zeroed() const { return lead_zeroed_; }
+    bool lead_zeroed_;
     ScratchScope(const ScratchScope&) = delete;
     ScratchScope& operator=(const ScratchScope&) = delete;
 };
@@ -59,6 +61,21 @@
 bool wino_enabled();
 bool wino_pays(int n, int h, int w, int cin, int cout);
 void wino_set(int on);
+struct WinoChainConv {
+    const float* x;
+    const float* u;
+    const float* scale;
+    const float* shift;
+    const float* residual;
+    float* y;
+    int relu;
+};
+void wino_chain_set(int on);
+bool wino_chain_fits(int n, int h, int w, int c);
+bool wino_chain_takes(int n, int h, int w, int c);
+size_t wino_chain_ctl_bytes(int n_conv, int n, int h, int w, int c);
+int launch_wino_chain(const WinoChainConv* convs, int n_conv, int n, int h, int w, int c, void* ctl, size_t ctl_bytes, hipStream_t s,
+                      bool ctl_zeroed = false);
 void wino2d_set(int v);
 size_t wino_weight_floats(int cout, int cin);
 int launch_wino2d_weights(const float* w_ohwi, float* u2, int cout, int cin, hipStream_t s);
diff --git a/relpose-gnn_amd/csrc/wino_chain.inc b/relpose-gnn_amd/csrc/wino_chain.inc
--- /dev/null
+++ b/relpose-gnn_amd/csrc/wino_chain.inc
@@ -0,0 +1,290 @@
+constexpr int kChainMax = 7;
+constexpr unsigned kChainCtlHead = 64;
+constexpr unsigned long long kChainSpinTicks = 20000000ull;
+constexpr int kChainLdsExtra = 64;
+
+struct ChainConv {
+    const float* x;
+    const float* u;
+    const float* scale;
+    const float* shift;
+    const float* residual;
+    float* out;
+    int relu;
+};
+struct Chain { ChainConv c[kChainMax]; };
+
+__device__ unsigned g_chain_error = 0;
+
+__device__ __forceinline__ unsigned chain_flag_load(const unsigned* p) {
+    return __hip_atomic_load(p, __ATOMIC_RELAXED, __HIP_MEMORY_SCOPE_AGENT);
+}
+
+__device__ __forceinline__ bool chain_deps_done(const unsigned* done, int item, int ipc, int tiles_n, int Tw, int M) {
+    const int k = item / ipc;
+    if (k == 0) return true;
+    const int i = item - k * ipc, mt = i / tiles_n, rows = M / Tw;
+    const int last_tile = min(mt * BMT8 + BMT8 - 1, M - 1);
+    const int a = max(mt * BMT8 / Tw - 1, 0), b = min(last_tile / Tw + 1, rows - 1);
+    const int lo = (a * Tw) / BMT8 * tiles_n, hi = min(((b + 1) * Tw - 1) / BMT8 * tiles_n + tiles_n, ipc);
+    const unsigned* f = done + (size_t)(k - 1) * ipc;
+    bool ok = true;
+    for (int j = lo; j < hi; ++j) ok = ok && chain_flag_load(f + j) != 0u;
+    return ok;
+}
+
+__global__ __launch_bounds__(NT8) void wino43_chain_kernel(Chain ch, int H, int W, int C, int Tw, int M, int tiles_n, int ipc,
+                                                          int n_items, unsigned* ctl) {
+    extern __shared__ __attribute__((aligned(16))) float lds[];
+    int* lds_i = reinterpret_cast<int*>(lds + 2 * IMG8_FLOATS);
+    unsigned* const ticket = ctl;
+    unsigned* const err = ctl + 1;
+    unsigned* const done = ctl + kChainCtlHead;
+    const int K = 3 * C;
+    const int kpr = C / BK;
+    const int tid = threadIdx.x, lane = tid & 63, wave = tid >> 6;
+    const int wm = wave >> 1, wn = wave & 1;
+    const int row = tid >> 2, slot = tid & 3;
+    const int brow = row & 63, bhalf = tid >> 8;
+    const size_t img_floats = (size_t)H * W * C;
+    constexpr unsigned OOB = 0x80000000u;
+    const unsigned ustride_b = (unsigned)C * K * 4u;
+    const unsigned row_b = 4u * (unsigned)(W * C), krow_b = 4u * (unsigned)C;
+
+    auto wait_deps = [&](int item) -> bool {
+        if (tid == 0) {
+            int ok = 1;
+            if (item < n_items) {
+                const unsigned long long t0 = __builtin_amdgcn_s_memrealtime();
+                while (!chain_deps_done(done, item, ipc, tiles_n, Tw, M)) {
+                    if (chain_flag_load(err) != 0u || __builtin_amdgcn_s_memrealtime() - t0 > kChainSpinTicks) {
+                        __hip_atomic_store(err, 1u, __ATOMIC_RELAXED, __HIP_MEMORY_SCOPE_AGENT);
+                        __hip_atomic_store(&g_chain_error, 1u, __ATOMIC_RELAXED, __HIP_MEMORY_SCOPE_AGENT);
+                        ok = 0;
+                        break;
+                    }
+                    __builtin_amdgcn_s_sleep(8);
+                }
+            }
+            lds_i[1] = ok;
+        }
+        __syncthreads();
+        return __builtin_amdgcn_readfirstlane(lds_i[1]) != 0;
+    };
+
+    int f_item = 0, f_k = 0, f_m0 = 0, f_n0 = 0, f_kb = 0, f_nk = 0, f_kt = 0, f_c0 = 0;
+    const float* f_base = ch.c[0].x;
+    const float* f_u = ch.c[0].u;
+    unsigned va3[3][P], vb_eff;
+    auto decode = [&](bool poll) {
+        asm volatile("" ::: "memory");
+        int tid_d = tid;
+        asm volatile("" : "+v"(tid_d));
+        const int row = tid_d >> 2, slot = tid_d & 3, brow = row & 63, bhalf = tid_d >> 8;
+        const bool valid = f_item < n_items;
+        bool ready = true;
+        if (poll && valid) {
+            ready = __builtin_amdgcn_readfirstlane((int)chain_deps_done(done, f_item, ipc, tiles_n, Tw, M)) != 0;
+            if ((tid_d & 63) == 0) lds_i[8 + (tid_d >> 6)] = ready ? 1 : 0;
+        }
+        const bool use = valid && ready;
+        f_k = valid ? f_item / ipc : 0;
+        const int i = f_item - f_k * ipc;
+        f_m0 = (i / tiles_n) * BMT8;
+        f_n0 = (i - (i / tiles_n) * tiles_n) * BN;
+        f_base = ch.c[f_k].x;
+        f_u = ch.c[f_k].u;
+        const int n_first = (f_m0 / Tw) / H;
+        f_base = f_base + n_first * img_floats - (size_t)W * C;
+        const int m = f_m0 + row;
+        int img_off = 0, ho = 0, wi0 = -(1 << 24);
+        unsigned rowbits = 0;
+        if (use && m < M) {
+            const int t = m / Tw;
+            const int tw = m - t * Tw;
+            const int n = t / H;
+            ho = t - n * H;
+            img_off = (n - n_first) * (int)img_floats;
+            wi0 = 4 * tw - 1;
+            rowbits = (ho > 0 ? 1u : 0u) | 2u | (ho < H - 1 ? 4u : 0u);
+        }
+#pragma unroll
+        for (int j = 0; j < P; ++j) {
+            const int wi = wi0 + j;
+            const unsigned o = (unsigned)wi < (unsigned)W ? 4u * (unsigned)(img_off + (ho * W + wi) * C + 4 * slot) : OOB;
+            va3[0][j] = (rowbits & 1u) ? o : OOB;
+            va3[1][j] = OOB;
+            va3[2][j] = (rowbits & 4u) ? o : OOB;
+        }
+        vb_eff = use && f_n0 + brow < C ? 4u * (unsigned)((f_n0 + brow) * K + 4 * slot) + 3u * bhalf * ustride_b : OOB;
+        f_kb = 0;
+        f_kt = 0;
+        f_nk = valid ? 3 * kpr : 0x3fffffff;
+        f_c0 = 0;
+    };
+    auto fix_row1 = [&]() {
+#pragma unroll
+        for (int j = 0; j < P; ++j) va3[1][j] = va3[0][j] < va3[2][j] ? va3[0][j] : va3[2][j];
+    };
+
+    float4 d[P], ub[3];
+    auto fetch_one = [&](int i, int kh) {
+        if (i < P) {
+            const __amdgpu_buffer_rsrc_t ra =
+                __builtin_amdgcn_make_buffer_rsrc(const_cast<float*>(f_base), 0, 0x7fffffff, 0x00020000);
+            const unsigned sa = (unsigned)kh * row_b + 4u * (unsigned)f_c0;
+            d[i] = __builtin_bit_cast(float4, __builtin_amdgcn_raw_buffer_load_b128(ra, va3[kh][i], sa, 0));
+        } else {
+            const __amdgpu_buffer_rsrc_t rb = __builtin_amdgcn_make_buffer_rsrc(const_cast<float*>(f_u), 0, 0x7fffffff, 0x00020000);
+            const unsigned sb = (unsigned)kh * krow_b + 4u * (unsigned)f_c0 + (unsigned)(i - P) * ustride_b;
+            ub[i - P] = __builtin_bit_cast(float4, __builtin_amdgcn_raw_buffer_load_b128(rb, vb_eff, sb, 0));
+        }
+    };
+    auto fetch_next = [&](int kh) {
+        ++f_kt;
+        if (kh == 2) {
+            f_c0 += BK;
+            if (f_kt >= f_nk) {
+                f_item = __builtin_amdgcn_readfirstlane(lds_i[0]);
+                decode(true);
+            }
+        }
+    };
+
+    const int st_a = row * LD + 4 * (slot ^ ((row >> 2) & 3));
+    const int st_b = A8_FLOATS + (3 * bhalf) * BN * LD + brow * LD + 4 * (slot ^ ((brow >> 2) & 3));
+    struct Img { int a[2], b[2], sa, sb; };
+    float4* lds4 = reinterpret_cast<float4*>(lds);
+    auto stage_one = [&](int p, const Img& I) {
+        if (p >= P) {
+            lds4[I.sb + (p - P) * (BN * LD / 4)] = ub[p - P];
+            return;
+        }
+        const F4 d0 = to_f4(d[0]), d1 = to_f4(d[1]), d2 = to_f4(d[2]), d3 = to_f4(d[3]), d4 = to_f4(d[4]), d5 = to_f4(d[5]);
+        F4 v;
+        if (p == 0) v = fma4_p4(sub4(d0, d2), sub4(d4, d2));
+        else if (p == 5) v = fma4_m4(sub4(d3, d1), sub4(d5, d3));
+        else if (p <= 2) {
+            const F4 sx = fma4_m4(d2, d4);
+            const F4 tx = fma4_m4(d1, d3);
+            v = p == 1 ? add4(sx, tx) : sub4(sx, tx);
+        } else {
+            const F4 r = sub4(d4, d2), t = sub4(d3, d1);
+            v = p == 3 ? fma4_p2(t, r) : fma4_m2(t, r);
+        }
+        lds4[I.sa + p * (BMT8 * LD / 4)] = to_float4(v);
+    };
+
+    f32x16 acc[P];
+    const int rsw = 4 * ((lane >> 5) ^ ((lane >> 2) & 3));
+    const int a_off = (wm * 32 + (lane & 31)) * LD + rsw;
+    const int b_off = A8_FLOATS + (wn * 32 + (lane & 31)) * LD + rsw;
+    float4 fa[2][2], fb[2][2];
+    constexpr int IMG4 = IMG8_FLOATS / 4;
+    const Img X{{a_off >> 2, (a_off ^ 8) >> 2}, {b_off >> 2, (b_off ^ 8) >> 2}, st_a >> 2, st_b >> 2};
+    const Img Y{{X.a[0] + IMG4, X.a[1] + IMG4}, {X.b[0] + IMG4, X.b[1] + IMG4}, X.sa + IMG4, X.sb + IMG4};
+    auto frag_one = [&](int g, int set, int i, const Img& I) {
+        const int xi = 2 * (g % 3) + (i >> 1);
+        if (i & 1) fb[set][i >> 1] = lds4[I.b[g / 3] + xi * (BN * LD / 4)];
+        else       fa[set][i >> 1] = lds4[I.a[g / 3] + xi * (BMT8 * LD / 4)];
+    };
+    auto kstep = [&](const Img& cur, const Img& nxt, int khf) {
+        __builtin_amdgcn_sched_barrier(0);
+#pragma unroll
+        for (int g = 0; g < 6; ++g) {
+            const int set = g & 1, x0 = 2 * (g % 3);
+#pragma unroll
+            for (int i = 0; i < 8; ++i) {
+                const int j = i & 1, e = i >> 1;
+                const float av = e == 0 ? fa[set][j].x : e == 1 ? fa[set][j].y : e == 2 ? fa[set][j].z : fa[set][j].w;
+                const float bv = e == 0 ? fb[set][j].x : e == 1 ? fb[set][j].y : e == 2 ? fb[set][j].z : fb[set][j].w;
+                acc[x0 + j] = __builtin_amdgcn_mfma_f32_32x32x2f32(av, bv, acc[x0 + j], 0, 0, 0);
+                if (i < 4) {
+                    if (g < 5) frag_one(g + 1, set ^ 1, i, cur);
+                    else frag_one(0, 0, i, nxt);
+                } else {
+                    const int s = 4 * (g % 3) + (i - 4);
+                    if (s < 9) {
+                        if (g < 3) stage_one(s, nxt);
+                        else fetch_one(s, khf);
+                    }
+                }
+                __builtin_amdgcn_sched_barrier(0);
+            }
+            if (g == 4) {
+                __syncthreads();
+                __builtin_amdgcn_sched_barrier(0);
+            }
+        }
+        fetch_next(khf);
+    };
+    auto cold_start = [&]() {
+        decode(false);
+        fix_row1();
+#pragma unroll
+        for (int i = 0; i < 9; ++i) fetch_one(i, 0);
+        ++f_kt;
+#pragma unroll
+        for (int p = 0; p < 9; ++p) stage_one(p, X);
+#pragma unroll
+        for (int i = 0; i < 9; ++i) fetch_one(i, 1);
+        ++f_kt;
+    };
+
+    if (tid == 0) lds_i[0] = (int)atomicAdd(ticket, 1u);
+    __syncthreads();
+    f_item = __builtin_amdgcn_readfirstlane(lds_i[0]);
+    if (f_item >= n_items) return;
+    if (!wait_deps(f_item)) return;
+    cold_start();
+    const int ws = __builtin_amdgcn_readfirstlane(wave);
+    int c_item = f_item, c_k = f_k, c_m0 = f_m0, c_n0 = f_n0, c_ns = f_nk - f_kb;
+    __syncthreads();
+    for (;;) {
+        if (tid == 0) lds_i[0] = (int)atomicAdd(ticket, 1u);
+#pragma unroll
+        for (int xi = 0; xi < P; ++xi)
+#pragma unroll
+            for (int e = 0; e < 16; ++e) acc[xi][e] = 0.f;
+#pragma unroll
+        for (int i = 0; i < 4; ++i) frag_one(0, 0, i, X);
+        for (int s = 0; s < c_ns; s += 6) {
+            kstep(X, Y, 2);
+            kstep(Y, X, 0);
+            kstep(X, Y, 1);
+            kstep(Y, X, 2);
+            kstep(X, Y, 0);
+            kstep(Y, X, 1);
+        }
+        __syncthreads();
+        float* slab = lds + IMG8_FLOATS + ws * (64 * 36);
+        auto refetch = [&]() {
+            fix_row1();
+#pragma unroll
+            for (int i = 0; i < 9; ++i) fetch_one(i, 1);
+        };
+        int lane_e = lane;
+        asm volatile("" : "+v"(lane_e));
+        const ChainConv& cc = ch.c[c_k];
+        const Epi ep{cc.scale, cc.shift, cc.residual, cc.out, cc.relu};
+        wino43_epilogue_lean<decltype(refetch), rpg::kAuxAgentScope>(acc, slab, lane_e, c_m0 + (ws >> 1) * 32, c_n0 + (ws & 1) * 32, M,
+                                                                Tw, W, C, ep, refetch);
+        asm volatile("s_waitcnt vmcnt(0)" ::: "memory");
+        __syncthreads();
+        if (tid == 0) __hip_atomic_store(done + c_item, 1u, __ATOMIC_RELAXED, __HIP_MEMORY_SCOPE_AGENT);
+        if (f_item >= n_items) break;
+        bool ready = true;
+#pragma unroll
+        for (int w = 0; w < NT8 / 64; ++w) ready = ready && lds_i[8 + w] != 0;
+        if (!__builtin_amdgcn_readfirstlane((int)ready)) {
+            if (!wait_deps(f_item)) return;
+            cold_start();
+            __syncthreads();
+        }
+        c_item = f_item;
+        c_k = f_k;
+        c_m0 = f_m0;
+        c_n0 = f_n0;
+        c_ns = f_nk - f_kb;
+    }
+}
diff --git a/relpose-gnn_amd/csrc/winograd.hip b/relpose-gnn_amd/csrc/winograd.hip
--- a/relpose-gnn_amd/csrc/winograd.hip
+++ b/relpose-gnn_amd/csrc/winograd.hip
@@ -118,7 +118,7 @@
     }
 }
 
-template <bool RES, class Mid>
+template <bool RES, class Mid, int AUX = 0>
 __device__ __forceinline__ void wino43_epilogue_lean_body(const f32x16 (&acc)[P], float* slab, int lane, int mw0, int nw0, int M,
                                                           int Tw, int W, int Cout, const Epi& ep, Mid mid) {
     constexpr int EP = 32 + 4;
@@ -205,7 +205,7 @@
 #ifdef RPG_ABL_NOSTORE
             if (yv.x == 1234.5678f)
 #endif
-            __builtin_amdgcn_raw_buffer_store_b128(__builtin_bit_cast(u32x4, yv), ro, off(half, it), 0, 0);
+            __builtin_amdgcn_raw_buffer_store_b128(__builtin_bit_cast(u32x4, yv), ro, off(half, it), 0, AUX);
         }
     };
     load_res(0);
@@ -221,11 +221,11 @@
     __builtin_amdgcn_wave_barrier();
 }
 
-template <class Mid>
+template <class Mid, int AUX = 0>
 __device__ __forceinline__ void wino43_epilogue_lean(const f32x16 (&acc)[P], float* slab, int lane, int mw0, int nw0, int M,
                                                      int Tw, int W, int Cout, const Epi& ep, Mid mid) {
-    if (ep.residual) wino43_epilogue_lean_body<true>(acc, slab, lane, mw0, nw0, M, Tw, W, Cout, ep, mid);
-    else wino43_epilogue_lean_body<false>(acc, slab, lane, mw0, nw0, M, Tw, W, Cout, ep, mid);
+    if (ep.residual) wino43_epilogue_lean_body<true, Mid, AUX>(acc, slab, lane, mw0, nw0, M, Tw, W, Cout, ep, mid);
+    else wino43_epilogue_lean_body<false, Mid, AUX>(acc, slab, lane, mw0, nw0, M, Tw, W, Cout, ep, mid);
 }
 
 struct NoMid { __device__ __forceinline__ void operator()() const {} };
@@ -981,12 +981,21 @@
     for (int xi = 0; xi < 6; ++xi) U[xi * plane + i] = (float)u[xi];
 }
 
+#include "wino_chain.inc"
+
 int g_wino_split = 1;
 int g_wino_split_steps = 3;
 int g_wino = 1;
 int g_wino_min_blocks = 16;
 int g_wino_persist = 1;
 int g_wino_combine_max = 8;
+
+int g_wino_chain = 1;
+
+long chain_items(int n, int h, int w, int c) {
+    const long M = (long)n * h * ((w + 3) / 4);
+    return ((M + BMT8 - 1) / BMT8) * ((c + BN - 1) / BN);
+}
 
 }
 
@@ -1013,6 +1022,64 @@
     const int tw = (w + 3) / 4;
     return blocks >= g_wino_min_blocks && (long)h * w * cin * 4 * 67 < (1L << 31) && 6L * cout * 3 * cin * 4 < (1L << 31) &&
            (32L / tw + 3) * w * cout * 4 < (1L << 31);
+}
+
+void wino_chain_set(int on) { g_wino_chain = on; }
+
+bool wino_chain_fits(int n, int h, int w, int c) {
+    if (n <= 0 || h < 2 || w <= 0 || c <= 0 || c % (2 * BK) || !wino_pays(n, h, w, c, c)) return false;
+    if ((long)h * w * c * 4 * 131 >= (1L << 31) || (long)n * h * ((w + 3) / 4) >= (1L << 31)) return false;
+    const long items = chain_items(n, h, w, c);
+    return items >= num_cus() && items * kChainMax < (1L << 28);
+}
+bool wino_chain_takes(int n, int h, int w, int c) { return g_wino_chain && g_wino == 1 && wino_chain_fits(n, h, w, c); }
+
+size_t wino_chain_ctl_bytes(int n_conv, int n, int h, int w, int c) {
+    if (n_conv <= 0 || n_conv > kChainMax || n <= 0 || h <= 0 || w <= 0 || c <= 0) return 0;
+    return ((size_t)kChainCtlHead + (size_t)n_conv * chain_items(n, h, w, c)) * sizeof(unsigned);
+}
+
+int launch_wino_chain(const WinoChainConv* cv, int n_conv, int n, int h, int w, int c, void* ctl, size_t ctl_bytes, hipStream_t s,
+                      bool ctl_zeroed) {
+    if (!cv || n_conv <= 0 || n_conv > kChainMax || !ctl || ((uintptr_t)ctl & 3) || !wino_chain_fits(n, h, w, c) ||
+        ctl_bytes < wino_chain_ctl_bytes(n_conv, n, h, w, c))
+        return RPG_ERR_BAD_ARG;
+    Chain ch{};
+    for (int k = 0; k < n_conv; ++k) {
+        const WinoChainConv& a = cv[k];
+        if (!a.x || !a.u || !a.y || !aligned16(a.x) || !aligned16(a.u) || !aligned16(a.y) || (a.scale && !aligned16(a.scale)) ||
+            (a.shift && !aligned16(a.shift)) || (a.residual && !aligned16(a.residual)))
+            return RPG_ERR_BAD_ARG;
+        if (k > 0 && a.x != cv[k - 1].y) return RPG_ERR_BAD_ARG;
+        for (int j = 0; j < n_conv; ++j) {
+            if (j != k && cv[j].y == a.y) return RPG_ERR_BAD_ARG;
+            if (cv[j].x == a.y && j != k + 1) return RPG_ERR_BAD_ARG;
+            if (cv[j].residual == a.y && j != k + 1 && j != k + 2) return RPG_ERR_BAD_ARG;
+        }
+        ch.c[k] = ChainConv{a.x, a.u, a.scale, a.shift, a.residual, a.y, a.relu};
+    }
+    int dev = 0;
+    if (hipGetDevice(&dev) != hipSuccess || dev < 0 || dev >= 64) dev = 0;
+    static bool attr[64] = {};
+    if (!attr[dev]) {
+        (void)hipFuncSetAttribute(reinterpret_cast<const void*>(wino43_chain_kernel), hipFuncAttributeMaxDynamicSharedMemorySize,
+                                  LDS8_BYTES + kChainLdsExtra);
+        attr[dev] = true;
+    }
+    const int tw = (w + 3) / 4, tn = (c + BN - 1) / BN;
+    const long M = (long)n * h * tw, ipc = chain_items(n, h, w, c), items = ipc * n_conv;
+    const int S = num_cus();
+    if (!ctl_zeroed && hipMemsetAsync(ctl, 0, wino_chain_ctl_bytes(n_conv, n, h, w, c), s) != hipSuccess) {
+        rpg::set_last_error("wino43_chain memset", hipGetLastError());
+        return RPG_ERR_LAUNCH;
+    }
+    const int slot = timing_begin(RPG_TIMER_CONV_WINO, s);
+    hipLaunchKernelGGL(wino43_chain_kernel, dim3((unsigned)(items < S ? items : S)), dim3(NT8), LDS8_BYTES + kChainLdsExtra, s, ch, h,
+                       w, c, tw, (int)M, tn, (int)ipc, (int)items, reinterpret_cast<unsigned*>(ctl));
+    const double executed = (double)items * (3 * (c / BK)) * 48.0 * 8.0 * 4096.0;
+    timing_end(slot, n_conv * 2.0 * (double)n * h * w * c * 9.0 * c, s, executed);
+    RPG_CHECK_LAUNCH("wino43_chain");
+    return RPG_OK;
 }
 
 int launch_conv_wino(const float* x, const float* u, const float* scale, const float* shift, const float* residual,
@@ -1149,3 +1216,39 @@
                                                   int relu, void* stream) {
     return rpg::launch_conv_wino(x, u, scale, shift, residual, y, n, h, w, cin, cout, relu, rpg::as_stream(stream));
 }
+
+extern "C" size_t rpg_wino43_chain_ctl_bytes(int n_conv, int n, int h, int w, int c) {
+    return rpg::wino_chain_ctl_bytes(n_conv, n, h, w, c);
+}
+
+extern "C" int rpg_wino43_chain_f32(const float* const* convs, const int* relu, int n_conv, int n, int h, int w, int c, void* ctl,
+                                    size_t ctl_bytes, void* stream) {
+    if (!convs || !relu || n_conv <= 0 || n_conv > kChainMax) return RPG_ERR_BAD_ARG;
+    rpg::WinoChainConv cv[kChainMax];
+    for (int k = 0; k < n_conv; ++k)
+        cv[k] = rpg::WinoChainConv{convs[6 * k], convs[6 * k + 1], convs[6 * k + 2], convs[6 * k + 3], convs[6 * k + 4],
+                                   const_cast<float*>(convs[6 * k + 5]), relu[k]};
+    hipStream_t s = rpg::as_stream(stream);
+    const int rc = rpg::launch_wino_chain(cv, n_conv, n, h, w, c, ctl, ctl_bytes, s);
+    if (rc != RPG_OK) return rc;
+    unsigned err = 0;
+    if (hipStreamSynchronize(s) != hipSuccess ||
+        hipMemcpy(&err, reinterpret_cast<unsigned*>(ctl) + 1, sizeof(err), hipMemcpyDeviceToHost) != hipSuccess) {
+        rpg::set_last_error("wino43_chain", hipGetLastError());
+        return RPG_ERR_LAUNCH;
+    }
+    return err ? RPG_ERR_CHAIN_WAIT : RPG_OK;
+}
+
+extern "C" int rpg_wino43_chain_error(int reset) {
+    unsigned err = 0;
+    if (hipDeviceSynchronize() != hipSuccess || hipMemcpyFromSymbol(&err, HIP_SYMBOL(g_chain_error), sizeof(err)) != hipSuccess) {
+        rpg::set_last_error("wino43_chain_error", hipGetLastError());
+        return RPG_ERR_LAUNCH;
+    }
+    if (reset && err) {
+        const unsigned zero = 0;
+        if (hipMemcpyToSymbol(HIP_SYMBOL(g_chain_error), &zero, sizeof(zero)) != hipSuccess) return RPG_ERR_LAUNCH;
+    }
+    return err ? RPG_ERR_CHAIN_WAIT : RPG_OK;
+}
diff --git a/relpose-gnn_amd/ops.py b/relpose-gnn_amd/ops.py
--- a/relpose-gnn_amd/ops.py
+++ b/relpose-gnn_amd/ops.py
@@ -387,11 +387,35 @@
             for i, name in enumerate(L.TIMER_NAMES)}
 
 
+def wino43_chain(x: torch.Tensor, convs, residual0: Optional[torch.Tensor] = None) -> list:
+    x = _req(x, "x")
+    n, h, w, c = x.shape
+    k = len(convs)
+    ys = [torch.empty_like(x) for _ in range(k)]
+    ptrs, relu = [], []
+    for i, (u, scale, shift, res, rl) in enumerate(convs):
+        if u.dim() != 4 or tuple(u.shape) != (6, c, 3, c):
+            raise ValueError("u must be [6][C][3][C] from wino43_transform_weights")
+        r = None if res is None else x if res == "x" else residual0 if res == "r0" else ys[int(res)]
+        ptrs += [_p(x if i == 0 else ys[i - 1]), _p(_req(u, "u")), _p(scale), _p(shift), _p(r), _p(ys[i])]
+        relu.append(int(rl))
+    nbytes = int(L.lib().rpg_wino43_chain_ctl_bytes(k, n, h, w, c))
+    ctl = torch.empty(max(nbytes, 4), dtype=torch.uint8, device=x.device)
+    arr = (C.c_void_p * len(ptrs))(*ptrs)
+    rl_arr = (C.c_int * k)(*relu)
+    L.check(L.lib().rpg_wino43_chain_f32(arr, rl_arr, k, n, h, w, c, ctl.data_ptr(), nbytes, _stream()), "wino43_chain")
+    return ys
+
+
+def wino43_chain_error(reset: bool = True) -> int:
+    return int(L.lib().rpg_wino43_chain_error(int(reset)))
+
+
 def release_scratch() -> None:
     L.check(L.lib().rpg_release_scratch(), "release_scratch")
 
 
-TUNE_TILE, TUNE_BK, TUNE_EPILOGUE, TUNE_STREAMK, TUNE_WINOGRAD, TUNE_GNN_SPLIT, TUNE_BF16_BK, TUNE_FAST_LOADER, TUNE_WINO_SPLIT, TUNE_BF16_FAST, TUNE_FUSED_STEM, TUNE_WAVES8, TUNE_WINO_SHORT, TUNE_GNN_FUSE_AGG, TUNE_WINO_PERSIST, TUNE_BF16_TILE, TUNE_BF16_DMA, TUNE_BF16_PATCH, TUNE_BF16_WS64, TUNE_SK_MIN_ITS, TUNE_INKERNEL_FIXUP, TUNE_BF16_CHUNK, TUNE_WINO2D, TUNE_BF16_LEAN_EPI, TUNE_BF16_LINEAR_DMA, TUNE_BF16_PERSIST, TUNE_FOLD_K, TUNE_BF16_FUSE_BLOCK, TUNE_BF16_TAIL, TUNE_LIN112, TUNE_FIXUP_PRIO, TUNE_BF16_PAIR = 0, 1, 2, 3, 4, 5, 6, 7, 8, 9, 10, 11, 12, 13, 14, 15, 16, 17, 18, 19, 20, 21, 22, 23, 24, 25, 26, 27, 28, 29, 30, 31
+TUNE_TILE, TUNE_BK, TUNE_EPILOGUE, TUNE_STREAMK, TUNE_WINOGRAD, TUNE_GNN_SPLIT, TUNE_BF16_BK, TUNE_FAST_LOADER, TUNE_WINO_SPLIT, TUNE_BF16_FAST, TUNE_FUSED_STEM, TUNE_WAVES8, TUNE_WINO_SHORT, TUNE_GNN_FUSE_AGG, TUNE_WINO_PERSIST, TUNE_BF16_TILE, TUNE_BF16_DMA, TUNE_BF16_PATCH, TUNE_BF16_WS64, TUNE_SK_MIN_ITS, TUNE_INKERNEL_FIXUP, TUNE_BF16_CHUNK, TUNE_WINO2D, TUNE_BF16_LEAN_EPI, TUNE_BF16_LINEAR_DMA, TUNE_BF16_PERSIST, TUNE_FOLD_K, TUNE_BF16_FUSE_BLOCK, TUNE_BF16_TAIL, TUNE_LIN112, TUNE_FIXUP_PRIO, TUNE_BF16_PAIR, TUNE_WINO_CHAIN = 0, 1, 2, 3, 4, 5, 6, 7, 8, 9, 10, 11, 12, 13, 14, 15, 16, 17, 18, 19, 20, 21, 22, 23, 24, 25, 26, 27, 28, 29, 30, 31, 32
 
 
 def set_tuning(key: int, value: int) -> None:
```

After: 3058 graphs/s, median of 6. About the same (+0.6%).
